# viridityzhu/HiFiHR

Hardware: AMD Instinct MI355X
Metric: train images/sec, FreiHAND 224x224 (ResNet-18 + MANO LBS + render + losses + Adam) (higher is better)
Workload: dtype f32; 1 GPU; BASELINE configs[1]: FreiHAND batch=32/GPU, ResNet-18 encoder + MANO LBS + silhouette/texture render losses, 224x224, aa=3 (672^2 samples); per_gpu_batch=32, global_batch=32, parallelism=dp1

## Files before the change

hifihr_amd/_lib.py:

```python
from __future__ import annotations

import ctypes
import os
from ctypes import POINTER, c_char_p, c_float, c_int, c_int32, c_long, c_size_t, c_void_p

import torch

_HERE = os.path.dirname(os.path.abspath(__file__))
LIB_PATH = os.path.join(_HERE, "libhifihr.so")

_c_float_p = POINTER(c_float)


class _LinearDesc(ctypes.Structure):
    _fields_ = [("x", c_void_p), ("w", c_void_p), ("b", c_void_p), ("y", c_void_p), ("B", c_int), ("I", c_int), ("O", c_int), ("act", c_int),
                ("dy", c_void_p), ("dz_scratch", c_void_p), ("dW_acc", c_void_p), ("db_acc", c_void_p), ("dx", c_void_p)]

_c_int_p = POINTER(c_int32)


class HifihrError(RuntimeError):
    pass


# ... 74 lines not shown
        c.hifihr_conv2d_workspace_bytes.argtypes = [c_int] * 10
        c.hifihr_conv2d_workspace_bytes.restype = c_size_t
        c.hifihr_conv2d_bwd_data.argtypes = [_c_float_p] * 4 + ci + [c_void_p, c_size_t, c_void_p]
        c.hifihr_conv2d_fwd_bnstats.argtypes = [_c_float_p] * 4 + ci + [c_void_p, c_size_t, c_void_p]
        c.hifihr_conv2d_fwd_bnstats_pair_supported.argtypes = [c_int] * 11
        c.hifihr_conv2d_fwd_bnstats_pair.argtypes = [_c_float_p] * 4 + [c_int] * 3 + [_c_float_p] * 3 + [c_int] * 8 + [c_void_p]
        for fn in (c.hifihr_dwconv2d_bwd_data, c.hifihr_dwconv2d_bwd_weight):
            fn.argtypes = [_c_float_p] * 3 + [c_int] * 10 + [c_void_p]
        c.hifihr_dwconv2d_fwd.argtypes = [_c_float_p] * 4 + [c_int] * 10 + [c_void_p]
        c.hifihr_dwconv2d_fwd_bnswish.argtypes = [_c_float_p] * 8 + [c_int] * 10 + [c_void_p]
        c.hifihr_dwconv2d_bwd_weight_bnswish.argtypes = [_c_float_p] * 7 + [c_int] * 10 + [c_void_p]
        c.hifihr_bn_finalize_fwd.argtypes = [_c_float_p, c_long, c_int, c_float, c_float] + [_c_float_p] * 4 + [c_void_p]
        c.hifihr_bn_stats_floats.argtypes = [c_int]
        c.hifihr_bn_stats_floats.restype = c_int
        c.hifihr_bn_stats.argtypes = [_c_float_p, c_long, c_int, _c_float_p, c_void_p]
        c.hifihr_bn_act_fwd.argtypes = [_c_float_p] * 5 + [c_int, c_long, c_int, c_float, c_float] + [_c_float_p] * 5 + [c_void_p]
        c.hifihr_bn_act_eval.argtypes = [_c_float_p] * 6 + [c_int, c_long, c_int, c_float, _c_float_p, c_void_p]
        c.hifihr_bn_act_bwd.argtypes = [_c_float_p] * 7 + [c_int, c_long, c_int] + [_c_float_p] * 5 + [c_void_p]
        c.hifihr_bn_relu_maxpool_supported.argtypes = [c_int] * 4
        c.hifihr_bn_relu_maxpool_fwd.argtypes = [_c_float_p] * 4 + [c_int] * 4 + [c_float, c_float, _c_float_p, c_void_p] + [_c_float_p] * 4 + [c_void_p]
        c.hifihr_bn_relu_maxpool_bwd.argtypes = [_c_float_p, c_void_p] + [_c_float_p] * 5 + [c_int] * 4 + [_c_float_p] * 4 + [c_void_p]
        c.hifihr_bn_relu_maxpool_bwd_y.argtypes = [_c_float_p, _c_float_p, c_void_p] + [_c_float_p] * 5 + [c_int] * 4 + [_c_float_p] * 4 + [c_void_p]
        c.hifihr_conv2d_bwd_weight.argtypes = [_c_float_p] * 3 + ci + [c_void_p]
        c.hifihr_conv2d_bwd_weight_ws.argtypes = [_c_float_p] * 3 + ci + [c_void_p, c_size_t, c_void_p]
        c.hifihr_conv2d_wgrad_workspace_bytes.argtypes = ci
        c.hifihr_conv2d_bwd_weight_c3_supported.argtypes = [c_int] * 8
        c.hifihr_conv2d_bwd_weight_c3.argtypes = [_c_float_p] * 3 + [c_int] * 8 + [c_void_p, c_size_t, c_void_p]
        c.hifihr_conv2d_wgrad_workspace_bytes.restype = c_size_t
        c.hifihr_image_to_nhwc4.argtypes = [_c_float_p, _c_float_p, c_int, c_int, c_int, c_void_p]
        c.hifihr_image_to_nhwc4_padded.argtypes = [_c_float_p, _c_float_p] + [c_int] * 8 + [c_void_p]
        c.hifihr_image_scale_to_nhwc4.argtypes = [_c_float_p, _c_float_p, c_int, c_int, c_int, _c_float_p, _c_float_p, c_void_p]
        c.hifihr_maxpool2d_fwd_notap.argtypes = [_c_float_p] + [c_int] * 7 + [_c_float_p, c_void_p]
        c.hifihr_lpips_tap_max_channels.argtypes = []
        c.hifihr_lpips_tap_max_channels.restype = c_int
        c.hifihr_lpips_tap_partial_floats.argtypes = [c_int]
        c.hifihr_lpips_tap_partial_floats.restype = c_size_t
        c.hifihr_lpips_tap.argtypes = [_c_float_p] * 3 + [c_int] * 4 + [_c_float_p, _c_float_p, c_void_p]
        c.hifihr_lpips_tap_bwd.argtypes = [_c_float_p] * 4 + [c_int] * 4 + [_c_float_p, c_void_p]
        c.hifihr_lpips_tap_bwd_relu.argtypes = [_c_float_p] * 4 + [c_int] * 4 + [_c_float_p, c_void_p]
        c.hifihr_lpips_maxpool_fwd.argtypes = [_c_float_p] + [c_int] * 4 + [_c_float_p, c_void_p]
        c.hifihr_lpips_maxpool_bwd.argtypes = [_c_float_p, _c_float_p] + [c_int] * 4 + [_c_float_p, c_void_p]
        c.hifihr_image_scale_to_nhwc4_bwd.argtypes = [_c_float_p, _c_float_p, c_int, c_int, c_int, _c_float_p, c_void_p]
        c.hifihr_geom_loss_fwd.argtypes = [_c_float_p] * 6 + [_c_int_p] + [c_int] * 7 + [_c_float_p] * 3 + [c_void_p]
        c.hifihr_geom_loss_bwd.argtypes = [_c_float_p] * 6 + [_c_int_p] * 3 + [c_int] * 7 + [_c_float_p] * 6 + [c_void_p]
        c.hifihr_photo_loss_partial_floats.argtypes = []
        c.hifihr_photo_loss_partial_floats.restype = c_int
        c.hifihr_photo_loss_fwd.argtypes = [_c_float_p, _c_float_p, c_void_p, c_int, c_int, c_int, c_float, c_float, c_float] + \
            [_c_float_p] * 4 + [c_void_p]
        c.hifihr_photo_loss_bwd.argtypes = [_c_float_p] * 6 + [c_int, c_int, c_int, c_float, c_float, _c_float_p, c_void_p]
        c.hifihr_sil_post.argtypes = [_c_float_p, _c_float_p, c_int, c_int, c_int, _c_float_p, _c_float_p, c_void_p]
        c.hifihr_linear_fwd.argtypes = [_c_float_p] * 3 + [c_int] * 4 + [_c_float_p] * 2 + [c_float, c_float] + [_c_float_p] * 6 + [c_void_p]
        c.hifihr_linear_bwd.argtypes = [_c_float_p] * 4 + [c_int] * 4 + [_c_float_p] * 10 + [c_void_p]
        c.hifihr_linear_fwd_group.argtypes = [POINTER(_LinearDesc), c_int, c_void_p]
        c.hifihr_linear_bwd_group.argtypes = [POINTER(_LinearDesc), c_int, c_void_p]
        c.hifihr_conv2d_bwd_data_pre.argtypes = [_c_float_p] * 3 + [c_int] * 9 + [c_void_p, c_size_t, c_void_p]
        c.hifihr_conv2d_bwd_data_pre_res.argtypes = [_c_float_p] * 4 + [c_int] * 9 + [c_void_p, c_size_t, c_void_p]
        c.hifihr_conv2d_bwd_data_pre_plus1x1.argtypes = [_c_float_p] * 5 + [c_int] * 9 + [c_void_p]
        c.hifihr_conv2d_bwd_data_pre_plus1x1_supported.argtypes = [c_int] * 9
        c.hifihr_conv2d_bwd_weight_plus1x1.argtypes = [_c_float_p] * 5 + [c_int] * 9 + [c_void_p]
        c.hifihr_conv2d_bwd_weight_plus1x1_supported.argtypes = [c_int] * 9
        c.hifihr_weight_prep.argtypes = [c_void_p, c_int, c_int, c_void_p]
        c.hifihr_freihand_augment.argtypes = [c_void_p, c_void_p, _c_int_p, _c_int_p, c_int, c_int, c_int, _c_float_p, _c_float_p, c_void_p]
        c.hifihr_ho3d_workspace_bytes.argtypes = [c_int, c_int]
        c.hifihr_ho3d_workspace_bytes.restype = c_size_t
        c.hifihr_ho3d_batch.argtypes = ([c_void_p, c_void_p] + [_c_float_p] * 3 + [c_int, c_int, _c_int_p, c_int, c_int, c_void_p, c_size_t] +
                                        [_c_float_p] * 5 + [c_void_p])
        c.hifihr_freihand_batch.argtypes = ([c_void_p, c_void_p] + [_c_float_p] * 4 + [c_int, c_int, _c_int_p, c_int, c_int, c_int, _c_float_p,
                                            _c_float_p, c_void_p] + [_c_float_p] * 6 + [c_void_p, c_void_p])
        c.hifihr_freihand_batch_step.argtypes = ([c_void_p, c_void_p] + [_c_float_p] * 4 + [c_int, c_int, _c_int_p, c_int, c_int, c_int, _c_float_p,
                                                 _c_float_p, c_void_p] + [_c_float_p] * 6 + [c_void_p, c_int, c_float] + [_c_float_p] * 4 + [c_void_p])
        c.hifihr_light_split_fwd.argtypes = [_c_float_p, c_int, _c_float_p, _c_float_p, c_void_p]
        c.hifihr_light_split_bwd.argtypes = [_c_float_p, _c_float_p, _c_float_p, c_int, _c_float_p, c_void_p]
        c.hifihr_wino4_bwd_gemm_pair_supported.argtypes = [c_int] * 5
        c.hifihr_wino4_bwd_gemm_pair.argtypes = [_c_float_p] * 6 + [c_int] * 6 + [c_void_p]
        c.hifihr_loss_total_fwd.argtypes = [POINTER(_c_float_p), POINTER(c_int), c_int, _c_float_p, c_void_p]
        c.hifihr_loss_total_bwd.argtypes = [_c_float_p, POINTER(_c_float_p), POINTER(c_int), POINTER(c_int), c_int, c_void_p]
        c.hifihr_procrustes_error.argtypes = [_c_float_p, _c_float_p, c_int, c_int, _c_float_p, _c_float_p, c_void_p]
        c.hifihr_point_error_hist.argtypes = [_c_float_p, _c_float_p, c_void_p, c_int, c_int, POINTER(ctypes.c_double), c_int, _c_int_p, c_void_p,
                                              c_void_p]
        c.hifihr_fscore_counts.argtypes = [_c_float_p, _c_float_p, c_int, c_int, c_int, POINTER(ctypes.c_double), c_int, _c_int_p, c_void_p]
        c.hifihr_wino_wgrad_gemm.argtypes = [_c_float_p] * 3 + [c_int] * 5 + [c_void_p]
        c.hifihr_wino_dw_transform.argtypes = [_c_float_p, _c_float_p, c_int, c_int, c_int, c_void_p]
        c.hifihr_weight_transpose.argtypes = [_c_float_p, _c_float_p, c_int, c_int, c_int, c_void_p]
        c.hifihr_bgemm_nt.argtypes = [_c_float_p] * 3 + [c_int] * 4 + [c_void_p, c_size_t, c_void_p]
        c.hifihr_bgemm_nt_workspace_bytes.argtypes = [c_int] * 4
        c.hifihr_bgemm_nt_workspace_bytes.restype = c_size_t
        c.hifihr_renderer_set_light_mode.argtypes = [c_void_p, c_int]
        c.hifihr_texture_pca_fwd.argtypes = [_c_float_p] * 3 + [c_int, c_int, c_long, _c_float_p, c_void_p]
        c.hifihr_texture_pca_bwd.argtypes = [_c_float_p] * 2 + [c_int, c_int, c_long, _c_float_p, c_void_p]
        c.hifihr_comm_last_error.restype = c_char_p
        c.hifihr_comm_get_unique_id.argtypes = [c_void_p]
        c.hifihr_comm_init.argtypes = [POINTER(c_void_p), c_int, c_int, c_void_p]
        c.hifihr_comm_allreduce_f32.argtypes = [c_void_p, _c_float_p, c_size_t, c_void_p]
        c.hifihr_comm_broadcast_f32.argtypes = [c_void_p, _c_float_p, c_size_t, c_int, c_void_p]
        c.hifihr_comm_destroy.argtypes = [c_void_p]
        c.hifihr_wino_tile.argtypes = [c_int] * 5
        c.hifihr_wino_gemm_workspace_bytes.argtypes = [c_int] * 6
        c.hifihr_wino_gemm_workspace_bytes.restype = c_size_t
        c.hifihr_wino_weight_transform.argtypes = [_c_float_p, _c_float_p, c_int, c_int, c_int, c_int, c_void_p]
        c.hifihr_wino_input_transform.argtypes = [_c_float_p, _c_float_p] + [c_int] * 5 + [c_void_p]
        c.hifihr_wino_gemm.argtypes = [_c_float_p] * 3 + [c_int] * 6 + [c_void_p, c_size_t, c_void_p]
        c.hifihr_wino_output_transform.argtypes = [_c_float_p] * 3 + [c_int] * 5 + [c_void_p]
        c.hifihr_wino_output_transform_act.argtypes = [_c_float_p] * 3 + [c_int] * 6 + [c_void_p]
        c.hifihr_conv3x3_c64_wino_supported.argtypes = [c_int] * 5
        c.hifihr_conv3x3_c64_wino.argtypes = [c_void_p, c_void_p, c_void_p, c_int, c_void_p, c_void_p, c_int, c_int, c_int, c_void_p]
        c.hifihr_conv3x3_c64_wino_res.argtypes = [c_void_p, c_void_p, c_void_p, c_void_p, c_int, c_int, c_int, c_void_p]
        c.hifihr_conv3x3_c64_bwd_pair_supported.argtypes = [c_int] * 3
        c.hifihr_conv3x3_c64_bwd_pair.argtypes = [c_void_p] * 7 + [c_size_t] + [c_int] * 3 + [c_void_p]
        c.hifihr_conv3x3_c64_bwd_pair_slabs.argtypes = [c_void_p] * 6 + [c_size_t] + [c_int] * 3 + [c_void_p, c_void_p]
        c.hifihr_conv_halo_wgrad_reduce_multi.argtypes = [c_void_p, c_int, c_void_p]
        c.hifihr_wino_bn_input_supported.argtypes = [c_int, c_int]
        c.hifihr_wino_bn_input_transform.argtypes = [_c_float_p] * 7 + [c_int] * 5 + [c_float, c_float] + [_c_float_p] * 4 + [c_void_p]
        c.hifihr_wino_output_transform_bnred.argtypes = [_c_float_p] * 10 + [c_int] * 5 + [c_void_p]
        c.hifihr_wino_bn_bwd_dual_transform.argtypes = [_c_float_p] * 8 + [c_int] * 5 + [_c_float_p] * 2 + [c_void_p]
        c.hifihr_bn_bwd_apply.argtypes = [_c_float_p] * 5 + [c_long, c_int] + [_c_float_p] * 4 + [c_void_p]
        c.hifihr_joint_terms_fwd.argtypes = [_c_float_p] * 4 + [c_int] * 3 + [POINTER(c_float), _c_float_p, c_void_p]
        c.hifihr_joint_terms_bwd.argtypes = [_c_float_p] * 4 + [c_int] * 3 + [POINTER(c_float)] + [_c_float_p] * 3 + [c_void_p]
        c.hifihr_wino_dy_transform.argtypes = [_c_float_p] * 2 + [c_int] * 5 + [c_void_p]
        c.hifihr_wino_input_dy_transform.argtypes = [_c_float_p] * 3 + [c_int] * 5 + [c_void_p]
        c.hifihr_wino_wgrad_parts.argtypes = [c_int] * 6
        c.hifihr_wino_wgrad_gemm_parts.argtypes = [_c_float_p] * 3 + [c_int] * 7 + [c_void_p]
        c.hifihr_wino_dw_transform_parts.argtypes = [_c_float_p, c_int, _c_float_p, c_int, c_int, c_int, c_void_p]
        c.hifihr_bgemm_describe.argtypes = [c_int] * 5 + [ctypes.c_char_p, c_int]
        c.hifihr_conv2d_describe.argtypes = [c_int] * 10 + [ctypes.c_char_p, c_int]
        c.hifihr_bgemm_tn_parts.argtypes = [c_int] * 4
        c.hifihr_bgemm_tn.argtypes = [_c_float_p] * 3 + [c_int] * 5 + [c_void_p]
        c.hifihr_wino4_dw_transform_multi.argtypes = [c_void_p, c_int, c_void_p]
        c.hifihr_se_pool.argtypes = [_c_float_p, c_int, c_int, c_int, _c_float_p, c_void_p]
        c.hifihr_se_scale.argtypes = [_c_float_p, _c_float_p, _c_float_p, c_float, c_int, c_int, c_int, _c_float_p, c_void_p]
        c.hifihr_se_bwd_gate.argtypes = [_c_float_p, _c_float_p, c_int, c_int, c_int, _c_float_p, c_void_p]
        c.hifihr_se_mlp_supported.argtypes = [c_int, c_int]
        c.hifihr_wino_tiles.argtypes = [c_int] * 4
        c.hifihr_wino_tiles.restype = c_long
        c.hifihr_wino_tiles_computed.argtypes = [c_int] * 4
        c.hifihr_wino_tiles_computed.restype = c_long
        c.hifihr_zero_page_ready.argtypes = [c_void_p]
        c.hifihr_drop_connect_add.argtypes = [_c_float_p, _c_float_p, _c_float_p, c_float, c_int, c_size_t, _c_float_p, c_void_p]
        c.hifihr_se_mlp_fwd.argtypes = [_c_float_p] * 5 + [c_int] * 3 + [_c_float_p] * 4 + [c_void_p]
        c.hifihr_se_mlp_bwd.argtypes = [_c_float_p] * 7 + [c_int] * 3 + [_c_float_p] * 7 + [c_void_p]
        c.hifihr_mmpool_fwd.argtypes = [_c_float_p, _c_float_p, c_int, c_int, c_int, _c_float_p, _c_int_p, _c_float_p, _c_float_p, c_void_p]
        c.hifihr_mmpool_bwd.argtypes = [_c_float_p, _c_float_p, _c_int_p, _c_float_p, _c_float_p, c_int, c_int, c_int, _c_float_p,
                                        _c_float_p, c_void_p]
        c.hifihr_maxpool2d_fwd.argtypes = [_c_float_p] + [c_int] * 7 + [_c_float_p, c_void_p, c_void_p]
        c.hifihr_maxpool2d_bwd.argtypes = [_c_float_p, c_void_p] + [c_int] * 7 + [_c_float_p, c_void_p]
        c.hifihr_maxpool2d_fwd_flat.argtypes = [_c_float_p] + [c_int] * 7 + [_c_float_p, c_void_p, c_void_p]
        c.hifihr_maxpool2d_bwd_flat.argtypes = [_c_float_p, c_void_p] + [c_int] * 7 + [_c_float_p, c_void_p]
        c.hifihr_maxpool2d_bwd_relu.argtypes = [_c_float_p, c_void_p, _c_float_p] + [c_int] * 7 + [_c_float_p, c_void_p]
        c.hifihr_wino_output_transform_mask.argtypes = [_c_float_p] * 3 + [c_int] * 5 + [c_void_p]
        c.hifihr_adam_step.argtypes = [_c_float_p, _c_float_p, _c_float_p, _c_float_p, c_size_t, c_float, c_float, c_float,
                                       c_float, c_float, c_float, c_int, c_void_p]
        c.hifihr_adam_state_bytes.restype = c_size_t
        c.hifihr_adam_state_bytes.argtypes = []
        c.hifihr_adam_step_counted.argtypes = [_c_float_p, _c_float_p, _c_float_p, _c_float_p, c_size_t, c_float, c_float, c_float, c_void_p, c_void_p]
        c.hifihr_grad_guard_bytes.restype = c_size_t
        c.hifihr_grad_guard_bytes.argtypes = []
        c.hifihr_grad_norm_workspace_bytes.restype = c_size_t
        c.hifihr_grad_norm_workspace_bytes.argtypes = [c_size_t]
        c.hifihr_grad_norm.argtypes = [_c_float_p, c_size_t, c_float, c_float, c_void_p, c_void_p, c_void_p]
        c.hifihr_adam_step_guarded.argtypes = [_c_float_p, _c_float_p, _c_float_p, _c_float_p, c_size_t, c_float, c_float, c_float, c_float,
                                               c_float, c_float, c_int, c_void_p, c_void_p, c_void_p]
        c.hifihr_adam_step_dyn.argtypes = [_c_float_p, _c_float_p, _c_float_p, _c_float_p, c_size_t, c_float, c_float, c_float,
                                           c_float, c_float, _c_float_p, c_void_p]
        c.hifihr_renderer_destroy.argtypes = [c_void_p]
        c.hifihr_render_workspace_bytes.argtypes = [c_void_p, c_int]
        c.hifihr_render_workspace_bytes.restype = c_size_t
        c.hifihr_render_fwd.argtypes = [c_void_p, _c_float_p, _c_float_p, c_int, _c_float_p, _c_float_p, _c_float_p, c_int,
                                        _c_float_p, _c_int_p, c_void_p, c_void_p]
        c.hifihr_render_bwd.argtypes = [c_void_p, _c_float_p, _c_float_p, _c_float_p, _c_float_p, _c_int_p, _c_float_p, c_int,
                                        _c_float_p, _c_float_p, _c_float_p, _c_float_p, c_void_p, c_void_p]
        c.hifihr_soft_sil_workspace_bytes.argtypes = [c_void_p, c_int]
        c.hifihr_soft_sil_workspace_bytes.restype = c_size_t
        c.hifihr_soft_sil_fwd.argtypes = [c_void_p, _c_float_p, _c_float_p, c_int, c_float, c_float, _c_float_p, _c_float_p, c_void_p, c_void_p]
        c.hifihr_soft_sil_bwd.argtypes = [c_void_p, _c_float_p, _c_float_p, _c_float_p, _c_float_p, c_int, c_float, c_float, _c_float_p, c_void_p,
                                          c_void_p]
        c.hifihr_soft_sil_loss_fwd.argtypes = [_c_float_p, c_void_p, c_int, c_int, c_int, c_float, c_float, c_void_p, _c_float_p, c_void_p]
        c.hifihr_soft_sil_loss_bwd.argtypes = [_c_float_p, c_void_p, c_int, c_void_p, _c_float_p, c_int, c_int, c_float, c_float, _c_float_p,
                                               c_void_p]
        c.hifihr_mesh_topology_create.argtypes = [_c_int_p, c_int, c_int]
        c.hifihr_mesh_topology_create.restype = c_void_p
        c.hifihr_mesh_topology_destroy.argtypes = [c_void_p]
        c.hifihr_mesh_topology_counts.argtypes = [c_void_p, _c_int_p, _c_int_p, _c_int_p]
        c.hifihr_mesh_reg_partial_floats.argtypes = [c_void_p, c_int]
        c.hifihr_mesh_reg_partial_floats.restype = c_size_t
        c.hifihr_mesh_reg_fwd.argtypes = [c_void_p, _c_float_p, c_int, c_float, c_float, _c_float_p, _c_float_p, _c_float_p, c_void_p]
        c.hifihr_mesh_reg_bwd.argtypes = [c_void_p, _c_float_p, _c_float_p, _c_float_p, c_int, c_float, c_float, _c_float_p, c_void_p]
        c.hifihr_chamfer_geometry.argtypes = [_c_int_p, _c_int_p]
        c.hifihr_chamfer_geometry.restype = None
        c.hifihr_chamfer_workspace_bytes.argtypes = [c_int, c_int, c_int]
        c.hifihr_chamfer_workspace_bytes.restype = c_size_t
        c.hifihr_chamfer_fwd.argtypes = [_c_float_p, _c_float_p, c_int, c_int, c_int, c_float, c_float, _c_int_p, _c_int_p, c_void_p, c_void_p,
                                         c_void_p, _c_float_p, c_void_p, c_void_p]
        c.hifihr_chamfer_bwd.argtypes = [_c_float_p, _c_float_p, _c_int_p, _c_int_p, _c_float_p, c_int, c_int, c_int, c_float, c_float,
                                         _c_float_p, _c_float_p, c_void_p]
        c.hifihr_renderer_set_uv.argtypes = [c_void_p, _c_int_p, _c_float_p, c_int]
        c.hifihr_render_uv_scratch_bytes.argtypes = [c_void_p, c_int]
        c.hifihr_render_uv_scratch_bytes.restype = c_size_t
        c.hifihr_render_fwd_uv.argtypes = [c_void_p, _c_float_p, _c_float_p, c_int, c_int, _c_float_p, _c_float_p, _c_float_p, c_int, _c_float_p,
                                           _c_int_p, _c_float_p, c_void_p, c_void_p]
        c.hifihr_render_bwd_uv.argtypes = [c_void_p, _c_float_p, _c_float_p, c_int, c_int, _c_float_p, _c_float_p, _c_float_p, _c_int_p, _c_float_p,
                                           c_int] + [_c_float_p] * 6 + [c_void_p, c_void_p]

    def check(self, rc: int, what: str):
        if rc != 0:
            raise HifihrError(f"{what} failed ({rc}): {self.c.hifihr_last_error().decode()}")

    def mano_create(self, tables) -> c_void_p:
        h = c_void_p()
        keep = [_np_fp(a) for a in (tables.v_template, tables.shapedirs, tables.posedirs, tables.J_regressor,
                                    tables.weights, tables.hands_components, tables.hands_mean)]
        self.check(self.c.hifihr_mano_create(ctypes.byref(h), *[k[1] for k in keep]), "hifihr_mano_create")
        return h

    def mano_destroy(self, h):
        self.c.hifihr_mano_destroy(h)

    def mano_lbs_fwd(self, h, pose, beta, verts, jtr, saved):
        B = pose.shape[0]
        assert pose.shape == (B, 48) and beta.shape == (B, 10) and verts.shape == (B, 778, 3)
        self.check(self.c.hifihr_mano_lbs_fwd(h, _fp(pose), _fp(beta), B, _fp(verts), _fp(jtr), _fp(saved),
                                              _stream_of(pose)), "hifihr_mano_lbs_fwd")

    def mano_lbs_bwd(self, h, pose, beta, saved, gverts, gjtr, gpose, gbeta):
        B = pose.shape[0]
        self.check(self.c.hifihr_mano_lbs_bwd(h, _fp(pose), _fp(beta), _fp(saved), _fp(gverts), _fp(gjtr), B,
                                              _fp(gpose), _fp(gbeta), _stream_of(pose)), "hifihr_mano_lbs_bwd")

    def mano_joints_fwd(self, h, verts, root_id, joints_rel, verts_rel, root):
        B = verts.shape[0]
        self.check(self.c.hifihr_mano_joints_fwd(h, _fp(verts), B, root_id, _fp(joints_rel), _fp(verts_rel), _fp(root),
                                                 _stream_of(verts)), "hifihr_mano_joints_fwd")

    def mano_joints_bwd(self, h, gjoints_rel, gverts_rel, groot, root_id, gverts):
        B = gverts.shape[0]
        self.check(self.c.hifihr_mano_joints_bwd(h, _fp(gjoints_rel), _fp(gverts_rel), _fp(groot), B, root_id,
                                                 _fp(gverts), _stream_of(gverts)), "hifihr_mano_joints_bwd")

    def mano_full_fwd(self, h, pose, beta, root_id, root_xyz, verts, joints_rel, verts_rel, verts_cam, root, saved):
        B = pose.shape[0]
        self.check(self.c.hifihr_mano_full_fwd(h, _fp(pose), _fp(beta), B, int(root_id), _fp(root_xyz), _fp(verts), _fp(joints_rel), _fp(verts_rel),
                                               _fp(verts_cam), _fp(root), _fp(saved), _stream_of(pose)), "hifihr_mano_full_fwd")

    def mano_full_bwd(self, h, pose, beta, saved, gjoints_rel, gverts_rel, gverts_cam, groot, root_id, gpose, gbeta, gpose_add=None,
                      gbeta_add=None):
        B = pose.shape[0]
        self.check(self.c.hifihr_mano_full_bwd(h, _fp(pose), _fp(beta), _fp(saved), _fp(gjoints_rel), _fp(gverts_rel), _fp(gverts_cam),
                                               _fp(groot), _fp(gpose_add), _fp(gbeta_add), B, int(root_id), _fp(gpose), _fp(gbeta),
                                               _stream_of(pose)), "hifihr_mano_full_bwd")

    def lbs_create(self, v_template, shapedirs, j_regressor, weights, parents) -> c_void_p:
        V, J, S = int(v_template.shape[0]), int(weights.shape[1]), int(shapedirs.shape[2])
        assert shapedirs.shape == (V, 3, S) and j_regressor.shape == (J, V) and weights.shape == (V, J) and len(parents) == J
        h = c_void_p()
        keep = [_np_fp(a) for a in (v_template, shapedirs, j_regressor, weights)]
        import numpy as np
        par = np.ascontiguousarray(np.asarray(parents, dtype=np.int32))
        self.check(self.c.hifihr_lbs_create(ctypes.byref(h), V, J, S, *[k[1] for k in keep], par.ctypes.data_as(_c_int_p)), "hifihr_lbs_create")
        return h

    def lbs_destroy(self, h):
        self.c.hifihr_lbs_destroy(h)

    def lbs_fwd(self, h, theta, beta, verts, joints):
        self.check(self.c.hifihr_lbs_fwd(h, _fp(theta), _fp(beta), theta.shape[0], _fp(verts), _fp(joints), _stream_of(theta)), "hifihr_lbs_fwd")

    def lbs_bwd(self, h, theta, beta, gverts, gjoints, scratch, gtheta, gbeta):
        self.check(self.c.hifihr_lbs_bwd(h, _fp(theta), _fp(beta), _fp(gverts), _fp(gjoints), theta.shape[0], _fp(scratch), _fp(gtheta),
                                         _fp(gbeta), _stream_of(theta)), "hifihr_lbs_bwd")

    @staticmethod
    def _ws(ws):
        if ws is None:
            return c_void_p(0), c_size_t(0)
        assert ws.is_contiguous()
        return c_void_p(ws.data_ptr()), c_size_t(ws.numel() * ws.element_size())

    def conv2d_workspace_bytes(self, N, H, W, C, K, R, S, stride, pad, bwd_data=False):
        return int(self.c.hifihr_conv2d_workspace_bytes(N, H, W, C, K, R, S, stride, pad, int(bool(bwd_data))))

    def conv2d_fwd(self, x, w, bias, y, N, H, W, C, K, R, S, stride, pad, ws=None, act=0):
        self.check(self.c.hifihr_conv2d_fwd(_fp(x), _fp(w), _fp(bias), int(act), _fp(y), N, H, W, C, K, R, S, stride, pad,
                                            *self._ws(ws), _stream_of(x)), "hifihr_conv2d_fwd")

    def bias_relu_bwd(self, dy, y, M, C, g, db_acc):
        self.check(self.c.hifihr_bias_relu_bwd(_fp(dy), _fp(y), c_long(M), C, _fp(g), _fp(db_acc), _stream_of(dy)),
                   "hifihr_bias_relu_bwd")

    def conv2d_fwd_bnstats(self, x, w, y, stats, N, H, W, C, K, R, S, stride, pad, ws=None):
        self.check(self.c.hifihr_conv2d_fwd_bnstats(_fp(x), _fp(w), _fp(y), _fp(stats), N, H, W, C, K, R, S, stride, pad,
                                                    *self._ws(ws), _stream_of(x)), "hifihr_conv2d_fwd_bnstats")

    def conv2d_fwd_bnstats_pair_supported(self, N, H, W, C, stride, K1, R1, pad1, K2, R2, pad2):
        return bool(self.c.hifihr_conv2d_fwd_bnstats_pair_supported(N, H, W, C, stride, K1, R1, pad1, K2, R2, pad2))

    def conv2d_fwd_bnstats_pair(self, x, w1, y1, stats1, K1, R1, pad1, w2, y2, stats2, K2, R2, pad2, N, H, W, C, stride):
        self.check(self.c.hifihr_conv2d_fwd_bnstats_pair(_fp(x), _fp(w1), _fp(y1), _fp(stats1), K1, R1, pad1, _fp(w2), _fp(y2), _fp(stats2), K2, R2, pad2,
                                                         N, H, W, C, stride, _stream_of(x)), "hifihr_conv2d_fwd_bnstats_pair")

    def bn_stats_floats(self, C):
        return int(self.c.hifihr_bn_stats_floats(int(C)))

    def bn_stats(self, x, M, C, stats):
        self.check(self.c.hifihr_bn_stats(_fp(x), c_long(M), C, _fp(stats), _stream_of(x)), "hifihr_bn_stats")

    def bn_act_fwd(self, x, stats, gamma, beta, residual, act, M, C, eps, momentum, y, save_mean, save_invstd, rmean, rvar):
        self.check(self.c.hifihr_bn_act_fwd(_fp(x), _fp(stats), _fp(gamma), _fp(beta), _fp(residual), int(act), c_long(M), C,
                                            c_float(eps), c_float(momentum), _fp(y), _fp(save_mean), _fp(save_invstd), _fp(rmean),
# ... 451 lines not shown
                                            _fp(rm), _fp(rv), _fp(y), _fp(z), _fp(sm), _fp(si), _stream_of(x)), "hifihr_linear_fwd")

    def linear_bwd(self, dy, y, x, w, act, dz, dW_acc, db_acc, dx, bn=None, z=None):
        B, I = x.shape
        O = w.shape[0]
        gamma, z_bn, sm, si, dg, dbt = bn if bn is not None else (None,) * 6
        z = z_bn if bn is not None else z
        self.check(self.c.hifihr_linear_bwd(_fp(dy), _fp(y), _fp(x), _fp(w), B, I, O, int(act), _fp(gamma), _fp(z), _fp(sm), _fp(si),
                                            _fp(dz), _fp(dW_acc), _fp(db_acc), _fp(dg), _fp(dbt), _fp(dx), _stream_of(x)),
                   "hifihr_linear_bwd")

    @staticmethod
    def _descs(members):
        arr = (_LinearDesc * len(members))()
        p = lambda t: None if t is None else t.data_ptr()
        for d, m in zip(arr, members):
            d.x, d.w, d.b, d.y = p(m["x"]), p(m["w"]), p(m.get("b")), p(m["y"])
            d.B, d.I, d.O, d.act = m["x"].shape[0], m["x"].shape[1], m["w"].shape[0], int(m["act"])
            d.dy, d.dz_scratch, d.dW_acc, d.db_acc, d.dx = p(m.get("dy")), p(m.get("dz")), p(m.get("dW")), p(m.get("db")), p(m.get("dx"))
        return arr

    def linear_fwd_group(self, members):
        self.check(self.c.hifihr_linear_fwd_group(self._descs(members), len(members), _stream_of(members[0]["x"])), "hifihr_linear_fwd_group")

    def linear_bwd_group(self, members):
        self.check(self.c.hifihr_linear_bwd_group(self._descs(members), len(members), _stream_of(members[0]["x"])), "hifihr_linear_bwd_group")

    def mmpool_fwd(self, x, p, B, HW, C, y, argmax, xmax, xavg):
        self.check(self.c.hifihr_mmpool_fwd(_fp(x), _fp(p), B, HW, C, _fp(y), _ip(argmax), _fp(xmax), _fp(xavg), _stream_of(x)),
                   "hifihr_mmpool_fwd")

    def mmpool_bwd(self, gy, p, argmax, xmax, xavg, B, HW, C, dx, dp_acc):
        self.check(self.c.hifihr_mmpool_bwd(_fp(gy), _fp(p), _ip(argmax), _fp(xmax), _fp(xavg), B, HW, C, _fp(dx), _fp(dp_acc),
                                            _stream_of(gy)), "hifihr_mmpool_bwd")

    def maxpool2d_fwd(self, x, N, H, W, C, k, s, p, y, tap):
        assert tap.dtype == torch.uint8 and tap.is_contiguous()
        self.check(self.c.hifihr_maxpool2d_fwd(_fp(x), N, H, W, C, k, s, p, _fp(y), c_void_p(tap.data_ptr()), _stream_of(x)),
                   "hifihr_maxpool2d_fwd")

    def maxpool2d_fwd_flat(self, x, N, H, W, C, k, s, p, y_flat, tap):
        self.check(self.c.hifihr_maxpool2d_fwd_flat(_fp(x), N, H, W, C, k, s, p, _fp(y_flat), c_void_p(tap.data_ptr()), _stream_of(x)),
                   "hifihr_maxpool2d_fwd_flat")

    def maxpool2d_bwd_flat(self, gy_flat, tap, N, H, W, C, k, s, p, dx):
        self.check(self.c.hifihr_maxpool2d_bwd_flat(_fp(gy_flat), c_void_p(tap.data_ptr()), N, H, W, C, k, s, p, _fp(dx), _stream_of(gy_flat)),
                   "hifihr_maxpool2d_bwd_flat")

    def maxpool2d_bwd(self, gy, tap, N, H, W, C, k, s, p, dx, relu_y=None):
        if relu_y is not None:
            self.check(self.c.hifihr_maxpool2d_bwd_relu(_fp(gy), c_void_p(tap.data_ptr()), _fp(relu_y), N, H, W, C, k, s, p, _fp(dx),
                                                        _stream_of(gy)), "hifihr_maxpool2d_bwd_relu")
            return
        self.check(self.c.hifihr_maxpool2d_bwd(_fp(gy), c_void_p(tap.data_ptr()), N, H, W, C, k, s, p, _fp(dx), _stream_of(gy)),
                   "hifihr_maxpool2d_bwd")

    def conv2d_bwd_data(self, dy, w, dx, scratch, N, H, W, C, K, R, S, stride, pad, ws=None):
        self.check(self.c.hifihr_conv2d_bwd_data(_fp(dy), _fp(w), _fp(dx), _fp(scratch), N, H, W, C, K, R, S, stride, pad,
                                                 *self._ws(ws), _stream_of(dy)), "hifihr_conv2d_bwd_data")

    def conv2d_wgrad_workspace_bytes(self, N, H, W, C, K, R, S, stride, pad):
        return int(self.c.hifihr_conv2d_wgrad_workspace_bytes(N, H, W, C, K, R, S, stride, pad))

    def conv2d_bwd_weight(self, x, dy, dw, N, H, W, C, K, R, S, stride, pad, ws=None):
        p, n = self._ws(ws)
        self.check(self.c.hifihr_conv2d_bwd_weight_ws(_fp(x), _fp(dy), _fp(dw), N, H, W, C, K, R, S, stride, pad, p, n, _stream_of(x)),
                   "hifihr_conv2d_bwd_weight")

    def image_to_nhwc4(self, images, out):
        B, _, H, W = images.shape
        self.check(self.c.hifihr_image_to_nhwc4(_fp(images), _fp(out), B, H, W, _stream_of(images)), "hifihr_image_to_nhwc4")

    def image_to_nhwc4_padded(self, images, out, pad4, normalize):
        B, _, H, W = images.shape
        pl, pr, pt, pb = pad4
        self.check(self.c.hifihr_image_to_nhwc4_padded(_fp(images), _fp(out), B, H, W, pt, pl, pb, pr, int(bool(normalize)),
                                                       _stream_of(images)), "hifihr_image_to_nhwc4_padded")

    def image_scale_to_nhwc4(self, images, out, shift3, scale3):
        B, _, H, W = images.shape
        sh, sc = (c_float * 3)(*[float(v) for v in shift3]), (c_float * 3)(*[float(v) for v in scale3])
        self.check(self.c.hifihr_image_scale_to_nhwc4(_fp(images), _fp(out), B, H, W, sh, sc, _stream_of(images)), "hifihr_image_scale_to_nhwc4")

    def maxpool2d_fwd_notap(self, x, N, H, W, C, k, s, p, y):
        self.check(self.c.hifihr_maxpool2d_fwd_notap(_fp(x), N, H, W, C, k, s, p, _fp(y), _stream_of(x)), "hifihr_maxpool2d_fwd_notap")

    def lpips_tap_max_channels(self):
        return int(self.c.hifihr_lpips_tap_max_channels())

    def lpips_tap_partial_floats(self, B):
        return int(self.c.hifihr_lpips_tap_partial_floats(int(B)))

    def lpips_tap(self, f0, f1, w, B, HW, C, partial, val, accumulate=False):
        self.check(self.c.hifihr_lpips_tap(_fp(f0), _fp(f1), _fp(w), B, HW, C, int(bool(accumulate)), _fp(partial), _fp(val), _stream_of(f0)),
                   "hifihr_lpips_tap")

    def lpips_tap_bwd(self, f0, f1, w, gval, B, HW, C, gf0, accumulate=False, relu=False):
        fn, name = (self.c.hifihr_lpips_tap_bwd_relu, "hifihr_lpips_tap_bwd_relu") if relu else (self.c.hifihr_lpips_tap_bwd, "hifihr_lpips_tap_bwd")
        self.check(fn(_fp(f0), _fp(f1), _fp(w), _fp(gval), B, HW, C, int(bool(accumulate)), _fp(gf0), _stream_of(f0)), name)

    def lpips_maxpool_fwd(self, x, N, H, W, C, y):
        self.check(self.c.hifihr_lpips_maxpool_fwd(_fp(x), N, H, W, C, _fp(y), _stream_of(x)), "hifihr_lpips_maxpool_fwd")

    def lpips_maxpool_bwd(self, gy, x, N, H, W, C, dx):
        self.check(self.c.hifihr_lpips_maxpool_bwd(_fp(gy), _fp(x), N, H, W, C, _fp(dx), _stream_of(x)), "hifihr_lpips_maxpool_bwd")

    def image_scale_to_nhwc4_bwd(self, g4, gimg, scale3):
        B, _, H, W = gimg.shape
        sc = (c_float * 3)(*[float(v) for v in scale3])
        self.check(self.c.hifihr_image_scale_to_nhwc4_bwd(_fp(g4), _fp(gimg), B, H, W, sc, _stream_of(gimg)), "hifihr_image_scale_to_nhwc4_bwd")

    def ssim_partial_count(self, planes, H, W):
        return int(self.c.hifihr_ssim_partial_count(planes, H, W))

    def ssim_fwd(self, window, img1, img2, partial, dA, dB, dC):
        planes, H, W = img1.shape[0] * img1.shape[1], img1.shape[2], img1.shape[3]
        self.check(self.c.hifihr_ssim_fwd(window, _fp(img1), _fp(img2), planes, H, W, _fp(partial), _fp(dA), _fp(dB), _fp(dC),
                                          _stream_of(img1)), "hifihr_ssim_fwd")

    def ssim_finish(self, partial, scale, offset, out):
        self.check(self.c.hifihr_ssim_finish(_fp(partial), partial.numel(), c_float(scale), c_float(offset), _fp(out), _stream_of(partial)),
                   "hifihr_ssim_finish")

    def ssim_bwd_scaled(self, window, img1, img2, dA, dB, dC, grad_out, out_scale, gimg1):
        planes, H, W = img1.shape[0] * img1.shape[1], img1.shape[2], img1.shape[3]
        self.check(self.c.hifihr_ssim_bwd_scaled(window, _fp(img1), _fp(img2), _fp(dA), _fp(dB), _fp(dC), _fp(grad_out), c_float(out_scale),
                                                 planes, H, W, _fp(gimg1), _stream_of(img1)), "hifihr_ssim_bwd_scaled")

    def ssim_bwd(self, window, img1, img2, dA, dB, dC, grad_out, gimg1):
        planes, H, W = img1.shape[0] * img1.shape[1], img1.shape[2], img1.shape[3]
        self.check(self.c.hifihr_ssim_bwd(window, _fp(img1), _fp(img2), _fp(dA), _fp(dB), _fp(dC), _fp(grad_out), planes, H, W,
                                          _fp(gimg1), _stream_of(img1)), "hifihr_ssim_bwd")

    def adam_step(self, p, g, m, v, grad_scale, lr, beta1, beta2, eps, weight_decay, step):
        n = p.numel()
        assert g.numel() == n and m.numel() == n and v.numel() == n
        self.check(self.c.hifihr_adam_step(_fp(p), _fp(g), _fp(m), _fp(v), c_size_t(n), c_float(grad_scale), c_float(lr),
                                           c_float(beta1), c_float(beta2), c_float(eps), c_float(weight_decay), int(step),
                                           _stream_of(p)), "hifihr_adam_step")

    @staticmethod
    def adam_state_image(lr, beta1, beta2, step):
        import struct
        b1, b2 = float(beta1), float(beta2)
        return torch.frombuffer(bytearray(struct.pack("<dddddii", float(lr), b1, b2, b1 ** int(step), b2 ** int(step), int(step), 0)),
                                dtype=torch.uint8).clone()

    def adam_step_counted(self, p, g, m, v, grad_scale, eps, weight_decay, state):
        n = p.numel()
        assert state.dtype == torch.uint8 and state.numel() == int(self.c.hifihr_adam_state_bytes()) and state.device == p.device
        self.check(self.c.hifihr_adam_step_counted(_fp(p), _fp(g), _fp(m), _fp(v), c_size_t(n), c_float(grad_scale), c_float(eps),
                                                   c_float(weight_decay), c_void_p(state.data_ptr()), _stream_of(p)), "hifihr_adam_step_counted")

    def adam_step_dyn(self, p, g, m, v, grad_scale, beta1, beta2, eps, weight_decay, dyn):
        n = p.numel()
        self.check(self.c.hifihr_adam_step_dyn(_fp(p), _fp(g), _fp(m), _fp(v), c_size_t(n), c_float(grad_scale), c_float(beta1),
                                               c_float(beta2), c_float(eps), c_float(weight_decay), _fp(dyn), _stream_of(p)),
                   "hifihr_adam_step_dyn")

    def grad_guard_alloc(self, n, device):
        guard = torch.zeros(int(self.c.hifihr_grad_guard_bytes()), dtype=torch.uint8, device=device)
        ws = torch.zeros(int(self.c.hifihr_grad_norm_workspace_bytes(c_size_t(n))), dtype=torch.uint8, device=device)
        return guard, ws

    def grad_norm(self, g, grad_scale, max_norm, guard, ws):
        n = g.numel()
        assert guard.dtype == torch.uint8 and guard.numel() == int(self.c.hifihr_grad_guard_bytes()) and guard.device == g.device
        assert ws.dtype == torch.uint8 and ws.numel() >= int(self.c.hifihr_grad_norm_workspace_bytes(c_size_t(n))) and ws.device == g.device
        self.check(self.c.hifihr_grad_norm(_fp(g), c_size_t(n), c_float(grad_scale), c_float(max_norm), c_void_p(guard.data_ptr()),
                                           c_void_p(ws.data_ptr()), _stream_of(g)), "hifihr_grad_norm")

    def adam_step_guarded(self, p, g, m, v, grad_scale, lr, beta1, beta2, eps, weight_decay, step, state, guard):
        n = p.numel()
        assert g.numel() == n and m.numel() == n and v.numel() == n
        assert guard.dtype == torch.uint8 and guard.numel() == int(self.c.hifihr_grad_guard_bytes()) and guard.device == p.device
        if state is not None:
            assert state.dtype == torch.uint8 and state.numel() == int(self.c.hifihr_adam_state_bytes()) and state.device == p.device
        self.check(self.c.hifihr_adam_step_guarded(_fp(p), _fp(g), _fp(m), _fp(v), c_size_t(n), c_float(grad_scale), c_float(lr),
                                                   c_float(beta1), c_float(beta2), c_float(eps), c_float(weight_decay), int(step),
                                                   c_void_p(state.data_ptr()) if state is not None else c_void_p(0),
                                                   c_void_p(guard.data_ptr()), _stream_of(p)), "hifihr_adam_step_guarded")

    @staticmethod
    def grad_guard_unpack(raw):
        import struct
        norm, coef, finite, steps, clipped, skipped, _ = struct.unpack("<dfiiiii", bytes(raw))
        return {"norm": norm, "clip_coef": coef, "finite": bool(finite), "steps": steps, "clipped": clipped, "skipped": skipped}

    def renderer_create(self, faces, V, image_size=224, aa=3, ambient=(0.5, 0.5, 0.5), mat_diffuse=(0.8, 0.8, 0.8),
                        specular=(0.04, 0.04, 0.04), shininess=30.0, background=(1.0, 1.0, 1.0)) -> c_void_p:
        import numpy as np
        f = np.ascontiguousarray(faces, dtype=np.int32)
        h = c_void_p()
        a, m, s, b = (_np_fp(x) for x in (ambient, mat_diffuse, specular, background))
        self.check(self.c.hifihr_renderer_create(ctypes.byref(h), f.ctypes.data_as(_c_int_p), int(V), int(f.shape[0]),
                                                 int(image_size), int(aa), a[1], m[1], s[1], c_float(shininess), b[1]),
                   "hifihr_renderer_create")
        return h

    def texture_pca_fwd(self, coef, basis, mean, out):
        B, K = coef.shape
        n = basis.shape[1]
        self.check(self.c.hifihr_texture_pca_fwd(_fp(coef), _fp(basis), _fp(mean), B, K, c_long(n), _fp(out), _stream_of(coef)), "hifihr_texture_pca_fwd")

    def texture_pca_bwd(self, gtex, basis, dcoef_zeroed):
        B, K = dcoef_zeroed.shape
        n = basis.shape[1]
        self.check(self.c.hifihr_texture_pca_bwd(_fp(gtex), _fp(basis), B, K, c_long(n), _fp(dcoef_zeroed), _stream_of(gtex)), "hifihr_texture_pca_bwd")

    def renderer_set_light_mode(self, h, point_lights):
        self.check(self.c.hifihr_renderer_set_light_mode(h, int(bool(point_lights))), "hifihr_renderer_set_light_mode")

    def renderer_destroy(self, h):
        self.c.hifihr_renderer_destroy(h)

    def render_workspace_bytes(self, h, B) -> int:
        return int(self.c.hifihr_render_workspace_bytes(h, int(B)))

    def render_fwd(self, h, verts, vcolors, cam, light_color, light_dir, rgba, face_id, ws):
        B = verts.shape[0]
        batched = 1 if vcolors.dim() == 3 else 0
        self.check(self.c.hifihr_render_fwd(h, _fp(verts), _fp(vcolors), batched, _fp(cam), _fp(light_color), _fp(light_dir), B,
                                            _fp(rgba), _ip(face_id), c_void_p(ws.data_ptr()), _stream_of(verts)),
                   "hifihr_render_fwd")

    def renderer_set_uv(self, h, faces_uvs, verts_uvs):
        import numpy as np
        fu = np.ascontiguousarray(faces_uvs, dtype=np.int32)
        vu = np.ascontiguousarray(verts_uvs, dtype=np.float32)
        self.check(self.c.hifihr_renderer_set_uv(h, fu.ctypes.data_as(_c_int_p), vu.ctypes.data_as(_c_float_p), vu.shape[0]),
                   "hifihr_renderer_set_uv")

    def render_uv_scratch_bytes(self, h, B):
        return int(self.c.hifihr_render_uv_scratch_bytes(h, B))

    def render_fwd_uv(self, h, verts, maps, cam, light_color, light_dir, rgba, face_id, texels, ws):
        B, TH, TW = maps.shape[0], maps.shape[1], maps.shape[2]
        self.check(self.c.hifihr_render_fwd_uv(h, _fp(verts), _fp(maps), TH, TW, _fp(cam), _fp(light_color), _fp(light_dir), B, _fp(rgba),
                                               _ip(face_id), _fp(texels), c_void_p(ws.data_ptr()), _stream_of(verts)), "hifihr_render_fwd_uv")

    def render_bwd_uv(self, h, verts, maps, cam, light_color, light_dir, face_id, grad_rgba, texels, gtexels, gverts, gmaps, glc, gld, ws):
        B, TH, TW = maps.shape[0], maps.shape[1], maps.shape[2]
        self.check(self.c.hifihr_render_bwd_uv(h, _fp(verts), _fp(maps), TH, TW, _fp(cam), _fp(light_color), _fp(light_dir), _ip(face_id),
                                               _fp(grad_rgba), B, _fp(texels), _fp(gtexels), _fp(gverts), _fp(gmaps), _fp(glc), _fp(gld),
                                               c_void_p(ws.data_ptr()), _stream_of(verts)), "hifihr_render_bwd_uv")

    def render_bwd(self, h, verts, cam, light_color, light_dir, face_id, grad_rgba, gverts, gvcolors, glc, gld, ws):
        B = verts.shape[0]
        self.check(self.c.hifihr_render_bwd(h, _fp(verts), _fp(cam), _fp(light_color), _fp(light_dir), _ip(face_id),
                                            _fp(grad_rgba), B, _fp(gverts), _fp(gvcolors), _fp(glc), _fp(gld),
                                            c_void_p(ws.data_ptr()), _stream_of(verts)), "hifihr_render_bwd")

    def soft_sil_workspace_bytes(self, h, B) -> int:
        return int(self.c.hifihr_soft_sil_workspace_bytes(h, int(B)))

    def soft_sil_fwd(self, h, verts, cam, sigma, blur_radius, alpha, neglog, ws):
        self.check(self.c.hifihr_soft_sil_fwd(h, _fp(verts), _fp(cam), verts.shape[0], c_float(sigma), c_float(blur_radius), _fp(alpha),
                                              _fp(neglog), c_void_p(ws.data_ptr()), _stream_of(verts)), "hifihr_soft_sil_fwd")

    def soft_sil_bwd(self, h, verts, cam, neglog, galpha, sigma, blur_radius, gverts, ws):
        self.check(self.c.hifihr_soft_sil_bwd(h, _fp(verts), _fp(cam), _fp(neglog), _fp(galpha), verts.shape[0], c_float(sigma),
                                              c_float(blur_radius), _fp(gverts), c_void_p(ws.data_ptr()), _stream_of(verts)),
                   "hifihr_soft_sil_bwd")

    @staticmethod
    def _mask_arg(mask):
        assert mask.dtype in (torch.float32, torch.int64) and mask.is_contiguous(), (mask.dtype, mask.stride())
        return c_void_p(mask.data_ptr()), int(mask.dtype == torch.int64)

    def soft_sil_loss_fwd(self, alpha, mask, lam_sil, lam_iou, sums, out):
        B = alpha.shape[0]
        assert sums.dtype == torch.float64 and sums.is_contiguous() and mask.numel() == alpha.numel()
        mp, kind = self._mask_arg(mask)
        self.check(self.c.hifihr_soft_sil_loss_fwd(_fp(alpha), mp, kind, B, alpha.numel() // max(B, 1), c_float(lam_sil), c_float(lam_iou),
                                                   c_void_p(sums.data_ptr()), _fp(out), _stream_of(alpha)), "hifihr_soft_sil_loss_fwd")

    def soft_sil_loss_bwd(self, alpha, mask, sums, gout, lam_sil, lam_iou, galpha):
        B = alpha.shape[0]
        mp, kind = self._mask_arg(mask)
        self.check(self.c.hifihr_soft_sil_loss_bwd(_fp(alpha), mp, kind, c_void_p(sums.data_ptr()), _fp(gout), B, alpha.numel() // max(B, 1),
                                                   c_float(lam_sil), c_float(lam_iou), _fp(galpha), _stream_of(alpha)),
                   "hifihr_soft_sil_loss_bwd")

    def mesh_topology_create(self, faces, V) -> c_void_p:
        import numpy as np
        f = np.ascontiguousarray(faces, dtype=np.int32)
        assert f.ndim == 2 and f.shape[1] == 3, f.shape
        h = self.c.hifihr_mesh_topology_create(f.ctypes.data_as(_c_int_p), int(f.shape[0]), int(V))
        if not h:
            raise HifihrError(f"hifihr_mesh_topology_create failed: {self.c.hifihr_last_error().decode()}")
        return c_void_p(h)

    def mesh_topology_destroy(self, h):
        self.c.hifihr_mesh_topology_destroy(h)

    def mesh_topology_counts(self, h):
        v, e, q = c_int32(), c_int32(), c_int32()
        self.check(self.c.hifihr_mesh_topology_counts(h, ctypes.byref(v), ctypes.byref(e), ctypes.byref(q)), "hifihr_mesh_topology_counts")
        return v.value, e.value, q.value

    def mesh_reg_partial_floats(self, h, B) -> int:
        return int(self.c.hifihr_mesh_reg_partial_floats(h, int(B)))

    def mesh_reg_fwd(self, h, verts, lam_lap, lam_nc, unit, partial, out):
        self.check(self.c.hifihr_mesh_reg_fwd(h, _fp(verts), verts.shape[0], c_float(lam_lap), c_float(lam_nc), _fp(unit), _fp(partial),
                                              _fp(out), _stream_of(verts)), "hifihr_mesh_reg_fwd")
# ... 43 lines not shown
```

hifihr_amd/csrc/adam.hip:

```cpp
#include <hip/hip_runtime.h>

#include "hifihr_internal.h"

namespace hifihr {

struct GradGuard {
  double norm;
  float coef;
  int finite;
  int steps, clipped, skipped;
  int pad;
};

template <bool kGuard>
__global__ __launch_bounds__(256) void adam_kernel_t(float* __restrict__ p, const float* __restrict__ g, float* __restrict__ m,
                                                    float* __restrict__ v, size_t n, float grad_scale, float beta1, float beta2,
                                                    float eps, float weight_decay, float step_size, float inv_sqrt_bc2,
                                                    const float* __restrict__ dyn, const GradGuard* __restrict__ guard) {
  if (dyn) { step_size = dyn[0]; inv_sqrt_bc2 = dyn[1]; }
  if constexpr (kGuard) {
    if (!guard->finite) return;
    grad_scale = grad_scale * guard->coef;
  }
  const size_t n4 = n / 4;
  const size_t stride = (size_t)gridDim.x * blockDim.x;
  float4* p4 = reinterpret_cast<float4*>(p);
  const float4* g4 = reinterpret_cast<const float4*>(g);
  float4* m4 = reinterpret_cast<float4*>(m);
  float4* v4 = reinterpret_cast<float4*>(v);
  for (size_t i = (size_t)blockIdx.x * blockDim.x + threadIdx.x; i < n4; i += stride) {
    float4 pp = p4[i], gg = g4[i], mm = m4[i], vv = v4[i];
    float* pa = reinterpret_cast<float*>(&pp);
    float* ga = reinterpret_cast<float*>(&gg);
    float* ma = reinterpret_cast<float*>(&mm);
    float* va = reinterpret_cast<float*>(&vv);
#pragma unroll
    for (int k = 0; k < 4; ++k) {
      const float gr = ga[k] * grad_scale + weight_decay * pa[k];
      ma[k] = beta1 * ma[k] + (1.f - beta1) * gr;
      va[k] = beta2 * va[k] + (1.f - beta2) * gr * gr;
      const float denom = sqrtf(va[k]) * inv_sqrt_bc2 + eps;
      pa[k] = pa[k] - step_size * (ma[k] / denom);
    }
    p4[i] = pp; m4[i] = mm; v4[i] = vv;
  }
  for (size_t i = n4 * 4 + (size_t)blockIdx.x * blockDim.x + threadIdx.x; i < n; i += stride) {
    const float gr = g[i] * grad_scale + weight_decay * p[i];
    const float mi = beta1 * m[i] + (1.f - beta1) * gr;
    const float vi = beta2 * v[i] + (1.f - beta2) * gr * gr;
    m[i] = mi; v[i] = vi;
    p[i] = p[i] - step_size * (mi / (sqrtf(vi) * inv_sqrt_bc2 + eps));
  }
}

constexpr auto adam_kernel = adam_kernel_t<false>;
constexpr auto adam_kernel_guarded = adam_kernel_t<true>;

struct AdamState {
  double lr, beta1, beta2;
  double pow1, pow2;
  int step;
  int done;
};
template <bool kGuard>
__global__ __launch_bounds__(256) void adam_kernel_counted_t(float* __restrict__ p, const float* __restrict__ g, float* __restrict__ m,
                                                            float* __restrict__ v, size_t n, float grad_scale, float eps,
                                                            float weight_decay, AdamState* __restrict__ st,
                                                            const GradGuard* __restrict__ guard) {
  __shared__ float sc[4];
  int t = 0;
  double q1 = 0.0, q2 = 0.0;
  if (threadIdx.x == 0) {
    t = st->step + 1;
    const double b1 = st->beta1, b2 = st->beta2;
    q1 = st->pow1 * b1; q2 = st->pow2 * b2;
    sc[0] = (float)(st->lr / (1.0 - q1));
    sc[1] = (float)(1.0 / sqrt(1.0 - q2));
    sc[2] = (float)b1; sc[3] = (float)b2;
  }
  __syncthreads();
  const float step_size = sc[0], inv_sqrt_bc2 = sc[1], beta1 = sc[2], beta2 = sc[3];
  bool run = true;
  if constexpr (kGuard) {
    run = guard->finite != 0;
    grad_scale = grad_scale * guard->coef;
  }
  const size_t n4 = run ? n / 4 : 0;
  const size_t n_end = run ? n : 0;
  const size_t stride = (size_t)gridDim.x * blockDim.x;
  float4* p4 = reinterpret_cast<float4*>(p);
  const float4* g4 = reinterpret_cast<const float4*>(g);
  float4* m4 = reinterpret_cast<float4*>(m);
  float4* v4 = reinterpret_cast<float4*>(v);
  for (size_t i = (size_t)blockIdx.x * blockDim.x + threadIdx.x; i < n4; i += stride) {
    float4 pp = p4[i], gg = g4[i], mm = m4[i], vv = v4[i];
    float* pa = reinterpret_cast<float*>(&pp);
    float* ga = reinterpret_cast<float*>(&gg);
    float* ma = reinterpret_cast<float*>(&mm);
    float* va = reinterpret_cast<float*>(&vv);
#pragma unroll
    for (int k = 0; k < 4; ++k) {
      const float gr = ga[k] * grad_scale + weight_decay * pa[k];
      ma[k] = beta1 * ma[k] + (1.f - beta1) * gr;
      va[k] = beta2 * va[k] + (1.f - beta2) * gr * gr;
      const float denom = sqrtf(va[k]) * inv_sqrt_bc2 + eps;
      pa[k] = pa[k] - step_size * (ma[k] / denom);
    }
    p4[i] = pp; m4[i] = mm; v4[i] = vv;
  }
  for (size_t i = n4 * 4 + (size_t)blockIdx.x * blockDim.x + threadIdx.x; i < n_end; i += stride) {
    const float gr = g[i] * grad_scale + weight_decay * p[i];
    const float mi = beta1 * m[i] + (1.f - beta1) * gr;
    const float vi = beta2 * v[i] + (1.f - beta2) * gr * gr;
    m[i] = mi; v[i] = vi;
    p[i] = p[i] - step_size * (mi / (sqrtf(vi) * inv_sqrt_bc2 + eps));
  }
  __syncthreads();
  if (threadIdx.x == 0) {
    if (atomicAdd(&st->done, 1) == (int)gridDim.x - 1) {
      st->step = t;
      st->pow1 = q1; st->pow2 = q2;
      st->done = 0;
    }
  }
}

constexpr auto adam_kernel_counted = adam_kernel_counted_t<false>;
constexpr auto adam_kernel_counted_guarded = adam_kernel_counted_t<true>;

__device__ __forceinline__ double block_sum_f64(double s, double* lds) {
#pragma unroll
  for (int off = 32; off > 0; off >>= 1) s += __shfl_down(s, off, 64);
  if ((threadIdx.x & 63) == 0) lds[threadIdx.x >> 6] = s;
  __syncthreads();
  return (lds[0] + lds[1]) + (lds[2] + lds[3]);
}

__global__ __launch_bounds__(256) void grad_sqsum_kernel(const float* __restrict__ g, size_t n, double* __restrict__ partial) {
  __shared__ double lds[4];
  const size_t n4 = n / 4;
  const size_t stride = (size_t)gridDim.x * blockDim.x;
  const float4* g4 = reinterpret_cast<const float4*>(g);
  double s0 = 0.0, s1 = 0.0;
  for (size_t i = (size_t)blockIdx.x * blockDim.x + threadIdx.x; i < n4; i += stride) {
    const float4 gg = g4[i];
    const double x = gg.x, y = gg.y, z = gg.z, w = gg.w;
    s0 += x * x; s1 += y * y;
    s0 += z * z; s1 += w * w;
  }
  for (size_t i = n4 * 4 + (size_t)blockIdx.x * blockDim.x + threadIdx.x; i < n; i += stride) {
    const double x = g[i];
    s0 += x * x;
  }
  const double s = block_sum_f64(s0 + s1, lds);
  if (threadIdx.x == 0) partial[blockIdx.x] = s;
}

__global__ __launch_bounds__(256) void grad_norm_finish_kernel(const double* __restrict__ partial, int nblk, float grad_scale, float max_norm,
                                                              GradGuard* __restrict__ guard) {
  __shared__ double lds[4];
  double s = 0.0;
  for (int i = threadIdx.x; i < nblk; i += 256) s += partial[i];
  s = block_sum_f64(s, lds);
  if (threadIdx.x == 0) {
    const bool finite = fabs(s) <= 1.7976931348623157e308;
    const double norm = fabs((double)grad_scale) * sqrt(s);
    float coef = 0.f;
    if (finite) {
      const double c = (double)max_norm / (norm + 1e-6);
      coef = c >= 1.0 ? 1.0f : (float)c;
    }
    guard->norm = norm;
    guard->coef = coef;
    guard->finite = finite ? 1 : 0;
    guard->steps += 1;
    if (finite && coef < 1.0f) guard->clipped += 1;
    if (!finite) guard->skipped += 1;
  }
}

static size_t adam_blocks(size_t n) {
  size_t blocks = (n / 4 + 255) / 256;
  if (blocks > 2048) blocks = 2048;
  if (blocks < 1) blocks = 1;
  return blocks;
}

size_t grad_guard_bytes() { return sizeof(GradGuard); }
size_t grad_norm_workspace_bytes(size_t n) { return adam_blocks(n) * sizeof(double); }

hipError_t launch_grad_norm(const float* g, size_t n, float grad_scale, float max_norm, void* guard, void* ws, hipStream_t st) {
  const size_t blocks = adam_blocks(n);
  hipLaunchKernelGGL(grad_sqsum_kernel, dim3((unsigned)blocks), dim3(256), 0, st, g, n, static_cast<double*>(ws));
  hipError_t e = hipGetLastError();
  if (e != hipSuccess) return e;
  hipLaunchKernelGGL(grad_norm_finish_kernel, dim3(1), dim3(256), 0, st, static_cast<const double*>(ws), (int)blocks, grad_scale, max_norm,
                     static_cast<GradGuard*>(guard));
  return hipGetLastError();
}

hipError_t launch_adam_guarded(float* p, const float* g, float* m, float* v, size_t n, float grad_scale, float lr, float beta1, float beta2,
                               float eps, float weight_decay, int step, void* state, const void* guard, hipStream_t st) {
  const size_t blocks = adam_blocks(n);
  if (state) {
    hipLaunchKernelGGL(adam_kernel_counted_guarded, dim3((unsigned)blocks), dim3(256), 0, st, p, g, m, v, n, grad_scale, eps, weight_decay,
                       static_cast<AdamState*>(state), static_cast<const GradGuard*>(guard));
    return hipGetLastError();
  }
  const double bc1 = 1.0 - pow((double)beta1, (double)step);
  const double bc2 = 1.0 - pow((double)beta2, (double)step);
  const float step_size = (float)((double)lr / bc1);
  const float inv_sqrt_bc2 = (float)(1.0 / sqrt(bc2));
  hipLaunchKernelGGL(adam_kernel_guarded, dim3((unsigned)blocks), dim3(256), 0, st, p, g, m, v, n, grad_scale, beta1, beta2, eps,
                     weight_decay, step_size, inv_sqrt_bc2, (const float*)nullptr, static_cast<const GradGuard*>(guard));
  return hipGetLastError();
}

size_t adam_state_bytes() { return sizeof(AdamState); }

hipError_t launch_adam_counted(float* p, const float* g, float* m, float* v, size_t n, float grad_scale, float eps, float weight_decay,
                               void* state, hipStream_t st) {
  size_t blocks = (n / 4 + 255) / 256;
  if (blocks > 2048) blocks = 2048;
  if (blocks < 1) blocks = 1;
  hipLaunchKernelGGL(adam_kernel_counted, dim3((unsigned)blocks), dim3(256), 0, st, p, g, m, v, n, grad_scale, eps, weight_decay,
                     static_cast<AdamState*>(state), (const GradGuard*)nullptr);
  return hipGetLastError();
}

hipError_t launch_adam(float* p, const float* g, float* m, float* v, size_t n, float grad_scale, float lr, float beta1,
                       float beta2, float eps, float weight_decay, int step, const float* dyn, hipStream_t st) {
  float step_size = 0.f, inv_sqrt_bc2 = 0.f;
  if (!dyn) {
    const double bc1 = 1.0 - pow((double)beta1, (double)step);
    const double bc2 = 1.0 - pow((double)beta2, (double)step);
    step_size = (float)((double)lr / bc1);
    inv_sqrt_bc2 = (float)(1.0 / sqrt(bc2));
  }
  size_t blocks = (n / 4 + 255) / 256;
  if (blocks > 2048) blocks = 2048;
  if (blocks < 1) blocks = 1;
  hipLaunchKernelGGL(adam_kernel, dim3((unsigned)blocks), dim3(256), 0, st, p, g, m, v, n, grad_scale, beta1, beta2, eps,
                     weight_decay, step_size, inv_sqrt_bc2, dyn, (const GradGuard*)nullptr);
  return hipGetLastError();
}

}
```

hifihr_amd/csrc/hifihr_api.hip:

```cpp
#include <hip/hip_runtime.h>

#include <algorithm>
#include <array>
#include <cmath>
#include <cstdarg>
#include <cstdio>
#include <cstring>
#include <new>
#include <vector>

#include "../../include/hifihr.h"
#include "hifihr_internal.h"
#include "mano_math.h"

namespace {

thread_local char g_err[512] = "";

int fail(int code, const char* fmt, ...) {
  va_list ap;
  va_start(ap, fmt);
  vsnprintf(g_err, sizeof(g_err), fmt, ap);
  va_end(ap);
  return code;
// ... 444 lines not shown
    }
    for (int k = 0; k < 3; ++k) {
      const int i = v[k], j = v[(k + 1) % 3], o = v[(k + 2) % 3];
      sides.push_back({std::min(i, j), std::max(i, j), f, o});
    }
  }
  std::sort(sides.begin(), sides.end());
  std::vector<int> off(V + 1, 0), quads;
  std::vector<std::array<int, 2>> edges;
  for (size_t s = 0; s < sides.size();) {
    size_t t = s;
    while (t < sides.size() && sides[t][0] == sides[s][0] && sides[t][1] == sides[s][1]) ++t;
    edges.push_back({sides[s][0], sides[s][1]});
    for (size_t a = s; a < t; ++a)
      for (size_t b = a + 1; b < t; ++b) {
        if (quads.size() / 4 + 1 >= ((size_t)1 << 29)) {
          fail(HIFIHR_EINVAL, "hifihr_mesh_topology_create: too many face pairs on shared edges (4 Q >= 2^31)");
          return nullptr;
        }
        quads.insert(quads.end(), {sides[s][0], sides[s][1], sides[a][3], sides[b][3]});
      }
    s = t;
  }
  const int E = (int)edges.size(), Q = (int)(quads.size() / 4);
  for (const auto& e : edges) { off[e[0] + 1]++; off[e[1] + 1]++; }
  for (int v = 0; v < V; ++v) off[v + 1] += off[v];
  std::vector<int> idx((size_t)2 * E), cur(off.begin(), off.end() - 1);
  for (const auto& e : edges) idx[cur[e[1]]++] = e[0];
  for (const auto& e : edges) idx[cur[e[0]]++] = e[1];
  std::vector<float> deg((size_t)V);
  for (int v = 0; v < V; ++v) deg[v] = (float)(off[v + 1] - off[v]);
  std::vector<int> qoff(V + 1, 0), qidx((size_t)4 * Q);
  for (int x : quads) qoff[x + 1]++;
  for (int v = 0; v < V; ++v) qoff[v + 1] += qoff[v];
  std::vector<int> qcur(qoff.begin(), qoff.end() - 1);
  for (int q = 0; q < Q; ++q)
    for (int r = 0; r < 4; ++r) qidx[qcur[quads[4 * (size_t)q + r]]++] = q * 4 + r;
  hifihr_mesh_topology* h = new (std::nothrow) hifihr_mesh_topology();
  if (!h) {
    fail(HIFIHR_ENOMEM, "hifihr_mesh_topology_create: out of host memory");
    return nullptr;
  }
  if (upload_i(h->nbr_off, off) || upload_i(h->nbr_idx, idx) || upload(h->deg, deg) || upload_i(h->quads, quads) ||
      upload_i(h->vq_off, qoff) || upload_i(h->vq_idx, qidx)) {
    delete h;
    return nullptr;
  }
  hifihr::MeshTopoDev& d = h->dev;
  d.V = V; d.E = E; d.Q = Q;
  d.nbr_off = (const int*)h->nbr_off.p; d.nbr_idx = (const int*)h->nbr_idx.p; d.deg = (const float*)h->deg.p;
  d.quads = (const int*)h->quads.p; d.vq_off = (const int*)h->vq_off.p; d.vq_idx = (const int*)h->vq_idx.p;
  return h;
}

int hifihr_mesh_topology_destroy(hifihr_mesh_topology_t* h) {
  delete h;
  return HIFIHR_OK;
}

int hifihr_mesh_topology_counts(const hifihr_mesh_topology_t* h, int* V, int* E, int* Q) {
  if (!h) return fail(HIFIHR_EINVAL, "hifihr_mesh_topology_counts: null handle");
  if (V) *V = h->dev.V;
  if (E) *E = h->dev.E;
  if (Q) *Q = h->dev.Q;
  return HIFIHR_OK;
}

size_t hifihr_mesh_reg_partial_floats(const hifihr_mesh_topology_t* h, int B) {
  if (!h || B < 0) return 0;
  return (size_t)B * hifihr::mesh_reg_blocks(h->dev) * 2;
}

namespace {
bool mesh_reg_args_ok(const hifihr_mesh_topology_t* h, int B, float lam_lap, float lam_nc) {
  return h && B >= 0 && (long long)B * h->dev.V * 3 < (1LL << 31) && std::isfinite(lam_lap) && std::isfinite(lam_nc);
}
}

int hifihr_mesh_reg_fwd(const hifihr_mesh_topology_t* h, const float* verts, int B, float lam_lap, float lam_nc, float* unit, float* partial,
                        float* out, void* stream) {
  if (!verts || !unit || !partial || !out || !mesh_reg_args_ok(h, B, lam_lap, lam_nc))
    return fail(HIFIHR_EINVAL, "hifihr_mesh_reg_fwd: bad argument (B >= 0, B V 3 < 2^31, finite weights)");
  if (B == 0) return HIFIHR_OK;
  HIP_TRY(hifihr::launch_mesh_reg_fwd(h->dev, verts, B, lam_lap, lam_nc, unit, partial, out, (hipStream_t)stream));
  return HIFIHR_OK;
}

int hifihr_mesh_reg_bwd(const hifihr_mesh_topology_t* h, const float* verts, const float* unit, const float* gout, int B, float lam_lap,
                        float lam_nc, float* gverts, void* stream) {
  if (!verts || !unit || !gout || !gverts || !mesh_reg_args_ok(h, B, lam_lap, lam_nc))
    return fail(HIFIHR_EINVAL, "hifihr_mesh_reg_bwd: bad argument (B >= 0, B V 3 < 2^31, finite weights)");
  if (B == 0) return HIFIHR_OK;
  HIP_TRY(hifihr::launch_mesh_reg_bwd(h->dev, verts, unit, gout, B, lam_lap, lam_nc, gverts, (hipStream_t)stream));
  return HIFIHR_OK;
}

void hifihr_chamfer_geometry(int* queries_per_workgroup, int* tile_points) {
  if (queries_per_workgroup) *queries_per_workgroup = hifihr::kChamferQ;
  if (tile_points) *tile_points = hifihr::kChamferTile;
}

namespace {
bool chamfer_grid_ok(int B, int N, int M) { return (long long)B * 2 * hifihr::chamfer_chunks(N, M) <= 0x7fffffffLL; }
}

size_t hifihr_chamfer_workspace_bytes(int B, int N, int M) {
  if (B < 0 || N < 1 || M < 1) return 0;
  return (size_t)B * 2 * (size_t)hifihr::chamfer_chunks(N, M) * sizeof(double);
}

int hifihr_chamfer_fwd(const float* x, const float* y, int B, int N, int M, float w_xy, float w_yx, int32_t* idx_xy, int32_t* idx_yx,
                       double* min_xy, double* min_yx, double* sums, float* out, void* ws, void* stream) {
  if (!x || !y || !idx_xy || !idx_yx || !min_xy || !min_yx || !sums || !out || !ws || B < 0 || N < 1 || M < 1 || !std::isfinite(w_xy) ||
      !std::isfinite(w_yx) || !chamfer_grid_ok(B, N, M))
    return fail(HIFIHR_EINVAL, "hifihr_chamfer_fwd: bad argument (B >= 0, N, M >= 1, finite weights, 2 B chunks < 2^31)");
  if (B == 0) return HIFIHR_OK;
  HIP_TRY(hifihr::launch_chamfer_fwd(x, y, B, N, M, w_xy, w_yx, idx_xy, idx_yx, min_xy, min_yx, sums, out, (double*)ws, (hipStream_t)stream));
  return HIFIHR_OK;
}

int hifihr_chamfer_bwd(const float* x, const float* y, const int32_t* idx_xy, const int32_t* idx_yx, const float* gout, int B, int N, int M,
                       float w_xy, float w_yx, float* gx, float* gy, void* stream) {
  if (!x || !y || !idx_xy || !idx_yx || !gout || B < 0 || N < 1 || M < 1 || !std::isfinite(w_xy) || !std::isfinite(w_yx) ||
      !chamfer_grid_ok(B, N, M))
    return fail(HIFIHR_EINVAL, "hifihr_chamfer_bwd: bad argument (B >= 0, N, M >= 1, finite weights, 2 B chunks < 2^31)");
  if (B == 0 || (!gx && !gy)) return HIFIHR_OK;
  HIP_TRY(hifihr::launch_chamfer_bwd(x, y, idx_xy, idx_yx, gout, B, N, M, w_xy, w_yx, gx, gy, (hipStream_t)stream));
  return HIFIHR_OK;
}

int hifihr_adam_step(float* params, const float* grads, float* exp_avg, float* exp_avg_sq, size_t n, float grad_scale,
                     float lr, float beta1, float beta2, float eps, float weight_decay, int step, void* stream) {
  if (!params || !grads || !exp_avg || !exp_avg_sq || step < 1) return fail(HIFIHR_EINVAL, "hifihr_adam_step: bad argument");
  if (((uintptr_t)params | (uintptr_t)grads | (uintptr_t)exp_avg | (uintptr_t)exp_avg_sq) & 15)
    return fail(HIFIHR_EINVAL, "hifihr_adam_step: buffers must be 16-byte aligned");
  if (n == 0) return HIFIHR_OK;
  HIP_TRY(hifihr::launch_adam(params, grads, exp_avg, exp_avg_sq, n, grad_scale, lr, beta1, beta2, eps, weight_decay, step,
                              nullptr, (hipStream_t)stream));
  return HIFIHR_OK;
}

size_t hifihr_adam_state_bytes(void) { return hifihr::adam_state_bytes(); }

int hifihr_adam_step_counted(float* params, const float* grads, float* exp_avg, float* exp_avg_sq, size_t n, float grad_scale, float eps,
                             float weight_decay, void* state_d, void* stream) {
  if (!params || !grads || !exp_avg || !exp_avg_sq || !state_d) return fail(HIFIHR_EINVAL, "hifihr_adam_step_counted: bad argument");
  if ((((uintptr_t)params | (uintptr_t)grads | (uintptr_t)exp_avg | (uintptr_t)exp_avg_sq) & 15) || ((uintptr_t)state_d & 7))
    return fail(HIFIHR_EINVAL, "hifihr_adam_step_counted: buffers must be 16-byte aligned (the state: 8)");
  if (n == 0) return HIFIHR_OK;
  HIP_TRY(hifihr::launch_adam_counted(params, grads, exp_avg, exp_avg_sq, n, grad_scale, eps, weight_decay, state_d, (hipStream_t)stream));
  return HIFIHR_OK;
}

int hifihr_adam_step_dyn(float* params, const float* grads, float* exp_avg, float* exp_avg_sq, size_t n, float grad_scale,
                         float beta1, float beta2, float eps, float weight_decay, const float* dyn_d, void* stream) {
  if (!params || !grads || !exp_avg || !exp_avg_sq || !dyn_d) return fail(HIFIHR_EINVAL, "hifihr_adam_step_dyn: bad argument");
  if (((uintptr_t)params | (uintptr_t)grads | (uintptr_t)exp_avg | (uintptr_t)exp_avg_sq) & 15)
    return fail(HIFIHR_EINVAL, "hifihr_adam_step_dyn: buffers must be 16-byte aligned");
  if (n == 0) return HIFIHR_OK;
  HIP_TRY(hifihr::launch_adam(params, grads, exp_avg, exp_avg_sq, n, grad_scale, 0.f, beta1, beta2, eps, weight_decay, 1, dyn_d,
                              (hipStream_t)stream));
  return HIFIHR_OK;
}

size_t hifihr_grad_guard_bytes(void) { return hifihr::grad_guard_bytes(); }
size_t hifihr_grad_norm_workspace_bytes(size_t n) { return hifihr::grad_norm_workspace_bytes(n); }

int hifihr_grad_norm(const float* grads, size_t n, float grad_scale, float max_norm, void* guard_d, void* ws_d, void* stream) {
  if (!grads || !guard_d || !ws_d) return fail(HIFIHR_EINVAL, "hifihr_grad_norm: bad argument");
  if (((uintptr_t)grads & 15) || (((uintptr_t)guard_d | (uintptr_t)ws_d) & 7))
    return fail(HIFIHR_EINVAL, "hifihr_grad_norm: grads_d must be 16-byte aligned, guard_d and ws_d 8-byte");
  if (!(max_norm > 0.f) || !std::isfinite(grad_scale))
    return fail(HIFIHR_EINVAL, "hifihr_grad_norm: max_norm must be > 0 (+inf allowed) and grad_scale finite");
  if (n == 0) return HIFIHR_OK;
  HIP_TRY(hifihr::launch_grad_norm(grads, n, grad_scale, max_norm, guard_d, ws_d, (hipStream_t)stream));
  return HIFIHR_OK;
}

int hifihr_adam_step_guarded(float* params, const float* grads, float* exp_avg, float* exp_avg_sq, size_t n, float grad_scale, float lr,
                             float beta1, float beta2, float eps, float weight_decay, int step, void* state_d, const void* guard_d,
                             void* stream) {
  if (!params || !grads || !exp_avg || !exp_avg_sq || !guard_d || (!state_d && step < 1))
    return fail(HIFIHR_EINVAL, "hifihr_adam_step_guarded: bad argument");
  if ((((uintptr_t)params | (uintptr_t)grads | (uintptr_t)exp_avg | (uintptr_t)exp_avg_sq) & 15) ||
      (((uintptr_t)state_d | (uintptr_t)guard_d) & 7))
    return fail(HIFIHR_EINVAL, "hifihr_adam_step_guarded: buffers must be 16-byte aligned (the state and the guard block: 8)");
  if (!std::isfinite(grad_scale)) return fail(HIFIHR_EINVAL, "hifihr_adam_step_guarded: grad_scale must be finite");
  if (n == 0) return HIFIHR_OK;
  HIP_TRY(hifihr::launch_adam_guarded(params, grads, exp_avg, exp_avg_sq, n, grad_scale, lr, beta1, beta2, eps, weight_decay, step, state_d,
                                      guard_d, (hipStream_t)stream));
  return HIFIHR_OK;
}

static int conv_dims_ok(int N, int H, int W, int C, int K, int R, int S, int stride, int pad) {
  return N > 0 && H > 0 && W > 0 && C > 0 && K > 0 && R > 0 && S > 0 && stride > 0 && pad >= 0 && (H + 2 * pad - R) >= 0 &&
         (W + 2 * pad - S) >= 0;
}

static hifihr::ConvGeom conv_geom(int N, int H, int W, int C, int K, int R, int S, int stride, int pad) {
  return hifihr::ConvGeom{N, H, W, C, (H + 2 * pad - R) / stride + 1, (W + 2 * pad - S) / stride + 1, K, R, S, stride, pad, 0};
}
static hifihr::ConvGeom conv_dgrad_geom(int N, int H, int W, int C, int K, int R, int S, int stride, int pad) {
  const hifihr::ConvGeom f = conv_geom(N, H, W, C, K, R, S, stride, pad);
  return hifihr::ConvGeom{N, f.OH, f.OW, K, H, W, C, R, S, stride, pad, 1};
}

size_t hifihr_conv2d_workspace_bytes(int N, int H, int W, int C, int K, int R, int S, int stride, int pad, int bwd_data) {
  if (!conv_dims_ok(N, H, W, C, K, R, S, stride, pad)) return 0;
  return hifihr::conv_sk_workspace_bytes(bwd_data ? conv_dgrad_geom(N, H, W, C, K, R, S, stride, pad) : conv_geom(N, H, W, C, K, R, S, stride, pad));
}

int hifihr_conv2d_fwd(const float* x, const float* w, const float* bias, int act, float* y, int N, int H, int W, int C, int K, int R,
                      int S, int stride, int pad, void* ws, size_t ws_bytes, void* stream) {
  if (!x || !w || !y || !conv_dims_ok(N, H, W, C, K, R, S, stride, pad) || C % 4 || act < 0 || act > 1)
    return fail(HIFIHR_EINVAL, "hifihr_conv2d_fwd: bad argument (C must be a multiple of 4; act 0/1)");
  hifihr::ConvGeom g = conv_geom(N, H, W, C, K, R, S, stride, pad);
  g.relu = act;
  HIP_TRY(hifihr::launch_conv_igemm(g, x, w, bias, y, nullptr, ws, ws_bytes, (hipStream_t)stream));
  return HIFIHR_OK;
}

int hifihr_conv2d_describe(int N, int H, int W, int C, int K, int R, int S, int stride, int pad, int dgrad, char* out, int cap) {
  if (!out || cap < 24 || !conv_dims_ok(N, H, W, C, K, R, S, stride, pad)) return fail(HIFIHR_EINVAL, "hifihr_conv2d_describe: bad argument");
  if (dgrad == 1) hifihr::conv_describe(conv_dgrad_geom(N, H, W, C, K, R, S, stride, pad), out, cap);
  else if (dgrad == 2) hifihr::conv_wgrad_describe(conv_geom(N, H, W, C, K, R, S, stride, pad), out, cap);
  else hifihr::conv_describe(conv_geom(N, H, W, C, K, R, S, stride, pad), out, cap);
  return HIFIHR_OK;
}

static bool pair_geoms(int N, int H, int W, int C, int stride, int K1, int R1, int pad1, int K2, int R2, int pad2, hifihr::ConvGeom* g1, hifihr::ConvGeom* g2) {
  if (!conv_dims_ok(N, H, W, C, K1, R1, R1, stride, pad1) || !conv_dims_ok(N, H, W, C, K2, R2, R2, stride, pad2) || C % 4) return false;
  *g1 = conv_geom(N, H, W, C, K1, R1, R1, stride, pad1);
  *g2 = conv_geom(N, H, W, C, K2, R2, R2, stride, pad2);
  return true;
}
int hifihr_conv2d_fwd_bnstats_pair_supported(int N, int H, int W, int C, int stride, int K1, int R1, int pad1, int K2, int R2, int pad2) {
  hifihr::ConvGeom g1, g2;
  return (pair_geoms(N, H, W, C, stride, K1, R1, pad1, K2, R2, pad2, &g1, &g2) && hifihr::conv_rows_pair_supported(g1, g2) &&
          hifihr::bgemm_nt_stats_supported(K1) && hifihr::bgemm_nt_stats_supported(K2)) ? 1 : 0;
}
int hifihr_conv2d_fwd_bnstats_pair(const float* x, const float* w1, float* y1, float* stats1, int K1, int R1, int pad1, const float* w2, float* y2,
                                   float* stats2, int K2, int R2, int pad2, int N, int H, int W, int C, int stride, void* stream) {
  hifihr::ConvGeom g1, g2;
  if (!x || !w1 || !y1 || !stats1 || !w2 || !y2 || !stats2 || !pair_geoms(N, H, W, C, stride, K1, R1, pad1, K2, R2, pad2, &g1, &g2) ||
      !hifihr_conv2d_fwd_bnstats_pair_supported(N, H, W, C, stride, K1, R1, pad1, K2, R2, pad2))
    return fail(HIFIHR_EINVAL, "hifihr_conv2d_fwd_bnstats_pair: bad argument or unsupported pair (ask hifihr_conv2d_fwd_bnstats_pair_supported)");
  const float* zeros = hifihr::conv_halo_zero_page((hipStream_t)stream);
  if (zeros == nullptr) return fail(HIFIHR_EINVAL, "hifihr_conv2d_fwd_bnstats_pair: the zero page is not available inside a capture (call once outside)");
  HIP_TRY(hifihr::launch_conv_rows_pair(g1, x, w1, y1, stats1, g2, w2, y2, stats2, zeros, (hipStream_t)stream));
  return HIFIHR_OK;
}

int hifihr_conv2d_fwd_bnstats(const float* x, const float* w, float* y, float* stats, int N, int H, int W, int C, int K, int R,
                              int S, int stride, int pad, void* ws, size_t ws_bytes, void* stream) {
  if (!x || !w || !y || !stats || !conv_dims_ok(N, H, W, C, K, R, S, stride, pad) || C % 4)
    return fail(HIFIHR_EINVAL, "hifihr_conv2d_fwd_bnstats: bad argument (C must be a multiple of 4)");
  const hifihr::ConvGeom g = conv_geom(N, H, W, C, K, R, S, stride, pad);
  HIP_TRY(hifihr::launch_conv_igemm(g, x, w, nullptr, y, stats, ws, ws_bytes, (hipStream_t)stream));
  return HIFIHR_OK;
}

int hifihr_conv2d_bwd_data(const float* dy, const float* w, float* dx, float* wt_scratch, int N, int H, int W, int C, int K,
                           int R, int S, int stride, int pad, void* ws, size_t ws_bytes, void* stream) {
  if (!dy || !w || !dx || !wt_scratch || !conv_dims_ok(N, H, W, C, K, R, S, stride, pad) || K % 4 || (K % 16 && stride != 1))
    return fail(HIFIHR_EINVAL, "hifihr_conv2d_bwd_data: bad argument (K % 4 == 0; K % 16 == 0 when stride > 1)");
  if (stride > 1 && R * S > 62 && hifihr::lpips_stem_bwd_data_supported(N, H, W, C, K, R, S, stride, pad)) {
    HIP_TRY(hifihr::launch_lpips_stem_bwd_data(dy, w, dx, N, H, W, C, K, R, S, stride, pad, (hipStream_t)stream));
    return HIFIHR_OK;
  }
  HIP_TRY(hifihr::launch_weight_transpose(w, wt_scratch, K, R * S, C, (hipStream_t)stream));
  HIP_TRY(hifihr::launch_conv_igemm(conv_dgrad_geom(N, H, W, C, K, R, S, stride, pad), dy, wt_scratch, nullptr, dx, nullptr, ws, ws_bytes, (hipStream_t)stream));
  return HIFIHR_OK;
}

int hifihr_conv2d_bwd_data_pre(const float* dy, const float* wt, float* dx, int N, int H, int W, int C, int K, int R, int S, int stride,
                               int pad, void* ws, size_t ws_bytes, void* stream) {
  if (!dy || !wt || !dx || !conv_dims_ok(N, H, W, C, K, R, S, stride, pad) || K % 4 || (K % 16 && stride != 1))
    return fail(HIFIHR_EINVAL, "hifihr_conv2d_bwd_data_pre: bad argument (K % 4 == 0; K % 16 == 0 when stride > 1)");
  HIP_TRY(hifihr::launch_conv_igemm(conv_dgrad_geom(N, H, W, C, K, R, S, stride, pad), dy, wt, nullptr, dx, nullptr, ws, ws_bytes, (hipStream_t)stream));
  return HIFIHR_OK;
}

int hifihr_conv2d_bwd_data_pre_res(const float* dy, const float* wt, const float* res, float* dx, int N, int H, int W, int C, int K, int R, int S,
                                   int stride, int pad, void* ws, size_t ws_bytes, void* stream) {
  if (!dy || !wt || !dx || !res || !conv_dims_ok(N, H, W, C, K, R, S, stride, pad) || K % 4 || (K % 16 && stride != 1))
    return fail(HIFIHR_EINVAL, "hifihr_conv2d_bwd_data_pre_res: bad argument (K % 4 == 0; K % 16 == 0 when stride > 1)");
  hifihr::ConvGeom g = conv_dgrad_geom(N, H, W, C, K, R, S, stride, pad);
  g.residual = res;
  HIP_TRY(hifihr::launch_conv_igemm(g, dy, wt, nullptr, dx, nullptr, ws, ws_bytes, (hipStream_t)stream));
  return HIFIHR_OK;
}

int hifihr_conv2d_bwd_data_pre_plus1x1_supported(int N, int H, int W, int C, int K, int R, int S, int stride, int pad) {
  if (!conv_dims_ok(N, H, W, C, K, R, S, stride, pad) || stride < 2 || K % 16 || C % 4 || R * S > 62 || pad >= R || pad >= S) return 0;
  const hifihr::ConvGeom f = conv_geom(N, H, W, C, K, R, S, stride, pad);
  if (f.OH != (H - 1) / stride + 1 || f.OW != (W - 1) / stride + 1) return 0;
  if ((long)N * f.OH * f.OW * K >= (1L << 30) || (long)C * R * S * K >= (1L << 30)) return 0;
  static const int on = hifihr::env_int("HIFIHR_DGRAD_PLUS1X1", 1);
  return on;
}

int hifihr_conv2d_bwd_data_pre_plus1x1(const float* dy, const float* wt, const float* dy2, const float* wt2, float* dx, int N, int H, int W, int C,
                                       int K, int R, int S, int stride, int pad, void* stream) {
  if (!dy || !wt || !dy2 || !wt2 || !dx || !hifihr_conv2d_bwd_data_pre_plus1x1_supported(N, H, W, C, K, R, S, stride, pad))
    return fail(HIFIHR_EINVAL, "hifihr_conv2d_bwd_data_pre_plus1x1: bad argument (see hifihr_conv2d_bwd_data_pre_plus1x1_supported)");
  hifihr::ConvGeom g = conv_dgrad_geom(N, H, W, C, K, R, S, stride, pad);
// ... 1004 lines not shown
```

hifihr_amd/csrc/hifihr_internal.h:

```cpp
#pragma once
#include <hip/hip_runtime.h>

#include <cstdint>
#include <cstdlib>
#include <stdint.h>

#include "render_math.h"

namespace hifihr {

inline int device_cus() {
  static int cus = 0;
  if (cus == 0) {
    int dev = 0;
    hipDeviceProp_t prop;
    if (hipGetDevice(&dev) == hipSuccess && hipGetDeviceProperties(&prop, dev) == hipSuccess && prop.multiProcessorCount > 0) cus = prop.multiProcessorCount;
  }
  return cus > 0 ? cus : 256;
}

static inline int env_int(const char* name, int unset) {
  const char* e = getenv(name);
  return e ? atoi(e) : unset;
}
// ... 286 lines not shown
  return __builtin_amdgcn_rcpf(1.0f + __expf(-z));
#endif
}
struct LinearArgs {
  const float *x, *W, *b;
  float *y, *z;
  const float *gamma, *beta;
  float *save_mean, *save_invstd, *running_mean, *running_var;
  float eps, momentum;
  int B, I, O, act;
};
struct LinearGrads {
  const float* dy;
  float *dz, *dW_acc, *db_acc, *dgamma_acc, *dbeta_acc, *dx;
};
constexpr int kMaxLinearGroup = 6;
struct LinearGroup {
  LinearArgs a[kMaxLinearGroup];
  int n;
};
struct LinearGradsGroup {
  LinearGrads g[kMaxLinearGroup];
};
hipError_t launch_linear_fwd_group(const LinearGroup& grp, hipStream_t st);
hipError_t launch_linear_bwd_group(const LinearGroup& grp, const LinearGradsGroup& gg, hipStream_t st);
hipError_t launch_linear_fwd(const LinearArgs& a, hipStream_t st);
hipError_t launch_linear_bwd(const LinearArgs& a, const LinearGrads& g, hipStream_t st);

hipError_t launch_se_pool(const float* x, int B, int HW, int C, float* mean_zeroed, hipStream_t st);
hipError_t launch_se_bwd_gate(const float* dy, const float* x, int B, int HW, int C, float* dgate_zeroed, hipStream_t st);
hipError_t launch_se_scale(const float* x, const float* gate, const float* add, float ascale, int B, int HW, int C, float* y, hipStream_t st);
hipError_t launch_drop_connect_add(const float* x, const float* skip, const float* u, float keep, int B, size_t per_sample, float* out,
                                   hipStream_t st);
bool se_mlp_supported(int C, int SQ);
hipError_t launch_se_mlp_fwd(float* mean_acc, const float* W1, const float* b1, const float* W2T, const float* b2, int B, int C, int SQ,
                             float* mean_out, float* z1, float* h1, float* gate, hipStream_t st);
hipError_t launch_se_mlp_bwd(float* dgate_acc, const float* gate, const float* z1, const float* h1, const float* mean, const float* W1,
                             const float* W2T, int B, int C, int SQ, float* dz2, float* dz1, float* dmean, float* dW1_acc, float* db1_acc,
                             float* dW2_acc, float* db2_acc, hipStream_t st);

hipError_t launch_wino_weight_transform(const float* w, float* U, int K, int C, int flip, hipStream_t st);
hipError_t launch_wino_input_transform(const float* x, float* V, float* Y , int N, int H, int W, int C, hipStream_t st);
struct PrepJob {
  const float* src;
  float* dst;
  int K, C, RS, kind;
};
hipError_t launch_weight_prep(const PrepJob* jobs, int njobs, int blocks_per_job, hipStream_t st);
hipError_t launch_freihand_augment(const uint32_t* img, const uint8_t* mask, const int* idx, const int* coef, int B, int H, int W,
                                   float* out_img, float* out_mask, hipStream_t st);
struct BatchStepOut {
  int root_id;
  float image_size;
  float *oroot, *ojoints_rel, *overts_rel, *ocam;
};
hipError_t launch_freihand_batch(const uint32_t* img, const uint8_t* mask, const float* Ks, const float* joints, const float* verts,
                                 const float* scales, int J, int V, const int* packed, int B, int H, int W, float* out_img, float* out_mask,
                                 long long* out_segm, float* oKs, float* oPs, float* ojoints, float* overts, float* oj2d, float* oscales,
                                 long long* oidx, const BatchStepOut& step, hipStream_t st);
size_t ho3d_workspace_bytes(int B, int out_size);
hipError_t launch_ho3d_batch(const uint32_t* img, const uint8_t* mask, const float* Ks, const float* uv21, const float* xyz21, int FH, int FW,
                             const int* packed, int B, int out_size, void* ws, float* out_img, float* out_mask, float* out_K,
                             float* out_uv, float* out_xyz, hipStream_t st);
hipError_t launch_procrustes(const float* pred, const float* gt, int B, int N, float* aligned, float* err_sum, hipStream_t st);
constexpr int kHistMaxT = 128, kFscoreMaxT = 8;
struct HistThresholds { double v[kHistMaxT]; };
struct FscoreThresholds { double v[kFscoreMaxT]; };
bool thresholds_ok(const double* thr_h, int T, bool positive);
hipError_t launch_point_error_hist(const float* pred, const float* gt, const unsigned char* vis, int n, int K, const double* thr_h, int T,
                                   int* hist, double* sum, hipStream_t st);
hipError_t launch_fscore_counts(const float* pred, const float* gt, int B, int Np, int Ng, const double* thr_h, int T, int* counts,
                                hipStream_t st);
hipError_t launch_wino_output_transform(const float* Mm, float* y, float* stats, const float* bias, int relu, int N, int H, int W, int K,
                                        hipStream_t st);
hipError_t launch_wino_dy_transform(const float* dy, float* Y, int N, int H, int W, int K, hipStream_t st);
hipError_t launch_wino_dw_transform(float* dU, float* dw, int K, int C, int clear, hipStream_t st);

struct BgemmArgs {
  const float* A; const float* B; float* C;
  int M, N, K;
  int lda, ldb, ldc;
  long sa, sb, sc;
  int batch, tiles_m, tiles_n;
  int splits, cps;
  long sc_split;
  const float* zeros = nullptr;
  int cIH = 0, cIW = 0, cC = 0, cOH = 0, cOW = 0, cR = 0, cS = 0, cStride = 1, cPad = 0;
  int co_r = 0, co_rounds = 0;
  int k_valid = 0;
  float* stats = nullptr;
};
void bgemm_describe(int tn, int M, int N, int K, char* out, int cap);
void bgemm_describe_batch(int tn, int M, int N, int K, int batch, char* out, int cap);
bool bgemm_nt_supported(int M, int N, int K);
bool bgemm_nt_fits32(long M_alloc, int N, int K);
bool bgemm_tn_supported(int M, int N, int T);
size_t bgemm_nt_workspace_bytes(int M, int N, int K, int batch);
bool bgemm_nt_stats_supported(int N);
bool conv_rows_supported(const ConvGeom& g, const float* bias);
hipError_t launch_conv_rows(const ConvGeom& g, const float* src, const float* wgt, float* dst, float* stats, const float* zeros, hipStream_t st);
bool conv_rows_pair_supported(const ConvGeom& g1, const ConvGeom& g2);
hipError_t launch_conv_rows_pair(const ConvGeom& g1, const float* src, const float* w1, float* y1, float* stats1, const ConvGeom& g2, const float* w2,
                                 float* y2, float* stats2, const float* zeros, hipStream_t st);
bool bgemm_nt_ragged_supported(int M, int N, int K);
enum class NtKernel { rows, rows_ragged, sk, ws, tile };
struct NtPlan {
  bool ok;
  NtKernel kernel;
  int M, M_alloc, N, K, batch;
  int bm, bn, loaders;
  int G;
  long per;
  size_t ws_bytes;
};
NtPlan plan_nt(int M, int M_alloc, int N, int K, int batch, bool stats);
void describe_nt(const NtPlan& p, char* out, int cap);
hipError_t launch_bgemm_nt_plan(const NtPlan& p, const float* A, const float* B, float* C, void* ws, size_t ws_bytes, hipStream_t st, float* stats_or_null);
hipError_t launch_bgemm_nt(const float* A, const float* B, float* C, int M, int N, int K, int batch, void* ws, size_t ws_bytes, hipStream_t st,
                           float* stats_or_null = nullptr, int M_alloc = 0);
int bgemm_tn_parts(int M, int N, int T, int batch);
hipError_t launch_bgemm_tn(const float* A, const float* B, float* Cparts, int M, int N, int T, int batch, int parts, hipStream_t st, int T_valid = 0);
bool bgemm_nt_tn_pair_supported(int M, int M_alloc, int N, int K, int batch, int M2, int N2, int T2, int batch2, int parts2);
hipError_t launch_bgemm_nt_tn_pair(const float* A, const float* B, float* C, int M, int M_alloc, int N, int K, int batch, const float* A2,
                                   const float* B2, float* C2parts, int M2, int N2, int T2, int batch2, int parts2, hipStream_t st, int T2_valid = 0);
hipError_t launch_wino_dw_transform_parts(const float* dU_parts, int parts, float* dw, int K, int C, hipStream_t st);
long wino4_tiles(int N, int H, int W);
long wino4_tiles_real(int N, int H, int W);
hipError_t launch_wino4_weight_transform(const float* w, float* U, int K, int C, int flip, hipStream_t st);
hipError_t launch_wino4_input_transform(const float* x, float* V, float* Y , int N, int H, int W, int C, hipStream_t st);
bool wino4_bn_supported(int C);
hipError_t launch_wino4_bn_input_transform(const float* x, float* stats, const float* gamma, const float* beta, const float* res, float* out,
                                           float* V, int N, int H, int W, int C, float eps, float momentum, float* save_mean,
                                           float* save_invstd, float* running_mean, float* running_var, hipStream_t st);
hipError_t launch_wino4_output_transform_bnred(const float* Mm, const float* x, const float* outp, const float* gadd, const float* save_mean,
                                               const float* save_invstd, const float* gamma, const float* beta, float* red, float* g, int N,
                                               int H, int W, int C, hipStream_t st);
hipError_t launch_wino4_bn_bwd_dual_transform(const float* g, const float* y, const float* save_mean, const float* save_invstd, const float* gamma,
                                              float* red, float* V, float* Y, int N, int H, int W, int K, float* dgamma_acc, float* dbeta_acc,
                                              hipStream_t st);
hipError_t launch_bn_bwd_apply(const float* g, const float* x, const float* save_mean, const float* save_invstd, const float* gamma, long M,
                               int C, float* red, float* dx, float* dgamma_acc, float* dbeta_acc, hipStream_t st);
hipError_t launch_wino4_output_transform(const float* Mm, float* y, float* stats, const float* bias, int relu, const float* mask, int N, int H, int W, int K,
                                         hipStream_t st);
hipError_t launch_wino4_dy_transform(const float* dy, float* Y, int N, int H, int W, int K, hipStream_t st);
hipError_t launch_wino4_dw_transform_parts(const float* dU_parts, int parts, float* dw, int K, int C, hipStream_t st);
struct WinoDwJob { const float* dU; float* dw; int parts, K, C; };
hipError_t launch_wino4_dw_transform_multi(const WinoDwJob* jobs, int njobs, hipStream_t st);

hipError_t launch_texpca_fwd(const float* coef, const float* basis, const float* mean, int B, int K, long n, float* out, hipStream_t st);
hipError_t launch_texpca_bwd(const float* g, const float* basis, int B, int K, long n, float* dcoef_zeroed, hipStream_t st);
size_t adam_state_bytes();
hipError_t launch_adam_counted(float* p, const float* g, float* m, float* v, size_t n, float grad_scale, float eps, float weight_decay,
                               void* state, hipStream_t st);
hipError_t launch_adam(float* p, const float* g, float* m, float* v, size_t n, float grad_scale, float lr, float beta1,
                       float beta2, float eps, float weight_decay, int step, const float* dyn, hipStream_t st);
size_t grad_guard_bytes();
size_t grad_norm_workspace_bytes(size_t n);
hipError_t launch_grad_norm(const float* g, size_t n, float grad_scale, float max_norm, void* guard, void* ws, hipStream_t st);
hipError_t launch_adam_guarded(float* p, const float* g, float* m, float* v, size_t n, float grad_scale, float lr, float beta1, float beta2,
                               float eps, float weight_decay, int step, void* state, const void* guard, hipStream_t st);

hipError_t launch_joint_terms_fwd(const float* j2d, const float* j2d_gt, const float* j3d, const float* j3d_gt, int B, int J, int mse,
                                  const float* lam3, float* out3, hipStream_t st);
hipError_t launch_joint_terms_bwd(const float* j2d, const float* j2d_gt, const float* j3d, const float* j3d_gt, int B, int J, int mse,
                                  const float* lam3, const float* gout3, float* g_j2d, float* g_j3d, hipStream_t st);

}
```

hifihr_amd/ops.py:

```python
from __future__ import annotations

import math
import os
import threading

import torch

from ._lib import get_lib, require_cuda


import os as _os

_DEBUG_SYNC = _os.environ.get("HIFIHR_DEBUG_SYNC", "0") == "1"


class _Profile:

    def __init__(self):
        self.on = False
        self.events = []
        self.last_render = None
        self.conv_log = []

    def enable(self):
# ... 491 lines not shown
        self.on = bool(enabled) and _BRANCHES and like.is_cuda
        self.like, self.name, self.inputs = like, name, inputs

    def __enter__(self):
        if not self.on:
            return self
        dev = self.like.device
        key = (dev, self.name)
        st = side_branch._streams.get(key)
        if st is None:
            st = side_branch._streams[key] = torch.cuda.Stream(device=dev)
            BRANCH_STREAMS.add(st.cuda_stream)
        self.cur, self.side = torch.cuda.current_stream(dev), st
        side_branch._home[key] = self.cur
        side_branch._pending.add(key)
        st.wait_stream(self.cur)
        for t in (self.like,) + tuple(self.inputs):
            if torch.is_tensor(t) and t.is_cuda:
                t.record_stream(st)
        self._ctx = torch.cuda.stream(st)
        self._ctx.__enter__()
        return self

    def __exit__(self, *exc):
        if self.on:
            self._ctx.__exit__(*exc)
            if exc[0] is not None:
                self.cur.wait_stream(self.side)
        return False

    def join(self, *outs):
        if self.on:
            for t in outs:
                if torch.is_tensor(t) and t.is_cuda:
                    t.record_stream(self.cur)
            self.cur.wait_stream(self.side)

    @staticmethod
    def join_pending():
        for key in list(side_branch._pending):
            st, home = side_branch._streams.get(key), side_branch._home.get(key)
            if st is not None:
                cur = torch.cuda.current_stream(key[0])
                cur.wait_stream(st)
                if home is not None and home != cur:
                    home.wait_stream(st)
        side_branch._pending.clear()


_BRANCHES = True
_STEM_REDUCE_Y = os.environ.get("HIFIHR_STEM_REDUCE_Y", "1") != "0"
_GEMM_PAIR = os.environ.get("HIFIHR_GEMM_PAIR", "1") != "0"
_C64_PAIR = os.environ.get("HIFIHR_C64_PAIR", "1") != "0"
BRANCH_STREAMS = set()
_CONV_WS_BYTES = {}
_SCRATCH = {}
_RETIRED_SCRATCH = []


def _scratch(key, numel, device, zeroed=False, alloc=None):
    t = _SCRATCH.get(key)
    if t is None or t.numel() < numel:
        if t is not None:
            _RETIRED_SCRATCH.append(t)
        t = (torch.zeros if zeroed else torch.empty)(alloc or numel, device=device, dtype=torch.float32)
        _SCRATCH[key] = t
    return t


def _conv_ws(lib, device, geom, bwd):
    key = (geom, bwd)
    nb = _CONV_WS_BYTES.get(key)
    if nb is None:
        nb = lib.wino_gemm_workspace_bytes(*geom[1:]) if geom[0] == "wino" else lib.conv2d_workspace_bytes(*geom, bwd)
        _CONV_WS_BYTES[key] = nb
    if nb == 0:
        return None
    h = torch.cuda.current_stream(device).cuda_stream
    return _scratch(("conv_ws", device, h if h in BRANCH_STREAMS else 0), (nb + 3) // 4, device, zeroed=True,
                    alloc=max(nb, 32 << 20) // 4 + 64)


def _wgrad_slabs(device, nbytes):
    return _scratch(("wgrad_slabs", device, torch.cuda.current_stream(device).cuda_stream), (nbytes + 3) // 4, device)


def _wino_scratch(device, name, numel):
    return _scratch(("wino", device, name), numel, device)


class _PrecisionStack(threading.local):
    def __init__(self):
        self.stack = ["fast"]


_CONV_PRECISION = _PrecisionStack()
_WINOGRAD_ENV = os.environ.get("HIFIHR_WINOGRAD", "1") != "0"


class conv_precision:

    def __init__(self, mode):
        if mode not in ("fast", "reference"):
            raise ValueError(f"conv_precision: 'fast' or 'reference', not {mode!r}")
        self.mode = mode

    def __enter__(self):
        _CONV_PRECISION.stack.append(self.mode)
        return self

    def __exit__(self, *exc):
        _CONV_PRECISION.stack.pop()
        return False


def _wino_allowed():
    return _WINOGRAD_ENV and _CONV_PRECISION.stack[-1] != "reference"


def _wino_ok(C, K, R, S, stride, pad, allowed=None):
    if not (_wino_allowed() if allowed is None else allowed):
        return False
    if not (R == 3 and S == 3 and stride == 1 and pad == 1 and C % 32 == 0 and K % 32 == 0):
        return False
    if C >= 128 and K >= 128:
        return True
    return min(C, K) >= 64 and max(C, K) >= 128


def _wino2_fused_ok(lib, N, H, W, C, K, R, S, stride, pad, allowed=None, device=None):
    return (R == 3 and S == 3 and stride == 1 and pad == 1 and C == 64 and K == 64 and (_wino_allowed() if allowed is None else allowed)
            and lib.conv3x3_c64_wino_supported(N, H, W, C, K) and lib.zero_page_ready(device))


_WINO_TILE = {}


def _wino_tile(lib, N, H, W, C, K):
    key = (N, H, W, C, K)
    e = _WINO_TILE.get(key)
    if e is None:
        m = lib.wino_tile(N, H, W, C, K)
        e = (m, (m + 2) ** 2, lib.wino_tiles(N, H, W, m))
        _WINO_TILE[key] = e
    return e


class _WeightPrep:

    def __init__(self):
        self.entries = {}
        self.table, self.njobs, self.dirty, self.active, self.served = None, 0, False, False, set()
        self._retired = []

    def get(self, w, wk, kind):
        if not isinstance(w, torch.nn.Parameter) or wk.data_ptr() != w.data_ptr():
            return None
        key = (w.data_ptr(), kind)
        e = self.entries.get(key)
        if e is None:
            K, C, R, S = w.shape
            if kind == 5:
                n = K * ((C + 3) // 4 * 4) * R * S
            else:
                n = K * C * R * S if kind == 0 else K * C * (16 if kind in (1, 2) else 36)
            self.entries[key] = [w, K, C, R * S, kind, torch.empty(n, device=w.device, dtype=torch.float32)]
            self.dirty = True
            return None
        return e[5] if (self.active and key in self.served) else None

    def begin(self):
        live = {k: e for k, e in self.entries.items() if e[0].data_ptr() == k[0]}
        if len(live) != len(self.entries):
            self.entries, self.dirty = live, True
        if not self.entries:
            return
        lib = get_lib()
        if self.dirty:
            jobs = [(e[0], e[5], e[1], e[2], e[3], e[4]) for e in self.entries.values()]
            if self.table is not None:
                self._retired.append((self.table, [e[5] for e in self.entries.values()]))
            self.table, self.njobs = lib.prep_jobs(jobs, jobs[0][0].device), len(jobs)
            self.served, self.dirty = set(self.entries.keys()), False
        PROFILE.bracket("weight_prep", lambda: lib.weight_prep(self.table, self.njobs, 256))
        self.active = True

    def end(self):
        self.active = False


_WEIGHT_PREP = _WeightPrep()


class _DeferredDw:

    def __init__(self):
        self.on = os.environ.get("HIFIHR_DEFER_DW", "1") != "0"
        self.active = False
        self.jobs = []
        self.halo = []
        self.pending = set()
        self.early = os.environ.get("HIFIHR_DEFER_EARLY", "1") != "0"
        self.side, self.home, self._streams, self.n_early = None, None, {}, 0

    def wants(self, w, direct):
        if self.side is not None and w.grad is not None and w.grad.data_ptr() in self.pending:
            torch.cuda.current_stream(self.side.device).wait_stream(self.side)
        return (self.on and self.active and direct and not _ASYNC_WGRAD.active and getattr(w, "_hifihr_grad_ready", None) is None
                and (w.grad is None or w.grad.data_ptr() not in self.pending))

    def add(self, dU, parts, tgt, K, C):
        self.jobs.append((dU, int(parts), tgt, int(K), int(C), torch.cuda.current_stream(tgt.device).cuda_stream))
        self.pending.add(tgt.data_ptr())

    def add_halo(self, slabs, nslab, tgt):
        self.halo.append((slabs, int(nslab), tgt, torch.cuda.current_stream(tgt.device).cuda_stream))
        self.pending.add(tgt.data_ptr())

    def clear(self):
        self.jobs.clear(); self.halo.clear(); self.pending.clear()
        if self.side is not None:
            if not torch.cuda.is_current_stream_capturing():
                torch.cuda.current_stream(self.side.device).wait_stream(self.side)
            self.side = None

    def _run(self, jobs, halo):
        lib = get_lib() if (jobs or halo) else None
        if halo:
            PROFILE.bracket("halo_reduce_multi", lambda: lib.conv_halo_wgrad_reduce_multi([h[:3] for h in halo]))
        if jobs:
            PROFILE.bracket("wino_dw_multi", lambda: lib.wino4_dw_transform_multi([j[:5] for j in jobs]))

    def flush(self):
        jobs, self.jobs = self.jobs, []
        halo, self.halo = self.halo, []
        self.pending.clear()
        self._run(jobs, halo)
        if self.side is not None:
            cur = torch.cuda.current_stream(self.side.device)
            cur.wait_stream(self.side)
            if self.home is not None and self.home != cur:
                self.home.wait_stream(self.side)
            self.side = None

    def flush_early(self, device):
        if not (self.early and self.active and self.side is None and (self.jobs or self.halo)):
            return
        cur = torch.cuda.current_stream(device)
        h = cur.cuda_stream
        jobs, halo = [j for j in self.jobs if j[5] == h], [j for j in self.halo if j[3] == h]
        if not (jobs or halo):
            return
        self.jobs, self.halo = [j for j in self.jobs if j[5] != h], [j for j in self.halo if j[3] != h]
        st = self._streams.get(device)
        if st is None:
            st = self._streams[device] = torch.cuda.Stream(device=device)
        st.wait_stream(cur)
        with torch.cuda.stream(st):
            self._run(jobs, halo)
        self.side, self.home, self.n_early = st, cur, self.n_early + 1


_DEFER_DW = _DeferredDw()


class _AsyncWgrad:

    def __init__(self):
        self.active, self.streams, self.refs = False, {}, []

    def stream(self, device):
        s = self.streams.get(device)
        if s is None:
            s = torch.cuda.Stream(device=device)
            self.streams[device] = s
        return s

    def launch(self, device, fn, keep):
        cur = torch.cuda.current_stream(device)
        side = self.stream(device)
        side.wait_stream(cur)
        with torch.cuda.stream(side):
            fn()
        self.refs.append(keep)

    def join(self):
        for dev, s in self.streams.items():
            torch.cuda.current_stream(dev).wait_stream(s)
        self.refs.clear()


_ASYNC_WGRAD = _AsyncWgrad()


class prepared_weights:

    def __init__(self, async_wgrad=False):
        self.async_wgrad = bool(async_wgrad)

    def __enter__(self):
        if torch.cuda.is_available() and torch.cuda.is_current_stream_capturing():
            side_branch._pending.clear()
        else:
            side_branch.join_pending()
        _WEIGHT_PREP.begin()
        _DEFER_DW.clear()
        _DEFER_DW.active = True
        _ASYNC_WGRAD.active = self.async_wgrad and not torch.cuda.is_current_stream_capturing()
        return self

    def __exit__(self, *exc):
        _WEIGHT_PREP.end()
        _DEFER_DW.active = False
        if exc[0] is None:
            _DEFER_DW.flush()
        else:
            _DEFER_DW.clear()
        side_branch.join_pending()
        if _ASYNC_WGRAD.active:
            _ASYNC_WGRAD.active = False
            _ASYNC_WGRAD.join()
        return False


def _wino_conv(lib, x, w_krsc, y, stats, N, H, W, C, K, flip, keep_v=False, bias=None, act=0, U=None, dy_out=None, tile=None, mask=None,
               pair=None):
    dev = x.device
    m, P, T = tile if tile is not None else _wino_tile(lib, N, H, W, C, K)
    prepared = U is not None
    if not prepared:
        U = _wino_scratch(dev, "U", P * K * C)
    V = torch.empty(P * T * C, device=dev, dtype=torch.float32) if keep_v else _wino_scratch(dev, "V", P * T * C)
    M = _wino_scratch(dev, "M", P * T * K)
    ws = _conv_ws(lib, dev, ("wino", N, H, W, C, K, m), False)
    if PROFILE.on:
        PROFILE.conv_log.append((("wino", N, H, W, K, C, m), "gemm-pair") if pair is not None else (("wino", N, H, W, C, K, m), "gemm"))
    if not prepared:
        lib.wino_weight_transform(w_krsc, U, K, C, flip, m)
    if dy_out is not None:
        lib.wino_input_dy_transform(x, V, dy_out, N, H, W, C, m)
    else:
        lib.wino_input_transform(x, V, N, H, W, C, m)
    if pair is not None:
        vx, dU, parts = pair
        lib.wino4_bwd_gemm_pair(V, U, M, vx, dy_out, dU, N, H, W, K, C, parts)
    else:
        lib.wino_gemm(V, U, M, N, H, W, C, K, ws=ws, m=m)
    lib.wino_output_transform(M, y, stats, N, H, W, K, bias=bias, act=act, m=m, mask=mask)
    return V if keep_v else None


def _direct_grad(p, fmt=None):
    return getattr(p, "_hifihr_direct_grad", False) and p.grad is not None and (fmt is None or p.grad.is_contiguous(memory_format=fmt))


def _grad_target(p, like, fmt=None):
    if _direct_grad(p, fmt):
        return p.grad, None
    t = torch.zeros(like.shape, device=like.device) if fmt is None else torch.zeros_like(like, memory_format=fmt)
    return t, t


def _stem_c3_wgrad(lib, geom, w, w3, x, gy):
    N, H, W, C, K, R, S, stride, pad = geom
    if PROFILE.on:
        PROFILE.conv_log.append((geom, "wgrad"))
    nslab = lib.conv2d_wgrad_workspace_bytes(N, H, W, C, K, R, S, stride, pad)
    if w3.shape[1] == 3 and lib.conv2d_bwd_weight_c3_supported(N, H, W, K, R, S, stride, pad):
        tgt, dw = _grad_target(w, w3, _CL)
        PROFILE.bracket("conv_wgrad", lambda: lib.conv2d_bwd_weight_c3(x, gy, tgt, N, H, W, K, R, S, stride, pad, _wgrad_slabs(gy.device, nslab)))
    else:
        dw4 = torch.zeros((K, C, R, S), device=gy.device).contiguous(memory_format=_CL)
        PROFILE.bracket("conv_wgrad", lambda: lib.conv2d_bwd_weight(x, gy, dw4, N, H, W, C, K, R, S, stride, pad,
                                                                     ws=_wgrad_slabs(gy.device, nslab) if nslab else None))
        if not _direct_grad(w, _CL):
            return dw4[:, :w3.shape[1]].contiguous(memory_format=_CL)
        w.grad.add_(dw4[:, :w3.shape[1]])
        dw = None
    if dw is None:
        _grad_ready(w)
    return dw


def _wino_u_bwd(lib, wk, U2, dev, C, K, m):
    if U2 is None:
        wt = _wino_scratch(dev, "wt", wk.numel())
        lib.weight_transpose(wk, wt, K, 9, C)
        U2 = _wino_scratch(dev, "U", (m + 2) ** 2 * K * C)
        lib.wino_weight_transform(wt, U2, C, K, 1, m)
    return U2


def _wino_wgrad_slabs(lib, w, direct, own, dev, N, H, W, C, K, m):
    parts = lib.wino_wgrad_parts(N, H, W, C, K, m)
    if parts == 0:
        return _scratch(("wino", dev, "dU", 16 * K * C), 16 * K * C, dev, zeroed=True), 0, False
    defer = m == 4 and _DEFER_DW.wants(w, direct)
    dU = _wino_scratch(dev, ("dUp", w.data_ptr()) if (own or defer) else "dUp", parts * (m + 2) ** 2 * K * C)
    return dU, parts, defer


def _wino_wgrad_tail(lib, V, Yt, slabs, tgt, N, H, W, C, K, m, paired):
    dU, parts, defer = slabs
    if not paired:
        if parts > 0:
            lib.wino_wgrad_gemm_parts(V, Yt, dU, N, H, W, C, K, parts, m)
        else:
            lib.wino_wgrad_gemm(V, Yt, dU, N, H, W, C, K)
    if defer:
        _DEFER_DW.add(dU, parts, tgt, K, C)
    elif parts > 0:
        lib.wino_dw_transform_parts(dU, parts, tgt, K, C, m)
    else:
        lib.wino_dw_transform(dU, tgt, K, C, clear=True)


def _bias_relu_bwd(lib, gy, y, b, need_b, relu, grad_premasked, K):
    db_t, db_ret = _grad_target(b, b) if (b is not None and need_b) else (None, None)
    if relu and grad_premasked:
        assert db_t is None, "grad_premasked needs a frozen bias (the bias gradient comes out of the masking pass)"
    elif relu:
        g = torch.empty_like(gy, memory_format=_CL)
        PROFILE.bracket("bias_relu_bwd", lambda: lib.bias_relu_bwd(gy, y, gy.numel() // K, K, g, db_t))
        gy = g
    elif db_t is not None:
        raise NotImplementedError("gradient of a conv bias without ReLU")
    if db_t is not None and db_ret is None:
        _grad_ready(b)
    return gy, db_ret


def _wino_dgrad(lib, gy, wk, w, geom, tile, U2, mask, yt, pair, g_fork):
    N, H, W, C, K = geom[:5]
    dx = torch.empty((N, C, H, W), device=gy.device, dtype=torch.float32, memory_format=_CL)

    def run():
        U = _wino_u_bwd(lib, wk, U2, gy.device, C, K, tile[0])
        _wino_conv(lib, gy, None, dx, None, N, H, W, K, C, 1, U=U, dy_out=yt, tile=tile, mask=mask,
                   pair=None if pair is None else (pair[0], pair[1][0], pair[1][1]))
    PROFILE.bracket("conv_dgrad_wino", run)
    return dx if g_fork is None else dx + g_fork


def _c64_dgrad(lib, gy, x, wk, w, geom, g_fork, pair):
    N, H, W = geom[:3]
    dx = torch.empty_like(x, memory_format=_CL)
    U2 = _WEIGHT_PREP.get(w, wk, 2)
    if not pair:
        if PROFILE.on:
            PROFILE.conv_log.append((geom, "dgrad-wino2"))
        if g_fork is not None:
            PROFILE.bracket("conv_dgrad", lambda: lib.conv3x3_c64_wino_res(gy, U2, g_fork, dx, N, H, W))
        else:
            PROFILE.bracket("conv_dgrad", lambda: lib.conv3x3_c64_wino(gy, U2, None, False, dx, None, N, H, W))
        return dx, None
    tgt, dw = _grad_target(w, wk, _CL)
    if PROFILE.on:
        PROFILE.conv_log.append((geom, "c64-pair"))
    nslab = lib.conv2d_wgrad_workspace_bytes(*geom)
    if nslab and dw is None and _DEFER_DW.wants(w, True):
        own = _wino_scratch(gy.device, ("c64slabs", w.data_ptr()), (nslab + 3) // 4)
        box = []
        PROFILE.bracket("conv_dgrad", lambda: box.append(lib.conv3x3_c64_bwd_pair_slabs(gy, U2, g_fork, dx, x, own, N, H, W)))
        _DEFER_DW.add_halo(own, box[-1], tgt)
    else:
        slabs = _wgrad_slabs(gy.device, nslab) if nslab else None
        PROFILE.bracket("conv_dgrad", lambda: lib.conv3x3_c64_bwd_pair(gy, U2, g_fork, dx, x, tgt, N, H, W, ws=slabs))
    return dx, dw


# ... 1356 lines not shown
```

hifihr_amd/optim.py:

```python
from __future__ import annotations

import torch

from ._lib import get_lib, require_cuda


class FlatParams:

    def __init__(self, module: torch.nn.Module, align: int = 64):
        self.params = [p for p in module.parameters() if p.requires_grad]
        dev = self.params[0].device
        self.offsets = []
        off = 0
        for p in self.params:
            self.offsets.append(off)
            off += (p.numel() + align - 1) // align * align
        self.numel = off
        self.flat = torch.zeros(off, dtype=torch.float32, device=dev)
        self.grad = torch.zeros(off, dtype=torch.float32, device=dev)
        for p, o in zip(self.params, self.offsets):
            p.data = self._view(self.flat, p, o, init=p.data)
            p.grad = self._view(self.grad, p, o)
            p._hifihr_direct_grad = True

    @staticmethod
    def _view(buf, p, o, init=None):
        n = p.numel()
        seg = buf[o:o + n]
        if p.dim() == 4 and p.is_contiguous(memory_format=torch.channels_last) and not p.is_contiguous():
            K, C, R, S = p.shape
            v = seg.view(K, R, S, C).permute(0, 3, 1, 2)
        else:
            v = seg.view(p.shape)
        if init is not None:
            v.copy_(init)
        return v

    def zero_grad(self):
        self.grad.zero_()
        for p, o in zip(self.params, self.offsets):
            if p.grad is None or p.grad.data_ptr() != self.grad.data_ptr() + 4 * o:
                p.grad = self._view(self.grad, p, o)

    def param_count(self):
        return sum(p.numel() for p in self.params)


class FusedAdam(torch.optim.Optimizer):

    def __init__(self, flat: FlatParams, lr=1e-3, betas=(0.9, 0.999), eps=1e-8, weight_decay=0.0, grad_scale=1.0, max_grad_norm=None):
        if max_grad_norm is not None:
            ok = isinstance(max_grad_norm, (int, float)) and not isinstance(max_grad_norm, bool) and max_grad_norm > 0
            if not ok:
                raise ValueError(f"max_grad_norm must be None (off) or a number > 0 (inf = guard only), got {max_grad_norm!r}")
            max_grad_norm = float(max_grad_norm)
        self.max_grad_norm = max_grad_norm
        self.flatp = flat
        super().__init__([flat.flat], dict(lr=lr, betas=betas, eps=eps, weight_decay=weight_decay))
        self.exp_avg = torch.zeros_like(flat.flat)
        self.exp_avg_sq = torch.zeros_like(flat.flat)
        self._step_count = 0
        self.grad_scale = grad_scale
        self._lib = None
        self.graph_mode = False
        self._state = None
        self._state_sig = None
        self._prepared = False
        self._guard = self._guard_ws = None
        if max_grad_norm is not None:
            self._lib = get_lib()
            self._guard, self._guard_ws = self._lib.grad_guard_alloc(flat.flat.numel(), flat.flat.device)

    @property
    def step_count(self):
        return self._step_count

    @step_count.setter
    def step_count(self, value):
        self._step_count = int(value)
        self._state_sig = None
        self._prepared = False

    def enable_graph_mode(self):
        self.graph_mode = True
        self._prepared = False
        self._state_sig = None
        require_cuda(self.flatp.flat)
        if self._lib is None:
            self._lib = get_lib()
        if self._state is None:
            self._state = torch.zeros(int(self._lib.c.hifihr_adam_state_bytes()), dtype=torch.uint8, device=self.flatp.flat.device)

    def disable_graph_mode(self):
        self.graph_mode = False
        self._prepared = False
        self._state_sig = None

    def note_step_done(self):
        self._prepared = False

    def prepare_step(self):
        g = self.param_groups[0]
        if self._prepared:
            self._step_count -= 1
            self._state_sig = None
        self._prepared = True
        self._step_count += 1
        b1, b2 = g["betas"]
        want = (float(g["lr"]), float(b1), float(b2), self._step_count - 1)
        if self._state_sig != want:
            self._state.copy_(self._lib.adam_state_image(*want))
        self._state_sig = (want[0], want[1], want[2], self._step_count)

    def zero_grad(self, set_to_none: bool = False):
        self.flatp.zero_grad()

    @torch.no_grad()
    def step(self, closure=None):
        if self._lib is None:
            self._lib = get_lib()
        require_cuda(self.flatp.flat)
        g = self.param_groups[0]
        if self.graph_mode:
            capturing = self.flatp.flat.is_cuda and torch.cuda.is_current_stream_capturing()
            if not capturing:
                if not self._prepared:
                    raise RuntimeError("FusedAdam.step() in graph mode without prepare_step(): the device-side step counter / the uploaded "
                                       "bias corrections would be those of the previous step")
                self._prepared = False
            if self.max_grad_norm is not None:
                self._lib.grad_norm(self.flatp.grad, self.grad_scale, self.max_grad_norm, self._guard, self._guard_ws)
                self._lib.adam_step_guarded(self.flatp.flat, self.flatp.grad, self.exp_avg, self.exp_avg_sq, self.grad_scale, 0.0, 0.0, 0.0,
                                            g["eps"], g["weight_decay"], 0, self._state, self._guard)
                return
            self._lib.adam_step_counted(self.flatp.flat, self.flatp.grad, self.exp_avg, self.exp_avg_sq, self.grad_scale, g["eps"],
                                        g["weight_decay"], self._state)
            return
        self._step_count += 1
        from .ops import PROFILE
        if self.max_grad_norm is not None:
            def guarded():
                self._lib.grad_norm(self.flatp.grad, self.grad_scale, self.max_grad_norm, self._guard, self._guard_ws)
                self._lib.adam_step_guarded(self.flatp.flat, self.flatp.grad, self.exp_avg, self.exp_avg_sq, self.grad_scale, g["lr"],
                                            g["betas"][0], g["betas"][1], g["eps"], g["weight_decay"], self.step_count, None, self._guard)
            PROFILE.bracket("adam", guarded)
            return
        PROFILE.bracket("adam", lambda: self._lib.adam_step(self.flatp.flat, self.flatp.grad, self.exp_avg, self.exp_avg_sq,
                                                            self.grad_scale, g["lr"], g["betas"][0], g["betas"][1], g["eps"],
                                                            g["weight_decay"], self.step_count))

    def grad_stats(self):
        if self._guard is None:
            return None
        return self._lib.grad_guard_unpack(self._guard.cpu().numpy().tobytes())

    def guard_snapshot(self):
        return None if self._guard is None else self._guard.clone()

    def guard_restore(self, snap):
        if snap is not None:
            self._guard.copy_(snap)

    def state_dict(self):
        return {"step": self.step_count, "exp_avg": self.exp_avg, "exp_avg_sq": self.exp_avg_sq,
                "param_groups": [{k: v for k, v in g.items() if k != "params"} for g in self.param_groups]}

    def load_state_dict(self, sd):
        self.step_count = int(sd["step"])
        self.exp_avg.copy_(sd["exp_avg"]); self.exp_avg_sq.copy_(sd["exp_avg_sq"])
        for g, s in zip(self.param_groups, sd["param_groups"]):
            g.update(s)
```

hifihr_amd/traineval.py:

```python
from __future__ import annotations

import torch
import torch.nn.functional as F


def proj_func(xyz, K):
    uv = (xyz.unsqueeze(2) * K.unsqueeze(1)).sum(3)
    return uv[:, :, :2] / uv[:, :, 2:3]


def trans_proj_j2d(outputs, Ks, root_xyz=None, which_joints="joints"):
    j3d = outputs[which_joints]
    if root_xyz is not None:
        j3d = j3d + root_xyz
    return proj_func(j3d, Ks)


_HO3D_TO_FREI = [0, 13, 14, 15, 16, 1, 2, 3, 17, 4, 5, 6, 18, 10, 11, 12, 19, 7, 8, 9, 20]


def HO3D2Frei(ho3d_joints):
    return ho3d_joints[:, _HO3D_TO_FREI]


def Frei2HO3D(frei_joints):
    inv = [0] * 21
    for frei, ho in enumerate(_HO3D_TO_FREI):
        inv[ho] = frei
    return frei_joints[:, inv]


_RHD_TO_FREI = [0, 4, 3, 2, 1, 8, 7, 6, 5, 12, 11, 10, 9, 16, 15, 14, 13, 20, 19, 18, 17]


def RHD2Frei(rhd_joints):
    return rhd_joints[:, _RHD_TO_FREI]


def data_dic(sample, dat_name, set_name, args, device="cuda", image_size=224):
    ex = {}
    to = lambda t: t.to(device, non_blocking=True)
    if dat_name == "FreiHand":
        training = "training" in set_name
        g = lambda k: sample["trans_" + k] if ("trans_" + k) in sample and (training or k in ("images", "Ks")) else sample.get(k)
        ex["imgs"] = to(g("images"))
        Ks = to(g("Ks"))
        if "scales" in sample:
            ex["scales"] = to(sample["scales"].float())
        ex["idxs"] = to(sample["idxs"])
        joints, verts, masks = g("joints"), g("verts"), g("masks")
    elif dat_name == "HO3D":
        ex["imgs"] = F.interpolate(to(sample["img_crop"]), (image_size, image_size))
        flip = torch.tensor([1.0, -1.0, -1.0], device=device)
        Ks = to(sample["K_crop"]) * flip.view(1, 1, 3)
        if "root_xyz" in sample:
            ex["root_xyz"] = to(sample["root_xyz"])
        if "uv21_crop" in sample:
            ex["j2d_gt"] = HO3D2Frei(to(sample["uv21_crop"].float()))
        joints = HO3D2Frei(to(sample["xyz21"])) * flip.view(1, 1, 3) if "xyz21" in sample else None
        verts, masks = None, sample.get("hand_mask_crop")
        if masks is not None and masks.shape[-1] != image_size:
            masks = F.interpolate(to(masks), (image_size, image_size))
    elif dat_name == "RHD":
        ex["imgs"] = to(sample["img_crop"])
        Ks = to(sample["K_crop"])
        if "uv21_crop" in sample:
            ex["j2d_gt"] = RHD2Frei(to(sample["uv21_crop"]))
        joints = RHD2Frei(to(sample["xyz21"])) if "xyz21" in sample else None
        if "keypoint_scale" in sample:
            ex["keypoint_scale"] = to(sample["keypoint_scale"])
            ex["scales"] = ex["keypoint_scale"]
        if "uv_vis" in sample:
            ex["uv_vis"] = RHD2Frei(to(sample["uv_vis"]))
        if "open_2dj" in sample:
            ex["open_2dj"], ex["open_2dj_con"] = to(sample["open_2dj_crop"]), to(sample["open_2dj_con"])
        verts, masks = None, None
    else:
        raise NotImplementedError(f"dat_name='{dat_name}': FreiHand, HO3D and RHD are built (Obman / Dart need their datasets)")
    ex["Ks"] = Ks
    ex["Ps"] = torch.cat([Ks, torch.zeros_like(Ks[:, :, :1])], dim=2)
    if joints is not None:
        ex["joints"] = to(joints)
        if dat_name == "FreiHand":
            ex["j2d_gt"] = proj_func(ex["joints"], Ks)
    if verts is not None:
        ex["verts"] = to(verts)
    if masks is not None:
        ex["masks"] = to(masks)
        ex["segms_gt"] = ex["masks"][:, 0].long()
    return ex


_BACKWARD_SEED = {}


def _backward_seed(loss):
    seed = _BACKWARD_SEED.get(loss.device)
    if seed is None or seed.dtype != loss.dtype or seed.shape != loss.shape:
        if torch.cuda.is_current_stream_capturing():
            return None
        seed = _BACKWARD_SEED[loss.device] = torch.ones_like(loss)
    return seed


def _prime_for_capture(device):
    from ._lib import get_lib
    dev = torch.device(device)
    if dev not in _BACKWARD_SEED:
        _BACKWARD_SEED[dev] = torch.ones((), device=dev, dtype=torch.float32)
    get_lib().zero_page_ready(dev)


def forward_backward(model, loss_func, optimizer, examples, args, dat_name="FreiHand"):
    from .ops import prepared_weights
    dp = torch.distributed.is_available() and torch.distributed.is_initialized() and torch.distributed.get_world_size() > 1
    with prepared_weights(async_wgrad=not dp):
        return _forward_backward(model, loss_func, optimizer, examples, args, dat_name)


def _forward_backward(model, loss_func, optimizer, examples, args, dat_name):
    pre = dat_name != "HO3D" and "joints_rel" in examples and "root_xyz" in examples
    root_xyz = examples["root_xyz"] if pre else examples["joints"][:, args.ROOT, :].unsqueeze(1)
    if pre and "verts" in examples and "verts_rel" not in examples:
        examples = dict(examples, verts_rel=examples["verts"] - root_xyz)
    same_size = getattr(model, "image_size", None) in (None, examples["imgs"].shape[-1])
    kw = {"cam_ndc": examples["cam_ndc"]} if ("cam_ndc" in examples and getattr(model, "accepts_cam_ndc", False) and same_size) else {}
    outputs = model(dat_name, True, examples["imgs"], Ks=examples["Ps"], root_xyz=root_xyz, **kw)
    ex = dict(examples)
    if pre:
        ex["joints"] = examples["joints_rel"]
        if "verts_rel" in examples:
            ex["verts"] = examples["verts_rel"]
    elif dat_name != "HO3D":
        ex["joints"] = examples["joints"] - root_xyz
        if "verts" in examples:
            ex["verts"] = examples["verts"] - root_xyz
    if any(k in args.losses for k in ("joint_2d", "bone_direc")):
        outputs["j2d"] = trans_proj_j2d(outputs, examples["Ks"], root_xyz=root_xyz)
    loss_dic = loss_func(ex, outputs, args.losses, dat_name, args)
    missing = [k for k in args.losses if k not in loss_dic]
    if missing:
        raise KeyError(f"loss terms {missing} were requested but not produced for {dat_name}: their inputs are absent from the model outputs / examples")
    if hasattr(loss_func, "total"):
        loss = loss_func.total(loss_dic, args.losses)
    else:
        terms = [loss_dic[k] for k in args.losses]
        loss = terms[0] if len(terms) == 1 else torch.stack(terms).sum()
    loss_dic["loss"] = loss
    optimizer.zero_grad(set_to_none=True)
    loss.backward(_backward_seed(loss))
    return loss, loss_dic


def train_step(model, loss_func, optimizer, examples, args, dat_name="FreiHand", backward_hook=None):
    loss, loss_dic = forward_backward(model, loss_func, optimizer, examples, args, dat_name)
    if backward_hook is not None:
        backward_hook()
    optimizer.step()
    return loss, loss_dic


def _check_step_terms(static, examples):
    missing = [k for k in ("root_xyz", "joints_rel", "verts_rel", "cam_ndc") if k in static and k not in examples]
    if missing:
        raise KeyError(f"load_batch: the captured step was built on a batch that carries {missing}; pass batches from the same source "
                       f"(batch_examples(..., root_id=args.ROOT)) or capture the step on a batch without them")


def _injected_capture_failure():
    import os
    r = os.environ.get("HIFIHR_TEST_FAIL_CAPTURE_RANK")
    if r is not None and torch.distributed.is_available() and torch.distributed.is_initialized() and torch.distributed.get_rank() == int(r):
        raise RuntimeError("injected capture failure (HIFIHR_TEST_FAIL_CAPTURE_RANK)")


class GraphedTrainStep:

    def __init__(self, model, loss_func, optimizer, examples, args, dat_name="FreiHand", warmup=3, reducer=None):
        self.model, self.loss_func, self.opt, self.args, self.dat_name = model, loss_func, optimizer, args, dat_name
        self.reducer = reducer
        self.static = {k: (v.clone() if torch.is_tensor(v) else v) for k, v in examples.items()}
        split = reducer is not None
        flat = optimizer.flatp
        snap = (flat.flat.clone(), optimizer.exp_avg.clone(), optimizer.exp_avg_sq.clone(), optimizer.step_count,
                [b.clone() for b in model.buffers()], optimizer.guard_snapshot())
        if split:
            reducer.pause_hooks(True)
        else:
            optimizer.enable_graph_mode()
        try:
            _injected_capture_failure()
            _prime_for_capture(flat.flat.device)
            side = torch.cuda.Stream()
            side.wait_stream(torch.cuda.current_stream())
            with torch.cuda.stream(side):
                for _ in range(warmup):
                    if split:
                        forward_backward(model, loss_func, optimizer, self.static, args, dat_name)
                        optimizer.step()
                    else:
                        optimizer.prepare_step()
                        train_step(model, loss_func, optimizer, self.static, args, dat_name)
            torch.cuda.current_stream().wait_stream(side)
            torch.cuda.synchronize()
            self.graph = torch.cuda.CUDAGraph()
            if split:
                with torch.cuda.graph(self.graph, capture_error_mode="thread_local"):
                    self.loss, self.loss_dic = forward_backward(model, loss_func, optimizer, self.static, args, dat_name)
            else:
                optimizer.prepare_step()
                with torch.cuda.graph(self.graph):
                    self.loss, self.loss_dic = train_step(model, loss_func, optimizer, self.static, args, dat_name)
        except BaseException:
            if split:
                reducer.pause_hooks(False)
            else:
                optimizer.disable_graph_mode()
            self._restore(snap)
            raise
        self._restore(snap)

    def _restore(self, snap):
        flat_w, m, v, step, bufs, guard = snap
        with torch.no_grad():
            self.opt.flatp.flat.copy_(flat_w)
            self.opt.exp_avg.copy_(m)
            self.opt.exp_avg_sq.copy_(v)
            self.opt.guard_restore(guard)
            for b, s in zip(self.model.buffers(), bufs):
                b.copy_(s)
        self.opt.step_count = step
        torch.cuda.synchronize()

    def release(self):
        if self.reducer is not None:
            self.reducer.pause_hooks(False)
        else:
            self.opt.disable_graph_mode()

    def load_batch(self, examples):
        _check_step_terms(self.static, examples)
        for k, v in examples.items():
            if torch.is_tensor(v):
                self.static[k].copy_(v, non_blocking=True)

    def __call__(self):
        if self.reducer is not None:
            self.graph.replay()
            self.reducer.all_reduce_flat()
            self.opt.step()
        else:
            self.opt.prepare_step()
            self.graph.replay()
            self.opt.note_step_done()
        return self.loss, self.loss_dic


class SegmentedGraphedTrainStep:

    def __init__(self, model, loss_func, optimizer, examples, args, reducer, dat_name="FreiHand", warmup=3):
        enc = getattr(getattr(model, "base_encoder", None), "encoder1", None)
        if enc is None or not hasattr(enc, "model") or not hasattr(enc.model, "layer3"):
            raise NotImplementedError("segmented backward is built for the ResNet trunks")
        self.model, self.loss_func, self.opt, self.args, self.dat_name, self.reducer = model, loss_func, optimizer, args, dat_name, reducer
        self.static = {k: (v.clone() if torch.is_tensor(v) else v) for k, v in examples.items()}
        flat = optimizer.flatp
        idx = {id(p): i for i, p in enumerate(flat.params)}

        def span(mods):
            ids = [idx[id(p)] for m in mods for p in m.parameters() if id(p) in idx]
            return (min(ids), max(ids) + 1) if ids else (0, 0)
        trunk = enc.model
        lo3, hi3 = span([trunk.layer3])
        lo4, hi4 = span([trunk.layer4])
        n = len(flat.params)
        self.ranges = [(hi4, n), (lo4, hi4), (lo3, hi3), (0, lo3)]
        assert 0 < lo3 <= hi3 == lo4 <= hi4 <= n, (lo3, hi3, lo4, hi4, n)
        snap = (flat.flat.clone(), optimizer.exp_avg.clone(), optimizer.exp_avg_sq.clone(), optimizer.step_count,
                [b.clone() for b in model.buffers()], optimizer.guard_snapshot())
        reducer.pause_hooks(True)
        self._enc = enc
        self._scope = None
        try:
            _injected_capture_failure()
            _prime_for_capture(flat.flat.device)
            side = torch.cuda.Stream()
            side.wait_stream(torch.cuda.current_stream())
            with torch.cuda.stream(side):
                for _ in range(warmup):
                    self._eager_segmented()
                    optimizer.step()
            torch.cuda.current_stream().wait_stream(side)
            torch.cuda.synchronize()
            pool = torch.cuda.graph_pool_handle()
            self.graphs = []
            stages = self._stages()
            for stage in stages:
                g = torch.cuda.CUDAGraph()
                with torch.cuda.graph(g, pool=pool, capture_error_mode="thread_local"):
                    stage()
                self.graphs.append(g)
        except BaseException:
            reducer.pause_hooks(False)
            enc.segment_cut = None
            if self._scope is not None:
                self._scope.__exit__(None, None, None)
                self._scope = None
            self._restore(snap)
            raise
        enc.segment_cut = None
        self._restore(snap)

    def _stages(self):
        from .ops import _WEIGHT_PREP, prepared_weights

        def fwd():
            self._b = {}

            def cut(name, t):
                leaf = t.detach().requires_grad_(True)
                self._b[name] = (t, leaf)
                return leaf
            self._enc.segment_cut = cut
            self._scope = prepared_weights(async_wgrad=False)
            self._scope.__enter__()
            root_xyz = self.static["joints"][:, self.args.ROOT, :].unsqueeze(1)
            self.loss, self.loss_dic = _forward_only(self.model, self.loss_func, self.opt, self.static, self.args, self.dat_name, root_xyz)

        def bwd_heads():
            self.loss.backward()

        def bwd(name):
            def run():
                t, leaf = self._b[name]
                t.backward(leaf.grad)
            return run

        def bwd_last():
            bwd("layer2")()
            self._scope.__exit__(None, None, None)
            self._scope = None
        return [fwd, bwd_heads, bwd("layer4"), bwd("layer3"), bwd_last]

    def _eager_segmented(self):
        for stage in self._stages():
            stage()

    def _restore(self, snap):
        GraphedTrainStep._restore(self, snap)

    def release(self):
        self.reducer.pause_hooks(False)

    def load_batch(self, examples):
        _check_step_terms(self.static, examples)
        for k, v in examples.items():
            if torch.is_tensor(v):
                self.static[k].copy_(v, non_blocking=True)

    def __call__(self):
        self.graphs[0].replay()
        handles = []
        for g, (lo, hi) in zip(self.graphs[1:], self.ranges):
            g.replay()
            h = self.reducer.all_reduce_params_async(lo, hi)
            if h is not None:
                handles.append(h)
        for h in handles:
            h.wait()
        self.opt.step()
        return self.loss, self.loss_dic


def _forward_only(model, loss_func, optimizer, examples, args, dat_name, root_xyz):
    outputs = model(dat_name, True, examples["imgs"], Ks=examples["Ps"], root_xyz=root_xyz)
    ex = dict(examples)
    if dat_name != "HO3D":
        ex["joints"] = examples["joints"] - root_xyz
        if "verts" in examples:
            ex["verts"] = examples["verts"] - root_xyz
    if any(k in args.losses for k in ("joint_2d", "bone_direc")):
        outputs["j2d"] = trans_proj_j2d(outputs, examples["Ks"], root_xyz=root_xyz)
    loss_dic = loss_func(ex, outputs, args.losses, dat_name, args)
    missing = [k for k in args.losses if k not in loss_dic]
    if missing:
        raise KeyError(f"loss terms {missing} were requested but not produced for {dat_name}")
    terms = [loss_dic[k] for k in args.losses]
    loss = terms[0] if len(terms) == 1 else torch.stack(terms).sum()
    loss_dic["loss"] = loss
    optimizer.zero_grad(set_to_none=True)
    return loss, loss_dic
```

include/hifihr.h:

```cpp
#ifndef HIFIHR_H
#define HIFIHR_H

#include <stddef.h>
#include <stdint.h>

#ifdef __cplusplus
extern "C" {
#endif

#define HIFIHR_OK 0
#define HIFIHR_EINVAL (-1)
#define HIFIHR_EHIP (-2)
#define HIFIHR_ENOMEM (-3)

#define HIFIHR_MANO_NV 778
#define HIFIHR_MANO_NF 1538
#define HIFIHR_MANO_NJ 16

int hifihr_version(void);
const char* hifihr_last_error(void);
int hifihr_device_count(void);

typedef struct hifihr_mano hifihr_mano_t;

int hifihr_mano_create(hifihr_mano_t** out, const float* v_template_h, const float* shapedirs_h,
                       const float* posedirs_h, const float* j_regressor_h, const float* weights_h,
                       const float* hands_components_h, const float* hands_mean_h);
int hifihr_mano_destroy(hifihr_mano_t* h);

int hifihr_mano_lbs_fwd(const hifihr_mano_t* h, const float* pose_d, const float* beta_d, int B,
                        float* verts_d, float* jtr_d, float* saved_vposed_d, void* stream);

int hifihr_mano_lbs_bwd(const hifihr_mano_t* h, const float* pose_d, const float* beta_d,
                        const float* saved_vposed_d, const float* gverts_d, const float* gjtr_d, int B,
                        float* gpose_d, float* gbeta_d, void* stream);

int hifihr_mano_joints_fwd(const hifihr_mano_t* h, const float* verts_d, int B, int root_id,
                           float* joints_rel_d, float* verts_rel_d, float* root_d, void* stream);
int hifihr_mano_joints_bwd(const hifihr_mano_t* h, const float* gjoints_rel_d, const float* gverts_rel_d,
                           const float* groot_d, int B, int root_id, float* gverts_d, void* stream);

int hifihr_mano_full_fwd(const hifihr_mano_t* h, const float* pose_d, const float* beta_d, int B, int root_id,
                         const float* root_xyz_d, float* verts_d, float* joints_rel_d, float* verts_rel_d, float* verts_cam_d,
                         float* root_d, float* saved_vposed_d, void* stream);
int hifihr_mano_full_bwd(const hifihr_mano_t* h, const float* pose_d, const float* beta_d, const float* saved_vposed_d,
                         const float* gjoints_rel_d, const float* gverts_rel_d, const float* gverts_cam_d,
                         const float* groot_d, const float* gpose_add_d, const float* gbeta_add_d, int B, int root_id,
                         float* gpose_d, float* gbeta_d, void* stream);

typedef struct hifihr_lbs hifihr_lbs_t;

int hifihr_lbs_create(hifihr_lbs_t** out, int V, int J, int S, const float* v_template_h, const float* shapedirs_h,
                      const float* j_regressor_h, const float* weights_h, const int* parents_h);
int hifihr_lbs_destroy(hifihr_lbs_t* h);

int hifihr_lbs_fwd(const hifihr_lbs_t* h, const float* theta_d, const float* beta_d, int B, float* verts_d, float* joints_d, void* stream);

int hifihr_lbs_bwd(const hifihr_lbs_t* h, const float* theta_d, const float* beta_d, const float* gverts_d, const float* gjoints_d,
                   int B, float* scratch_zeroed_d, float* gtheta_d, float* gbeta_zeroed_d, void* stream);

typedef struct hifihr_renderer hifihr_renderer_t;


int hifihr_renderer_create(hifihr_renderer_t** out, const int32_t* faces_h, int V, int F, int image_size, int aa,
                           const float* ambient3, const float* mat_diffuse3, const float* specular3, float shininess,
                           const float* background3);
int hifihr_renderer_set_light_mode(hifihr_renderer_t* h, int point_lights);
int hifihr_renderer_destroy(hifihr_renderer_t* h);
size_t hifihr_render_workspace_bytes(const hifihr_renderer_t* h, int B);

int hifihr_render_fwd(const hifihr_renderer_t* h, const float* verts_d, const float* vcolors_d, int vcolors_batched,
                      const float* cam_d, const float* light_color_d, const float* light_dir_d, int B, float* rgba_d,
                      int32_t* face_id_d, void* workspace_d, void* stream);

int hifihr_render_bwd(const hifihr_renderer_t* h, const float* verts_d, const float* cam_d, const float* light_color_d,
                      const float* light_dir_d, const int32_t* face_id_d, const float* grad_rgba_d, int B,
                      float* gverts_d, float* gvcolors_d, float* glight_color_d, float* glight_dir_d, void* workspace_d,
                      void* stream);
int hifihr_renderer_set_uv(hifihr_renderer_t* h, const int32_t* faces_uvs_h, const float* verts_uvs_h, int n_uv);
size_t hifihr_render_uv_scratch_bytes(const hifihr_renderer_t* h, int B);
int hifihr_render_fwd_uv(const hifihr_renderer_t* h, const float* verts_d, const float* maps_d, int TH, int TW, const float* cam_d,
                         const float* light_color_d, const float* light_dir_d, int B, float* rgba_d, int32_t* face_id_d,
                         float* texels_scratch_d, void* ws_d, void* stream);
int hifihr_render_bwd_uv(const hifihr_renderer_t* h, const float* verts_d, const float* maps_d, int TH, int TW, const float* cam_d,
                         const float* light_color_d, const float* light_dir_d, const int32_t* face_id_d, const float* grad_rgba_d, int B,
                         const float* texels_scratch_d, float* gtexels_scratch_d, float* gverts_d, float* gmaps_acc_d,
                         float* glight_color_d, float* glight_dir_d, void* ws_d, void* stream);

size_t hifihr_soft_sil_workspace_bytes(const hifihr_renderer_t* h, int B);
int hifihr_soft_sil_fwd(const hifihr_renderer_t* h, const float* verts_d, const float* cam_d, int B, float sigma, float blur_radius,
                        float* alpha_d, float* neglog_d, void* ws_d, void* stream);
int hifihr_soft_sil_bwd(const hifihr_renderer_t* h, const float* verts_d, const float* cam_d, const float* neglog_d, const float* galpha_d,
                        int B, float sigma, float blur_radius, float* gverts_d, void* ws_d, void* stream);
int hifihr_soft_sil_loss_fwd(const float* alpha_d, const void* mask_d, int mask_i64, int B, int HW, float lam_sil, float lam_iou,
                             double* sums_d, float* out_d, void* stream);
int hifihr_soft_sil_loss_bwd(const float* alpha_d, const void* mask_d, int mask_i64, const double* sums_d, const float* gout_d, int B, int HW,
                             float lam_sil, float lam_iou, float* galpha_d, void* stream);

typedef struct hifihr_mesh_topology hifihr_mesh_topology_t;
hifihr_mesh_topology_t* hifihr_mesh_topology_create(const int32_t* faces_host, int F, int V);
int hifihr_mesh_topology_destroy(hifihr_mesh_topology_t* h);
int hifihr_mesh_topology_counts(const hifihr_mesh_topology_t* h, int* V, int* E, int* Q);
size_t hifihr_mesh_reg_partial_floats(const hifihr_mesh_topology_t* h, int B);
int hifihr_mesh_reg_fwd(const hifihr_mesh_topology_t* h, const float* verts_d, int B, float lam_lap, float lam_nc, float* unit_d,
                        float* partial_d, float* out_d, void* stream);
int hifihr_mesh_reg_bwd(const hifihr_mesh_topology_t* h, const float* verts_d, const float* unit_d, const float* gout_d, int B,
                        float lam_lap, float lam_nc, float* gverts_d, void* stream);

void hifihr_chamfer_geometry(int* queries_per_workgroup, int* tile_points);
size_t hifihr_chamfer_workspace_bytes(int B, int N, int M);
int hifihr_chamfer_fwd(const float* x_d, const float* y_d, int B, int N, int M, float w_xy, float w_yx, int32_t* idx_xy_d, int32_t* idx_yx_d,
                       double* min_xy_d, double* min_yx_d, double* sums_d, float* out_d, void* ws_d, void* stream);
int hifihr_chamfer_bwd(const float* x_d, const float* y_d, const int32_t* idx_xy_d, const int32_t* idx_yx_d, const float* gout_d, int B, int N,
                       int M, float w_xy, float w_yx, float* gx_d , float* gy_d , void* stream);

int hifihr_texture_pca_fwd(const float* coef_d, const float* basis_d, const float* mean_d , int B, int K, long n,
                           float* tex_d, void* stream);
int hifihr_texture_pca_bwd(const float* gtex_d, const float* basis_d, int B, int K, long n, float* dcoef_zeroed_d, void* stream);

typedef struct hifihr_comm hifihr_comm;
typedef struct { char bytes[128]; } hifihr_comm_uid;
const char* hifihr_comm_last_error(void);
int hifihr_comm_get_unique_id(hifihr_comm_uid* out);
int hifihr_comm_init(hifihr_comm** out, int rank, int world, const hifihr_comm_uid* uid);
int hifihr_comm_allreduce_f32(hifihr_comm* comm, float* buf_d , size_t n, void* stream);
int hifihr_comm_broadcast_f32(hifihr_comm* comm, float* buf_d, size_t n, int root, void* stream);
int hifihr_comm_destroy(hifihr_comm* comm);

int hifihr_adam_step(float* params_d, const float* grads_d, float* exp_avg_d, float* exp_avg_sq_d, size_t n,
                     float grad_scale, float lr, float beta1, float beta2, float eps, float weight_decay, int step,
                     void* stream);
size_t hifihr_adam_state_bytes(void);
int hifihr_adam_step_counted(float* params_d, const float* grads_d, float* exp_avg_d, float* exp_avg_sq_d, size_t n, float grad_scale,
                             float eps, float weight_decay, void* state_d, void* stream);
int hifihr_adam_step_dyn(float* params_d, const float* grads_d, float* exp_avg_d, float* exp_avg_sq_d, size_t n,
                         float grad_scale, float beta1, float beta2, float eps, float weight_decay, const float* dyn_d,
                         void* stream);

size_t hifihr_grad_guard_bytes(void);
size_t hifihr_grad_norm_workspace_bytes(size_t n);
int hifihr_grad_norm(const float* grads_d, size_t n, float grad_scale, float max_norm, void* guard_d, void* ws_d, void* stream);
int hifihr_adam_step_guarded(float* params_d, const float* grads_d, float* exp_avg_d, float* exp_avg_sq_d, size_t n, float grad_scale,
                             float lr, float beta1, float beta2, float eps, float weight_decay, int step, void* state_d,
                             const void* guard_d, void* stream);

size_t hifihr_conv2d_workspace_bytes(int N, int H, int W, int C, int K, int R, int S, int stride, int pad, int bwd_data);
int hifihr_conv2d_fwd(const float* x_d, const float* w_d, const float* bias_d , int act, float* y_d, int N,
                      int H, int W, int C, int K, int R, int S, int stride, int pad, void* ws_d, size_t ws_bytes, void* stream);
int hifihr_bias_relu_bwd(const float* dy_d, const float* y_d, long M, int C, float* g_d, float* db_acc_d ,
                         void* stream);
int hifihr_light_split_fwd(const float* lights_d, int B, float* colors_d, float* directions_d, void* stream);
int hifihr_light_split_bwd(const float* lights_d, const float* gcolors_d, const float* gdirections_d, int B, float* glights_d,
                           void* stream);
int hifihr_conv2d_bwd_data(const float* dy_d, const float* w_d, float* dx_d, float* wt_scratch_d, int N, int H, int W, int C,
                           int K, int R, int S, int stride, int pad, void* ws_d, size_t ws_bytes, void* stream);
int hifihr_conv2d_bwd_weight(const float* x_d, const float* dy_d, float* dw_d, int N, int H, int W, int C, int K, int R, int S,
                             int stride, int pad, void* stream);
size_t hifihr_conv2d_wgrad_workspace_bytes(int N, int H, int W, int C, int K, int R, int S, int stride, int pad);
int hifihr_conv2d_bwd_weight_ws(const float* x_d, const float* dy_d, float* dw_accumulate_d, int N, int H, int W, int C, int K, int R, int S,
                                int stride, int pad, void* ws_d, size_t ws_bytes, void* stream);
int hifihr_conv2d_bwd_weight_c3_supported(int N, int H, int W, int K, int R, int S, int stride, int pad);
int hifihr_conv2d_bwd_weight_c3(const float* x4_d, const float* dy_d, float* dw3_d, int N, int H, int W, int K, int R, int S, int stride,
                                int pad, void* ws_d, size_t ws_bytes, void* stream);
int hifihr_wino_tile(int N, int H, int W, int C, int K);
long hifihr_wino_tiles(int N, int H, int W, int m);
long hifihr_wino_tiles_computed(int N, int H, int W, int m);
size_t hifihr_wino_gemm_workspace_bytes(int N, int H, int W, int C, int K, int m);
int hifihr_wino_wgrad_parts(int N, int H, int W, int C, int K, int m);
int hifihr_wino_weight_transform(const float* w_d, float* u_d, int K, int C, int flip, int m, void* stream);
int hifihr_wino_input_transform(const float* x_d, float* v_d, int N, int H, int W, int C, int m, void* stream);
int hifihr_wino_dy_transform(const float* dy_d, float* yt_d, int N, int H, int W, int K, int m, void* stream);
int hifihr_wino_input_dy_transform(const float* dy_d, float* v_d, float* yt_d, int N, int H, int W, int K, int m, void* stream);
int hifihr_wino_gemm(const float* v_d, const float* u_d, float* m_d, int N, int H, int W, int C, int K, int m, void* ws_d, size_t ws_bytes,
                     void* stream);
int hifihr_wino_output_transform(const float* m_d, float* y_d, float* stats_d , int N, int H, int W, int K, int m, void* stream);
int hifihr_wino_output_transform_act(const float* m_d, float* y_d, const float* bias_d , int act, int N, int H, int W, int K,
                                     int m, void* stream);
int hifihr_wino_output_transform_mask(const float* m_d, float* y_d, const float* mask_d, int N, int H, int W, int K, int m, void* stream);
int hifihr_wino_wgrad_gemm_parts(const float* v_d, const float* yt_d, float* du_parts_d, int N, int H, int W, int C, int K, int parts, int m,
                                 void* stream);
int hifihr_wino_dw_transform_parts(const float* du_parts_d, int parts, float* dw_acc_d, int K, int C, int m, void* stream);
int hifihr_wino_wgrad_gemm(const float* v_d, const float* yt_d, float* du_zeroed_d, int N, int H, int W, int C, int K, void* stream);
int hifihr_wino_dw_transform(float* du_d, float* dw_acc_d, int K, int C, int clear_du ,
                             void* stream);
int hifihr_conv3x3_c64_wino_supported(int N, int H, int W, int C, int K);
int hifihr_zero_page_ready(void* stream);
int hifihr_conv3x3_c64_wino(const float* x_d, const float* u_d, const float* bias_d , int relu, float* y_d,
                            float* stats_d , int N, int H, int W, void* stream);
int hifihr_conv3x3_c64_wino_res(const float* x_d, const float* u_d, const float* res_d, float* y_d, int N, int H, int W, void* stream);
int hifihr_conv3x3_c64_bwd_pair_supported(int N, int H, int W);
int hifihr_conv3x3_c64_bwd_pair(const float* dy_d, const float* u_bwd_d, const float* res_d , float* dx_d, const float* x_d,
                                float* dw_d, void* ws_d, size_t ws_bytes, int N, int H, int W, void* stream);
int hifihr_conv3x3_c64_bwd_pair_slabs(const float* dy_d, const float* u_bwd_d, const float* res_d , float* dx_d, const float* x_d,
                                      void* slabs_d, size_t slab_bytes, int N, int H, int W, int* nslab , void* stream);
typedef struct hifihr_halo_reduce_job {
  const float* slabs_d;
  float* dw_acc_d;
  int nslab;
} hifihr_halo_reduce_job;
int hifihr_conv_halo_wgrad_reduce_multi(const hifihr_halo_reduce_job* jobs , int njobs, void* stream);
int hifihr_wino_bn_input_supported(int C, int m);
int hifihr_wino_bn_input_transform(const float* x_d, float* stats_d, const float* gamma_d, const float* beta_d, const float* residual_d,
                                   float* out_d, float* v_d, int N, int H, int W, int C, int m, float eps, float momentum,
                                   float* save_mean_d, float* save_invstd_d, float* running_mean_d, float* running_var_d, void* stream);
int hifihr_wino_output_transform_bnred(const float* m_d, const float* x_d, const float* out_d , const float* gadd_d ,
                                       const float* save_mean_d, const float* save_invstd_d, const float* gamma_d, const float* beta_d,
                                       float* red_d, float* g_d, int N, int H, int W, int C, int m, void* stream);
int hifihr_wino_bn_bwd_dual_transform(const float* g_d, const float* y_d, const float* save_mean_d, const float* save_invstd_d,
                                      const float* gamma_d, float* red_d, float* v_d, float* yt_d, int N, int H, int W, int K, int m,
                                      float* dgamma_acc_d, float* dbeta_acc_d, void* stream);
int hifihr_bn_bwd_apply(const float* g_d, const float* x_d, const float* save_mean_d, const float* save_invstd_d, const float* gamma_d, long M,
                        int C, float* red_d, float* dx_d, float* dgamma_acc_d, float* dbeta_acc_d, void* stream);
int hifihr_wino4_bwd_gemm_pair_supported(int N, int H, int W, int C, int K);
int hifihr_wino4_bwd_gemm_pair(const float* V2_d, const float* U2_d, float* M2_d, const float* Vx_d, const float* Yt_d, float* dU_parts_d,
                               int N, int H, int W, int C, int K, int parts, void* stream);
typedef struct hifihr_wino_dw_job {
  const float* du_parts_d;
  float* dw_acc_d;
  int parts, K, C;
} hifihr_wino_dw_job;
int hifihr_wino4_dw_transform_multi(const hifihr_wino_dw_job* jobs, int njobs, void* stream);
size_t hifihr_bgemm_nt_workspace_bytes(int M, int N, int K, int batch);
int hifihr_bgemm_nt(const float* a_d, const float* b_d, float* c_d, int M, int N, int K, int batch,
                    void* ws_d , size_t ws_bytes, void* stream);
int hifihr_bgemm_tn_parts(int M, int N, int T, int batch);
int hifihr_bgemm_describe(int tn, int M, int N, int K_or_T, int batch, char* out, int cap);
int hifihr_bgemm_tn(const float* a_d, const float* b_d, float* c_parts_d, int M, int N, int T, int batch, int parts, void* stream);
int hifihr_weight_transpose(const float* w_d, float* wt_d, int K, int RS, int C, void* stream);
int hifihr_conv2d_bwd_data_pre(const float* dy_d, const float* wt_d, float* dx_d, int N, int H, int W, int C, int K, int R, int S,
                               int stride, int pad, void* ws_d, size_t ws_bytes, void* stream);
int hifihr_conv2d_bwd_data_pre_res(const float* dy_d, const float* wt_d, const float* res_d, float* dx_d, int N, int H, int W, int C, int K,
                                   int R, int S, int stride, int pad, void* ws_d, size_t ws_bytes, void* stream);
int hifihr_conv2d_bwd_data_pre_plus1x1_supported(int N, int H, int W, int C, int K, int R, int S, int stride, int pad);
int hifihr_conv2d_bwd_data_pre_plus1x1(const float* dy_d, const float* wt_d, const float* dy2_d, const float* wt2_d, float* dx_d, int N, int H,
                                       int W, int C, int K, int R, int S, int stride, int pad, void* stream);
int hifihr_conv2d_bwd_weight_plus1x1_supported(int N, int H, int W, int C, int K, int R, int S, int stride, int pad);
int hifihr_conv2d_bwd_weight_plus1x1(const float* x_d, const float* dy_d, float* dw_d, const float* dy2_d, float* dw2_d, int N, int H, int W,
                                     int C, int K, int R, int S, int stride, int pad, void* stream);
typedef struct hifihr_prep_job {
  const float* src;
  float* dst;
  int K, C, RS, kind;
} hifihr_prep_job;
int hifihr_weight_prep(const hifihr_prep_job* jobs_d, int njobs, int blocks_per_job, void* stream);

int hifihr_conv2d_describe(int N, int H, int W, int C, int K, int R, int S, int stride, int pad, int direction, char* out, int cap);

int hifihr_conv2d_fwd_bnstats(const float* x_d, const float* w_d, float* y_d, float* stats_d, int N, int H, int W, int C, int K,
                              int R, int S, int stride, int pad, void* ws_d, size_t ws_bytes, void* stream);
int hifihr_conv2d_fwd_bnstats_pair_supported(int N, int H, int W, int C, int stride, int K1, int R1, int pad1, int K2, int R2, int pad2);
int hifihr_conv2d_fwd_bnstats_pair(const float* x_d, const float* w1_d, float* y1_d, float* stats1_d, int K1, int R1, int pad1, const float* w2_d,
                                   float* y2_d, float* stats2_d, int K2, int R2, int pad2, int N, int H, int W, int C, int stride, void* stream);

int hifihr_bn_stats_floats(int C);
int hifihr_bn_stats(const float* x_d, long M, int C, float* stats_d, void* stream);
int hifihr_bn_act_fwd(const float* x_d, float* stats_d , const float* gamma_d, const float* beta_d,
                      const float* residual_d , int act, long M, int C, float eps, float momentum, float* y_d,
                      float* save_mean_d, float* save_invstd_d, float* running_mean_d, float* running_var_d, void* stream);
int hifihr_bn_act_eval(const float* x_d, const float* running_mean_d, const float* running_var_d, const float* gamma_d, const float* beta_d,
                       const float* residual_d , int act, long M, int C, float eps, float* y_d, void* stream);
int hifihr_bn_act_bwd(const float* dy_d, const float* y_d , const float* x_d, const float* save_mean_d,
                      const float* save_invstd_d, const float* gamma_d, const float* beta_d , int act, long M, int C,
                      float* red_scratch_d, float* dx_d, float* dres_d, float* dgamma_acc_d, float* dbeta_acc_d, void* stream);

int hifihr_bn_relu_maxpool_supported(int N, int H, int W, int C);
int hifihr_bn_relu_maxpool_fwd(const float* x_d, float* stats_d, const float* gamma_d, const float* beta_d, int N, int H, int W, int C,
                               float eps, float momentum, float* pooled_d, unsigned char* tap_d, float* save_mean_d, float* save_invstd_d,
                               float* running_mean_d, float* running_var_d, void* stream);
int hifihr_bn_relu_maxpool_bwd(const float* pooled_grad_d, const unsigned char* tap_d, const float* x_d, const float* save_mean_d,
                               const float* save_invstd_d, const float* gamma_d, const float* beta_d, int N, int H, int W, int C,
                               float* red_scratch_d, float* dx_d, float* dgamma_acc_d, float* dbeta_acc_d, void* stream);
int hifihr_bn_relu_maxpool_bwd_y(const float* pooled_grad_d, const float* pooled_d, const unsigned char* tap_d, const float* x_d,
                                 const float* save_mean_d, const float* save_invstd_d, const float* gamma_d, const float* beta_d, int N, int H, int W,
                                 int C, float* red_scratch_d, float* dx_d, float* dgamma_acc_d, float* dbeta_acc_d, void* stream);

int hifihr_dwconv2d_fwd(const float* x_d, const float* w_d, float* y_d, float* stats_d , int N, int H, int W, int C,
                        int OH, int OW, int K, int stride, int pad_top, int pad_left, void* stream);
int hifihr_dwconv2d_bwd_data(const float* dy_d, const float* w_d, float* dx_d, int N, int H, int W, int C, int OH, int OW, int K,
                             int stride, int pad_top, int pad_left, void* stream);
int hifihr_dwconv2d_bwd_weight(const float* x_d, const float* dy_d, float* dw_d, int N, int H, int W, int C, int OH, int OW,
                               int K, int stride, int pad_top, int pad_left, void* stream);
int hifihr_dwconv2d_fwd_bnswish(const float* x_d, const float* mean_d, const float* invstd_d, const float* gamma_d, const float* beta_d,
                                const float* w_d, float* y_d, float* stats_d , int N, int H, int W, int C, int OH, int OW,
                                int K, int stride, int pad_top, int pad_left, void* stream);
int hifihr_dwconv2d_bwd_weight_bnswish(const float* x_d, const float* mean_d, const float* invstd_d, const float* gamma_d,
                                       const float* beta_d, const float* dy_d, float* dw_d, int N, int H, int W, int C, int OH, int OW,
                                       int K, int stride, int pad_top, int pad_left, void* stream);
int hifihr_bn_finalize_fwd(float* stats_d, long M, int C, float eps, float momentum, float* save_mean_d, float* save_invstd_d,
                           float* running_mean_d , float* running_var_d , void* stream);

// ... 133 lines not shown
```

Before: 6705 images/sec.

## Fuse Winograd weight-gradient reduction with Adam update and weight re-transform

Deferred Winograd-domain weight-gradient jobs are routed to the optimizer. A new multi-job kernel sums the dU partials, applies the inverse transform to get dW, runs the Adam update in place, and writes the refreshed Winograd-transformed weights U and Ut in the same pass. The main Adam step then skips the fused parameter ranges through a range-excluding kernel. This removes the separate dW materialization, the Adam read of those gradients, and the separate weight-transform preparation pass. The cost is more bookkeeping to track weight-prep staleness and graph-capture state, and the fused path only runs in single-GPU graph mode without gradient clipping.

After: 6703 images/sec, median of 2. About the same (-0.0%).

```diff
diff --git a/hifihr_amd/_lib.py b/hifihr_amd/_lib.py
--- a/hifihr_amd/_lib.py
+++ b/hifihr_amd/_lib.py
@@ -250,6 +250,10 @@
         c.hifihr_adam_state_bytes.restype = c_size_t
         c.hifihr_adam_state_bytes.argtypes = []
         c.hifihr_adam_step_counted.argtypes = [_c_float_p, _c_float_p, _c_float_p, _c_float_p, c_size_t, c_float, c_float, c_float, c_void_p, c_void_p]
+        c.hifihr_adam_max_ranges.argtypes = []
+        c.hifihr_adam_step_counted_ranges.argtypes = [_c_float_p, _c_float_p, _c_float_p, _c_float_p, c_size_t, c_float, c_float, c_float, c_void_p,
+                                                      c_void_p, c_int, c_void_p]
+        c.hifihr_wino4_step_multi.argtypes = [c_void_p, c_int, c_float, c_float, c_float, c_void_p, c_void_p]
         c.hifihr_grad_guard_bytes.restype = c_size_t
         c.hifihr_grad_guard_bytes.argtypes = []
         c.hifihr_grad_norm_workspace_bytes.restype = c_size_t
@@ -1007,6 +1011,30 @@
         self.check(self.c.hifihr_adam_step_counted(_fp(p), _fp(g), _fp(m), _fp(v), c_size_t(n), c_float(grad_scale), c_float(eps),
                                                    c_float(weight_decay), c_void_p(state.data_ptr()), _stream_of(p)), "hifihr_adam_step_counted")
 
+    def adam_step_counted_ranges(self, p, g, m, v, grad_scale, eps, weight_decay, state, excluded):
+        import struct
+        n = p.numel()
+        assert state.dtype == torch.uint8 and state.numel() == int(self.c.hifihr_adam_state_bytes()) and state.device == p.device
+        raw = b"".join(struct.pack("<QQ", int(b), int(e)) for b, e in excluded)
+        buf = ctypes.create_string_buffer(raw, len(raw)) if excluded else None
+        self.check(self.c.hifihr_adam_step_counted_ranges(_fp(p), _fp(g), _fp(m), _fp(v), c_size_t(n), c_float(grad_scale), c_float(eps),
+                                                          c_float(weight_decay), c_void_p(state.data_ptr()),
+                                                          ctypes.cast(buf, c_void_p) if excluded else c_void_p(0), len(excluded), _stream_of(p)),
+                   "hifihr_adam_step_counted_ranges")
+
+    def wino4_step_multi(self, jobs, grad_scale, eps, weight_decay, state):
+        import struct
+        ptr = lambda t: 0 if t is None else t.data_ptr()
+        if jobs is None:
+            self.check(self.c.hifihr_wino4_step_multi(c_void_p(0), 0, c_float(grad_scale), c_float(eps), c_float(weight_decay),
+                                                      c_void_p(state.data_ptr()), c_void_p(0)), "hifihr_wino4_step_multi")
+            return
+        raw = b"".join(struct.pack("<QQQQQQQiiii", ptr(du), ptr(p), ptr(m), ptr(v), ptr(U), ptr(Ut), ptr(dw), int(parts), int(K), int(C), 0)
+                       for du, parts, p, m, v, U, Ut, dw, K, C in jobs)
+        buf = ctypes.create_string_buffer(raw, len(raw))
+        self.check(self.c.hifihr_wino4_step_multi(ctypes.cast(buf, c_void_p), len(jobs), c_float(grad_scale), c_float(eps), c_float(weight_decay),
+                                                  c_void_p(state.data_ptr()), _stream_of(jobs[0][0])), "hifihr_wino4_step_multi")
+
     def adam_step_dyn(self, p, g, m, v, grad_scale, beta1, beta2, eps, weight_decay, dyn):
         n = p.numel()
         self.check(self.c.hifihr_adam_step_dyn(_fp(p), _fp(g), _fp(m), _fp(v), c_size_t(n), c_float(grad_scale), c_float(beta1),
diff --git a/hifihr_amd/csrc/adam.hip b/hifihr_amd/csrc/adam.hip
--- a/hifihr_amd/csrc/adam.hip
+++ b/hifihr_amd/csrc/adam.hip
@@ -1,6 +1,7 @@
 #include <hip/hip_runtime.h>
 
 #include "hifihr_internal.h"
+#include "wino4_math.h"
 
 namespace hifihr {
 
@@ -179,6 +180,187 @@
   }
 }
 
+__device__ __forceinline__ void adam_update(float& p, float g, float& m, float& v, float grad_scale, float weight_decay, float beta1,
+                                            float beta2, float eps, float step_size, float inv_sqrt_bc2) {
+  const float gr = g * grad_scale + weight_decay * p;
+  m = beta1 * m + (1.f - beta1) * gr;
+  v = beta2 * v + (1.f - beta2) * gr * gr;
+  const float denom = sqrtf(v) * inv_sqrt_bc2 + eps;
+  p = p - step_size * (m / denom);
+}
+
+struct StepJob {
+  const float* dU;
+  float *p, *m, *v, *U, *Ut, *dw;
+  int parts, K, C, wg0;
+};
+constexpr int kStepMaxJobs = 16;
+struct StepJobs {
+  StepJob j[kStepMaxJobs];
+  int n;
+};
+constexpr int kStepTile = 32, kStepLd = 33;
+
+__global__ __launch_bounds__(256) void wino4_step_multi_kernel(StepJobs js, float grad_scale, float eps, float weight_decay,
+                                                              const AdamState* __restrict__ st) {
+  using namespace w4;
+  __shared__ float sc[4];
+  __shared__ float lds[kStepTile * 9 * kStepLd];
+  if (threadIdx.x == 0) {
+    const double b1 = st->beta1, b2 = st->beta2;
+    const double q1 = st->pow1 * b1, q2 = st->pow2 * b2;
+    sc[0] = (float)(st->lr / (1.0 - q1));
+    sc[1] = (float)(1.0 / sqrt(1.0 - q2));
+    sc[2] = (float)b1; sc[3] = (float)b2;
+  }
+  __syncthreads();
+  const float step_size = sc[0], inv_sqrt_bc2 = sc[1], beta1 = sc[2], beta2 = sc[3];
+  int jb = 0;
+  for (int q = 1; q < js.n; ++q)
+    if ((int)blockIdx.x >= js.j[q].wg0) jb = q;
+  const StepJob job = js.j[jb];
+  const int K = job.K, C = job.C;
+  const int wb = (int)blockIdx.x - job.wg0, kt = (K + kStepTile - 1) / kStepTile;
+  const int k0 = (wb % kt) * kStepTile, c0 = (wb / kt) * kStepTile;
+  {
+    const int cg = threadIdx.x & 7, kl = threadIdx.x >> 3;
+    const int k = k0 + kl, c = c0 + cg * 4;
+    if (k < K && c < C) {
+      const size_t plane = (size_t)K * C, slab = 36 * plane;
+      const float* du = job.dU + (size_t)k * C + c;
+      const size_t wo = (size_t)k * 9 * C + c;
+      V4 t[3][6];
+#pragma unroll
+      for (int jc = 0; jc < 6; ++jc) {
+        V4 col[6];
+#pragma unroll
+        for (int r = 0; r < 6; ++r) col[r] = ld4(du + (size_t)(r * 6 + jc) * plane);
+        for (int z = 1; z < job.parts; ++z) {
+#pragma unroll
+          for (int r = 0; r < 6; ++r) col[r] = col[r] + ld4(du + (size_t)z * slab + (size_t)(r * 6 + jc) * plane);
+        }
+        V4 o[3];
+        gt6(col, o);
+        t[0][jc] = o[0]; t[1][jc] = o[1]; t[2][jc] = o[2];
+      }
+      V4 g[3][3];
+#pragma unroll
+      for (int r = 0; r < 3; ++r) {
+        V4 o[3];
+        gt6(t[r], o);
+#pragma unroll
+        for (int s = 0; s < 3; ++s) {
+          const size_t at = wo + (size_t)(r * 3 + s) * C;
+          const V4 gr = zero4() + o[s];
+          V4 pp = ld4(job.p + at), mm = ld4(job.m + at), vv = ld4(job.v + at);
+          adam_update(pp.x, gr.x, mm.x, vv.x, grad_scale, weight_decay, beta1, beta2, eps, step_size, inv_sqrt_bc2);
+          adam_update(pp.y, gr.y, mm.y, vv.y, grad_scale, weight_decay, beta1, beta2, eps, step_size, inv_sqrt_bc2);
+          adam_update(pp.z, gr.z, mm.z, vv.z, grad_scale, weight_decay, beta1, beta2, eps, step_size, inv_sqrt_bc2);
+          adam_update(pp.w, gr.w, mm.w, vv.w, grad_scale, weight_decay, beta1, beta2, eps, step_size, inv_sqrt_bc2);
+          st4(job.p + at, pp); st4(job.m + at, mm); st4(job.v + at, vv);
+          if (job.dw != nullptr) st4(job.dw + at, gr);
+          g[r][s] = pp;
+        }
+      }
+      if (job.U != nullptr) wino4_weight_tile(g, job.U, plane, (size_t)k * C + c);
+      if (job.Ut != nullptr) {
+#pragma unroll
+        for (int q = 0; q < 9; ++q) {
+          float* d = lds + (kl * 9 + q) * kStepLd + cg * 4;
+          const V4& x = g[q / 3][q % 3];
+          d[0] = x.x; d[1] = x.y; d[2] = x.z; d[3] = x.w;
+        }
+      }
+    }
+  }
+  if (job.Ut == nullptr) return;
+  __syncthreads();
+  const int kg = threadIdx.x & 7, cl = threadIdx.x >> 3;
+  const int k = k0 + kg * 4, c = c0 + cl;
+  if (k < K && c < C) {
+    V4 g[3][3];
+#pragma unroll
+    for (int r = 0; r < 3; ++r)
+#pragma unroll
+      for (int s2 = 0; s2 < 3; ++s2) {
+        const float* p = lds + ((kg * 4) * 9 + (2 - r) * 3 + (2 - s2)) * kStepLd + cl;
+        g[r][s2] = V4{p[0], p[9 * kStepLd], p[18 * kStepLd], p[27 * kStepLd]};
+      }
+    wino4_weight_tile(g, job.Ut, (size_t)C * K, (size_t)c * K + k);
+  }
+}
+
+constexpr int kAdamMaxRanges = 16;
+struct AdamRanges {
+  size_t b[kAdamMaxRanges], e[kAdamMaxRanges];
+  int n;
+};
+__global__ __launch_bounds__(256) void adam_kernel_counted_ranges(float* __restrict__ p, const float* __restrict__ g, float* __restrict__ m,
+                                                                 float* __restrict__ v, size_t n, float grad_scale, float eps,
+                                                                 float weight_decay, AdamState* __restrict__ st, AdamRanges rg) {
+  __shared__ float sc[4];
+  int t = 0;
+  double q1 = 0.0, q2 = 0.0;
+  if (threadIdx.x == 0) {
+    t = st->step + 1;
+    const double b1 = st->beta1, b2 = st->beta2;
+    q1 = st->pow1 * b1; q2 = st->pow2 * b2;
+    sc[0] = (float)(st->lr / (1.0 - q1));
+    sc[1] = (float)(1.0 / sqrt(1.0 - q2));
+    sc[2] = (float)b1; sc[3] = (float)b2;
+  }
+  __syncthreads();
+  const float step_size = sc[0], inv_sqrt_bc2 = sc[1], beta1 = sc[2], beta2 = sc[3];
+  const size_t n4 = n / 4;
+  const size_t stride = (size_t)gridDim.x * blockDim.x;
+  float4* p4 = reinterpret_cast<float4*>(p);
+  const float4* g4 = reinterpret_cast<const float4*>(g);
+  float4* m4 = reinterpret_cast<float4*>(m);
+  float4* v4 = reinterpret_cast<float4*>(v);
+  for (size_t i = (size_t)blockIdx.x * blockDim.x + threadIdx.x; i < n4; i += stride) {
+    const size_t lo = i * 4, hi = lo + 4;
+    bool cut = false, inside = false;
+    for (int r = 0; r < rg.n; ++r) {
+      cut = cut || (rg.b[r] < hi && rg.e[r] > lo);
+      inside = inside || (rg.b[r] <= lo && rg.e[r] >= hi);
+    }
+    if (inside) continue;
+    if (!cut) {
+      float4 pp = p4[i], gg = g4[i], mm = m4[i], vv = v4[i];
+      adam_update(pp.x, gg.x, mm.x, vv.x, grad_scale, weight_decay, beta1, beta2, eps, step_size, inv_sqrt_bc2);
+      adam_update(pp.y, gg.y, mm.y, vv.y, grad_scale, weight_decay, beta1, beta2, eps, step_size, inv_sqrt_bc2);
+      adam_update(pp.z, gg.z, mm.z, vv.z, grad_scale, weight_decay, beta1, beta2, eps, step_size, inv_sqrt_bc2);
+      adam_update(pp.w, gg.w, mm.w, vv.w, grad_scale, weight_decay, beta1, beta2, eps, step_size, inv_sqrt_bc2);
+      p4[i] = pp; m4[i] = mm; v4[i] = vv;
+      continue;
+    }
+    for (size_t x = lo; x < hi; ++x) {
+      bool out = false;
+      for (int r = 0; r < rg.n; ++r) out = out || (x >= rg.b[r] && x < rg.e[r]);
+      if (out) continue;
+      float pi = p[x], mi = m[x], vi = v[x];
+      adam_update(pi, g[x], mi, vi, grad_scale, weight_decay, beta1, beta2, eps, step_size, inv_sqrt_bc2);
+      p[x] = pi; m[x] = mi; v[x] = vi;
+    }
+  }
+  for (size_t x = n4 * 4 + (size_t)blockIdx.x * blockDim.x + threadIdx.x; x < n; x += stride) {
+    bool out = false;
+    for (int r = 0; r < rg.n; ++r) out = out || (x >= rg.b[r] && x < rg.e[r]);
+    if (out) continue;
+    float pi = p[x], mi = m[x], vi = v[x];
+    adam_update(pi, g[x], mi, vi, grad_scale, weight_decay, beta1, beta2, eps, step_size, inv_sqrt_bc2);
+    p[x] = pi; m[x] = mi; v[x] = vi;
+  }
+  __syncthreads();
+  if (threadIdx.x == 0) {
+    if (atomicAdd(&st->done, 1) == (int)gridDim.x - 1) {
+      st->step = t;
+      st->pow1 = q1; st->pow2 = q2;
+      st->done = 0;
+    }
+  }
+}
+
 static size_t adam_blocks(size_t n) {
   size_t blocks = (n / 4 + 255) / 256;
   if (blocks > 2048) blocks = 2048;
@@ -228,6 +410,44 @@
   return hipGetLastError();
 }
 
+int adam_max_ranges() { return kAdamMaxRanges; }
+
+hipError_t launch_adam_counted_ranges(float* p, const float* g, float* m, float* v, size_t n, float grad_scale, float eps, float weight_decay,
+                                      void* state, const size_t* ranges, int nr, hipStream_t st) {
+  if (nr <= 0) return launch_adam_counted(p, g, m, v, n, grad_scale, eps, weight_decay, state, st);
+  AdamRanges rg;
+  rg.n = nr;
+  size_t kept = n;
+  for (int r = 0; r < kAdamMaxRanges; ++r) {
+    rg.b[r] = r < nr ? ranges[2 * r] : 0;
+    rg.e[r] = r < nr ? ranges[2 * r + 1] : 0;
+    kept -= rg.e[r] - rg.b[r];
+  }
+  hipLaunchKernelGGL(adam_kernel_counted_ranges, dim3((unsigned)adam_blocks(kept)), dim3(256), 0, st, p, g, m, v, n, grad_scale, eps,
+                     weight_decay, static_cast<AdamState*>(state), rg);
+  return hipGetLastError();
+}
+
+hipError_t launch_wino4_step_multi(const WinoStepJob* jobs, int njobs, float grad_scale, float eps, float weight_decay, const void* state,
+                                   hipStream_t st) {
+  for (int base = 0; base < njobs; base += kStepMaxJobs) {
+    StepJobs js;
+    js.n = njobs - base < kStepMaxJobs ? njobs - base : kStepMaxJobs;
+    long wg = 0;
+    for (int q = 0; q < js.n; ++q) {
+      const WinoStepJob& in = jobs[base + q];
+      js.j[q] = StepJob{in.dU, in.p, in.m, in.v, in.U, in.Ut, in.dw, in.parts, in.K, in.C, (int)wg};
+      wg += (long)((in.K + kStepTile - 1) / kStepTile) * ((in.C + kStepTile - 1) / kStepTile);
+      if (wg >= (1L << 30)) return hipErrorInvalidValue;
+    }
+    hipLaunchKernelGGL(wino4_step_multi_kernel, dim3((unsigned)wg), dim3(256), 0, st, js, grad_scale, eps, weight_decay,
+                       static_cast<const AdamState*>(state));
+    hipError_t e = hipGetLastError();
+    if (e != hipSuccess) return e;
+  }
+  return hipSuccess;
+}
+
 hipError_t launch_adam(float* p, const float* g, float* m, float* v, size_t n, float grad_scale, float lr, float beta1,
                        float beta2, float eps, float weight_decay, int step, const float* dyn, hipStream_t st) {
   float step_size = 0.f, inv_sqrt_bc2 = 0.f;
diff --git a/hifihr_amd/csrc/hifihr_api.hip b/hifihr_amd/csrc/hifihr_api.hip
--- a/hifihr_amd/csrc/hifihr_api.hip
+++ b/hifihr_amd/csrc/hifihr_api.hip
@@ -620,6 +620,45 @@
   return HIFIHR_OK;
 }
 
+int hifihr_adam_max_ranges(void) { return hifihr::adam_max_ranges(); }
+
+int hifihr_adam_step_counted_ranges(float* params, const float* grads, float* exp_avg, float* exp_avg_sq, size_t n, float grad_scale, float eps,
+                                    float weight_decay, void* state_d, const size_t* excluded, int n_excluded, void* stream) {
+  if (!params || !grads || !exp_avg || !exp_avg_sq || !state_d) return fail(HIFIHR_EINVAL, "hifihr_adam_step_counted_ranges: bad argument");
+  if ((((uintptr_t)params | (uintptr_t)grads | (uintptr_t)exp_avg | (uintptr_t)exp_avg_sq) & 15) || ((uintptr_t)state_d & 7))
+    return fail(HIFIHR_EINVAL, "hifihr_adam_step_counted_ranges: buffers must be 16-byte aligned (the state: 8)");
+  if (n_excluded < 0 || n_excluded > hifihr::adam_max_ranges() || (n_excluded > 0 && !excluded))
+    return fail(HIFIHR_EINVAL, "hifihr_adam_step_counted_ranges: bad range table (0 .. hifihr_adam_max_ranges() pairs)");
+  for (int r = 0; r < n_excluded; ++r) {
+    const size_t b = excluded[2 * r], e = excluded[2 * r + 1];
+    if (b > e || e > n) return fail(HIFIHR_EINVAL, "hifihr_adam_step_counted_ranges: a range must satisfy begin <= end <= n");
+    for (int q = 0; q < r; ++q)
+      if (b < excluded[2 * q + 1] && excluded[2 * q] < e) return fail(HIFIHR_EINVAL, "hifihr_adam_step_counted_ranges: ranges overlap");
+  }
+  if (n == 0) return HIFIHR_OK;
+  HIP_TRY(hifihr::launch_adam_counted_ranges(params, grads, exp_avg, exp_avg_sq, n, grad_scale, eps, weight_decay, state_d, excluded, n_excluded,
+                                             (hipStream_t)stream));
+  return HIFIHR_OK;
+}
+
+int hifihr_wino4_step_multi(const hifihr_wino_step_job* jobs, int njobs, float grad_scale, float eps, float weight_decay, const void* state_d,
+                            void* stream) {
+  static_assert(sizeof(hifihr_wino_step_job) == sizeof(hifihr::WinoStepJob), "hifihr_wino_step_job layout");
+  if (!jobs || njobs <= 0 || !state_d || ((uintptr_t)state_d & 7)) return fail(HIFIHR_EINVAL, "hifihr_wino4_step_multi: bad argument");
+  for (int i = 0; i < njobs; ++i) {
+    const hifihr_wino_step_job& j = jobs[i];
+    if (!j.du_parts_d || !j.params_d || !j.exp_avg_d || !j.exp_avg_sq_d || j.parts < 1 || j.K <= 0 || j.C < 4 || j.C % 4 != 0 ||
+        (j.ut_d && j.K % 4 != 0))
+      return fail(HIFIHR_EINVAL, "hifihr_wino4_step_multi: bad job (pointers, parts >= 1, K > 0, C % 4 == 0, K % 4 == 0 with ut_d)");
+    if (((uintptr_t)j.du_parts_d | (uintptr_t)j.params_d | (uintptr_t)j.exp_avg_d | (uintptr_t)j.exp_avg_sq_d | (uintptr_t)j.u_d |
+         (uintptr_t)j.ut_d | (uintptr_t)j.dw_d) & 15)
+      return fail(HIFIHR_EINVAL, "hifihr_wino4_step_multi: buffers must be 16-byte aligned");
+  }
+  HIP_TRY(hifihr::launch_wino4_step_multi(reinterpret_cast<const hifihr::WinoStepJob*>(jobs), njobs, grad_scale, eps, weight_decay, state_d,
+                                          (hipStream_t)stream));
+  return HIFIHR_OK;
+}
+
 int hifihr_adam_step_dyn(float* params, const float* grads, float* exp_avg, float* exp_avg_sq, size_t n, float grad_scale,
                          float beta1, float beta2, float eps, float weight_decay, const float* dyn_d, void* stream) {
   if (!params || !grads || !exp_avg || !exp_avg_sq || !dyn_d) return fail(HIFIHR_EINVAL, "hifihr_adam_step_dyn: bad argument");
diff --git a/hifihr_amd/csrc/hifihr_internal.h b/hifihr_amd/csrc/hifihr_internal.h
--- a/hifihr_amd/csrc/hifihr_internal.h
+++ b/hifihr_amd/csrc/hifihr_internal.h
@@ -462,6 +462,12 @@
 size_t adam_state_bytes();
 hipError_t launch_adam_counted(float* p, const float* g, float* m, float* v, size_t n, float grad_scale, float eps, float weight_decay,
                                void* state, hipStream_t st);
+int adam_max_ranges();
+hipError_t launch_adam_counted_ranges(float* p, const float* g, float* m, float* v, size_t n, float grad_scale, float eps, float weight_decay,
+                                      void* state, const size_t* ranges, int nr, hipStream_t st);
+struct WinoStepJob { const float* dU; float *p, *m, *v, *U, *Ut, *dw; int parts, K, C, pad; };
+hipError_t launch_wino4_step_multi(const WinoStepJob* jobs, int njobs, float grad_scale, float eps, float weight_decay, const void* state,
+                                   hipStream_t st);
 hipError_t launch_adam(float* p, const float* g, float* m, float* v, size_t n, float grad_scale, float lr, float beta1,
                        float beta2, float eps, float weight_decay, int step, const float* dyn, hipStream_t st);
 size_t grad_guard_bytes();
diff --git a/hifihr_amd/ops.py b/hifihr_amd/ops.py
--- a/hifihr_amd/ops.py
+++ b/hifihr_amd/ops.py
@@ -667,6 +667,9 @@
         self.entries = {}
         self.table, self.njobs, self.dirty, self.active, self.served = None, 0, False, False, set()
         self._retired = []
+        self.current = {}
+        self.skipped = frozenset()
+        self._tables = {}
 
     def get(self, w, wk, kind):
         if not isinstance(w, torch.nn.Parameter) or wk.data_ptr() != w.data_ptr():
@@ -684,6 +687,48 @@
             return None
         return e[5] if (self.active and key in self.served) else None
 
+    def buffer(self, w, kind):
+        e = self.entries.get((w.data_ptr(), kind))
+        return e[5] if (e is not None and e[0] is w) else None
+
+    def mark_current(self, w, flat):
+        for kind in (3, 4):
+            if (w.data_ptr(), kind) in self.entries:
+                self.current[(w.data_ptr(), kind)] = (w._version, flat, flat._version)
+
+    def mark_keys(self, keys, flat):
+        for key in keys:
+            e = self.entries.get(key)
+            if e is not None:
+                self.current[key] = (e[0]._version, flat, flat._version)
+
+    def is_current(self, key):
+        sig, e = self.current.get(key), self.entries.get(key)
+        return sig is not None and e is not None and e[0]._version == sig[0] and sig[1]._version == sig[2]
+
+    def weights_written(self, flat, keep=()):
+        if self.current:
+            lo, hi = flat.data_ptr(), flat.data_ptr() + 4 * flat.numel()
+            for key in [k for k in self.current if lo <= k[0] < hi and k[0] not in keep]:
+                del self.current[key]
+
+    def invalidate(self):
+        self.current.clear()
+
+    def _job_list(self, keys):
+        return [(e[0], e[5], e[1], e[2], e[3], e[4]) for k, e in self.entries.items() if k in keys]
+
+    def refresh(self, keys):
+        stale = [k for k in keys if k in self.entries and not self.is_current(k)]
+        if stale:
+            jobs = self._job_list(set(stale))
+            table = get_lib().prep_jobs(jobs, jobs[0][0].device)
+            PROFILE.bracket("weight_prep", lambda: get_lib().weight_prep(table, len(jobs), 256))
+            self._retired.append((table, [j[1] for j in jobs]))
+            if len(self._retired) > 64:
+                del self._retired[:32]
+        return len(stale)
+
     def begin(self):
         live = {k: e for k, e in self.entries.items() if e[0].data_ptr() == k[0]}
         if len(live) != len(self.entries):
@@ -691,13 +736,26 @@
         if not self.entries:
             return
         lib = get_lib()
+        skip = frozenset(k for k in self.current if self.is_current(k)) if self.current else frozenset()
         if self.dirty:
-            jobs = [(e[0], e[5], e[1], e[2], e[3], e[4]) for e in self.entries.values()]
-            if self.table is not None:
-                self._retired.append((self.table, [e[5] for e in self.entries.values()]))
-            self.table, self.njobs = lib.prep_jobs(jobs, jobs[0][0].device), len(jobs)
+            if self._tables:
+                self._retired.extend(self._tables.values())
+                self._tables = {}
+            self.current = {k: v for k, v in self.current.items() if k in self.entries}
             self.served, self.dirty = set(self.entries.keys()), False
-        PROFILE.bracket("weight_prep", lambda: lib.weight_prep(self.table, self.njobs, 256))
+            self.table = None
+        if self.table is None or skip != self.skipped:
+            hit = self._tables.get(skip)
+            if hit is None:
+                jobs = self._job_list(self.entries.keys() - skip)
+                hit = (lib.prep_jobs(jobs, jobs[0][0].device) if jobs else None, len(jobs), [e[5] for e in self.entries.values()])
+                if len(self._tables) >= 8:
+                    self._retired.extend(self._tables.values())
+                    self._tables = {}
+                self._tables[skip] = hit
+            self.table, self.njobs, self.skipped = hit[0], hit[1], skip
+        if self.njobs:
+            PROFILE.bracket("weight_prep", lambda: lib.weight_prep(self.table, self.njobs, 256))
         self.active = True
 
     def end(self):
@@ -705,6 +763,10 @@
 
 
 _WEIGHT_PREP = _WeightPrep()
+
+
+def invalidate_prepared_weights():
+    _WEIGHT_PREP.invalidate()
 
 
 class _DeferredDw:
@@ -717,10 +779,18 @@
         self.pending = set()
         self.early = os.environ.get("HIFIHR_DEFER_EARLY", "1") != "0"
         self.side, self.home, self._streams, self.n_early = None, None, {}, 0
+        self.sink, self.nofuse = None, set()
+        self.fused = os.environ.get("HIFIHR_FUSED_WINO_STEP", "0") != "0"
 
     def wants(self, w, direct):
-        if self.side is not None and w.grad is not None and w.grad.data_ptr() in self.pending:
-            torch.cuda.current_stream(self.side.device).wait_stream(self.side)
+        if w.grad is not None and w.grad.data_ptr() in self.pending:
+            if self.sink is not None:
+                if self.sink.has_fused(w):
+                    raise RuntimeError("a second backward of a Winograd layer inside one prepared_weights() scope, after the fused optimizer pass "
+                                       "already updated it: run the scope with HIFIHR_FUSED_WINO_STEP=0 or without optimizer=")
+                self.nofuse.add(w.grad.data_ptr())
+            if self.side is not None:
+                torch.cuda.current_stream(self.side.device).wait_stream(self.side)
         return (self.on and self.active and direct and not _ASYNC_WGRAD.active and getattr(w, "_hifihr_grad_ready", None) is None
                 and (w.grad is None or w.grad.data_ptr() not in self.pending))
 
@@ -733,7 +803,7 @@
         self.pending.add(tgt.data_ptr())
 
     def clear(self):
-        self.jobs.clear(); self.halo.clear(); self.pending.clear()
+        self.jobs.clear(); self.halo.clear(); self.pending.clear(); self.nofuse.clear()
         if self.side is not None:
             if not torch.cuda.is_current_stream_capturing():
                 torch.cuda.current_stream(self.side.device).wait_stream(self.side)
@@ -743,6 +813,9 @@
         lib = get_lib() if (jobs or halo) else None
         if halo:
             PROFILE.bracket("halo_reduce_multi", lambda: lib.conv_halo_wgrad_reduce_multi([h[:3] for h in halo]))
+        if jobs and self.sink is not None:
+            keep = [j for j in jobs if j[2].data_ptr() in self.nofuse]
+            jobs = keep + self.sink.take_dw_jobs([j for j in jobs if j[2].data_ptr() not in self.nofuse])
         if jobs:
             PROFILE.bracket("wino_dw_multi", lambda: lib.wino4_dw_transform_multi([j[:5] for j in jobs]))
 
@@ -751,6 +824,7 @@
         halo, self.halo = self.halo, []
         self.pending.clear()
         self._run(jobs, halo)
+        self.nofuse.clear()
         if self.side is not None:
             cur = torch.cuda.current_stream(self.side.device)
             cur.wait_stream(self.side)
@@ -810,8 +884,10 @@
 
 class prepared_weights:
 
-    def __init__(self, async_wgrad=False):
+    def __init__(self, async_wgrad=False, optimizer=None):
         self.async_wgrad = bool(async_wgrad)
+        sink = getattr(optimizer, "wino_step_sink", None) if _DEFER_DW.fused else None
+        self.sink = sink() if sink is not None else None
 
     def __enter__(self):
         if torch.cuda.is_available() and torch.cuda.is_current_stream_capturing():
@@ -821,7 +897,8 @@
         _WEIGHT_PREP.begin()
         _DEFER_DW.clear()
         _DEFER_DW.active = True
-        _ASYNC_WGRAD.active = self.async_wgrad and not torch.cuda.is_current_stream_capturing()
+        _DEFER_DW.sink = self.sink
+        _ASYNC_WGRAD.active = self.async_wgrad and self.sink is None and not torch.cuda.is_current_stream_capturing()
         return self
 
     def __exit__(self, *exc):
@@ -831,6 +908,7 @@
             _DEFER_DW.flush()
         else:
             _DEFER_DW.clear()
+        _DEFER_DW.sink = None
         side_branch.join_pending()
         if _ASYNC_WGRAD.active:
             _ASYNC_WGRAD.active = False
diff --git a/hifihr_amd/optim.py b/hifihr_amd/optim.py
--- a/hifihr_amd/optim.py
+++ b/hifihr_amd/optim.py
@@ -67,6 +67,8 @@
         self._state_sig = None
         self._prepared = False
         self._guard = self._guard_ws = None
+        self._fused_ranges, self._fused_ptrs = [], set()
+        self._by_grad_ptr = None
         if max_grad_norm is not None:
             self._lib = get_lib()
             self._guard, self._guard_ws = self._lib.grad_guard_alloc(flat.flat.numel(), flat.flat.device)
@@ -115,12 +117,57 @@
     def zero_grad(self, set_to_none: bool = False):
         self.flatp.zero_grad()
 
+    def wino_step_sink(self):
+        self._fused_ranges, self._fused_ptrs = [], set()
+        if not self.graph_mode or self._state is None or self.max_grad_norm is not None:
+            return None
+        if torch.distributed.is_available() and torch.distributed.is_initialized() and torch.distributed.get_world_size() > 1:
+            return None
+        return self
+
+    def has_fused(self, p):
+        return p.data_ptr() in self._fused_ptrs
+
+    def take_dw_jobs(self, jobs):
+        from .ops import _WEIGHT_PREP, PROFILE
+        flat = self.flatp
+        if self._by_grad_ptr is None or self._by_grad_ptr[0] != (flat.grad.data_ptr(), flat.flat.data_ptr()):
+            self._by_grad_ptr = ((flat.grad.data_ptr(), flat.flat.data_ptr()),
+                                 {flat.grad.data_ptr() + 4 * o: (p, o) for p, o in zip(flat.params, flat.offsets)})
+        table, room = self._by_grad_ptr[1], int(self._lib.c.hifihr_adam_max_ranges()) - len(self._fused_ranges)
+        fused, rest = [], []
+        for job in jobs:
+            dU, parts, tgt, K, C = job[:5]
+            p, o = table.get(tgt.data_ptr(), (None, 0))
+            n = K * 9 * C
+            ok = (p is not None and len(fused) < room and p.numel() == n and p.data_ptr() == flat.flat.data_ptr() + 4 * o
+                  and p.grad is not None and p.grad.data_ptr() == tgt.data_ptr() and not getattr(p, "_backward_hooks", None)
+                  and not getattr(p, "_post_accumulate_grad_hooks", None) and getattr(p, "_hifihr_grad_ready", None) is None)
+            if not ok:
+                rest.append(job)
+                continue
+            fused.append(((dU, parts, flat.flat[o:o + n], self.exp_avg[o:o + n], self.exp_avg_sq[o:o + n], _WEIGHT_PREP.buffer(p, 3),
+                           _WEIGHT_PREP.buffer(p, 4), None, K, C), p, (o, o + n)))
+        if fused:
+            g = self.param_groups[0]
+            PROFILE.bracket("wino_step_multi", lambda: self._lib.wino4_step_multi([f[0] for f in fused], self.grad_scale, g["eps"],
+                                                                                 g["weight_decay"], self._state))
+            for _, p, rng in fused:
+                self._fused_ranges.append(rng)
+                self._fused_ptrs.add(p.data_ptr())
+                _WEIGHT_PREP.mark_current(p, flat.flat)
+        return rest
+
     @torch.no_grad()
     def step(self, closure=None):
         if self._lib is None:
             self._lib = get_lib()
         require_cuda(self.flatp.flat)
         g = self.param_groups[0]
+        fused, keep = self._fused_ranges, self._fused_ptrs
+        self._fused_ranges, self._fused_ptrs = [], set()
+        from .ops import _WEIGHT_PREP
+        _WEIGHT_PREP.weights_written(self.flatp.flat, keep)
         if self.graph_mode:
             capturing = self.flatp.flat.is_cuda and torch.cuda.is_current_stream_capturing()
             if not capturing:
@@ -132,6 +179,10 @@
                 self._lib.grad_norm(self.flatp.grad, self.grad_scale, self.max_grad_norm, self._guard, self._guard_ws)
                 self._lib.adam_step_guarded(self.flatp.flat, self.flatp.grad, self.exp_avg, self.exp_avg_sq, self.grad_scale, 0.0, 0.0, 0.0,
                                             g["eps"], g["weight_decay"], 0, self._state, self._guard)
+                return
+            if fused:
+                self._lib.adam_step_counted_ranges(self.flatp.flat, self.flatp.grad, self.exp_avg, self.exp_avg_sq, self.grad_scale, g["eps"],
+                                                   g["weight_decay"], self._state, fused)
                 return
             self._lib.adam_step_counted(self.flatp.flat, self.flatp.grad, self.exp_avg, self.exp_avg_sq, self.grad_scale, g["eps"],
                                         g["weight_decay"], self._state)
diff --git a/hifihr_amd/traineval.py b/hifihr_amd/traineval.py
--- a/hifihr_amd/traineval.py
+++ b/hifihr_amd/traineval.py
@@ -114,7 +114,7 @@
 def forward_backward(model, loss_func, optimizer, examples, args, dat_name="FreiHand"):
     from .ops import prepared_weights
     dp = torch.distributed.is_available() and torch.distributed.is_initialized() and torch.distributed.get_world_size() > 1
-    with prepared_weights(async_wgrad=not dp):
+    with prepared_weights(async_wgrad=not dp, optimizer=None if dp else optimizer):
         return _forward_backward(model, loss_func, optimizer, examples, args, dat_name)
 
 
@@ -179,6 +179,8 @@
     def __init__(self, model, loss_func, optimizer, examples, args, dat_name="FreiHand", warmup=3, reducer=None):
         self.model, self.loss_func, self.opt, self.args, self.dat_name = model, loss_func, optimizer, args, dat_name
         self.reducer = reducer
+        self._prep_skipped = self._prep_fused = ()
+        from .ops import _WEIGHT_PREP
         self.static = {k: (v.clone() if torch.is_tensor(v) else v) for k, v in examples.items()}
         split = reducer is not None
         flat = optimizer.flatp
@@ -211,6 +213,8 @@
                 optimizer.prepare_step()
                 with torch.cuda.graph(self.graph):
                     self.loss, self.loss_dic = train_step(model, loss_func, optimizer, self.static, args, dat_name)
+                self._prep_skipped = tuple(_WEIGHT_PREP.skipped)
+                self._prep_fused = tuple(k for k in self._prep_skipped if _WEIGHT_PREP.is_current(k))
         except BaseException:
             if split:
                 reducer.pause_hooks(False)
@@ -250,8 +254,13 @@
             self.reducer.all_reduce_flat()
             self.opt.step()
         else:
+            from .ops import _WEIGHT_PREP
             self.opt.prepare_step()
+            if self._prep_skipped:
+                _WEIGHT_PREP.refresh(self._prep_skipped)
             self.graph.replay()
+            _WEIGHT_PREP.weights_written(self.opt.flatp.flat)
+            _WEIGHT_PREP.mark_keys(self._prep_fused, self.opt.flatp.flat)
             self.opt.note_step_done()
         return self.loss, self.loss_dic
 
diff --git a/include/hifihr.h b/include/hifihr.h
--- a/include/hifihr.h
+++ b/include/hifihr.h
@@ -136,6 +136,17 @@
 int hifihr_adam_step_dyn(float* params_d, const float* grads_d, float* exp_avg_d, float* exp_avg_sq_d, size_t n,
                          float grad_scale, float beta1, float beta2, float eps, float weight_decay, const float* dyn_d,
                          void* stream);
+int hifihr_adam_max_ranges(void);
+int hifihr_adam_step_counted_ranges(float* params_d, const float* grads_d, float* exp_avg_d, float* exp_avg_sq_d, size_t n, float grad_scale,
+                                    float eps, float weight_decay, void* state_d, const size_t* excluded, int n_excluded, void* stream);
+typedef struct hifihr_wino_step_job {
+  const float* du_parts_d;
+  float *params_d, *exp_avg_d, *exp_avg_sq_d;
+  float *u_d, *ut_d, *dw_d;
+  int parts, K, C, reserved;
+} hifihr_wino_step_job;
+int hifihr_wino4_step_multi(const hifihr_wino_step_job* jobs, int njobs, float grad_scale, float eps, float weight_decay,
+                            const void* state_d, void* stream);
 
 size_t hifihr_grad_guard_bytes(void);
 size_t hifihr_grad_norm_workspace_bytes(size_t n);
```
